# saholmes/stark-mlwe

Hardware: AMD Instinct MI355X
Metric: prove ms + Fr-NTT achieved GB/s, 2^20/2^24 trace at 1/2/4/8 GPUs (higher is better)
Workload: dtype u256 (4x u64 Montgomery limbs, Pallas Fr); 1 GPU; one 2^20-row trace x 4 columns (2^20 rows per GPU), blowup 8: LDE (iNTT + coset NTT) + DEEP-ALI merge + FRI folds + Poseidon leaf hashes + Poseidon-Merkle trees (schedule [16,16,8]), kernels only; log_trace_per_gpu=20, log_blowup=3, field=pallas_fr

## Files before the change

### stark_mlwe_amd/csrc/capi_poseidon.hip

```cpp
#include <algorithm>
#include <cstring>
#include <type_traits>
#include "poseidon_launch.hpp"
#include "poseidon_dev.hpp"
#include "poseidon_pair.hpp"
#include "poseidon_coop.hpp"
#include "poseidon_chain.hpp"
#include "poseidon_wave.hpp"
#include "poseidon_transcript.hpp"
#include "fri_dev.hpp"
#include "merkle_batch.hpp"

using namespace stark;

static const size_t kMaxLds = 160 * 1024;
static inline int poseidon_block(int t) { return (size_t)t * 32 * 64 <= kMaxLds ? 64 : 32; }
static inline size_t poseidon_lds(int t, int block) { return (size_t)t * 32 * block; }
enum class PoseidonForm { Lane, WavePair, OneWave, FiveWave, Wide };
enum class PoseidonOp { MerkleLevel, LeafLayer, TrHash, ColumnSponges, RaggedSponges, DeviceTranscript };
constexpr size_t kChainMaxNodes = 256, kChainMaxLeaves = 2048, kChainMaxSponges = 512, kCoopMaxNodes = 4096, kCoopMaxLeaves = 4096, kCoopMaxSponges = 4096;
static PoseidonForm poseidon_form(const stark_ctx* ctx, const stark_params* p, PoseidonOp op, size_t n) {
    const PoseidonDev& d = p->dev;
    const bool lane_only = ctx->opt.poseidon_lane_only, one_wave = ctx->opt.sponge_one_wave;
    const bool chain = !lane_only && !one_wave && d.t == 17 && d.rf == 8 && d.rp == 64 && d.chain_a;
    switch (op) {
    case PoseidonOp::MerkleLevel:
        if ((ctx->side_commit || ctx->opt.merkle_wave_pair) && !lane_only && (d.t == 9 || d.t == 17)) return PoseidonForm::WavePair;
        if (chain && n <= kChainMaxNodes) return PoseidonForm::FiveWave;
        if (!lane_only && (d.t == 9 || d.t == 17)) return n <= kCoopMaxNodes ? PoseidonForm::OneWave : PoseidonForm::WavePair;
        if (!lane_only && (d.t == 33 || d.t == 65 || d.t == 129) && n <= 0x7fffffffu) return PoseidonForm::Wide;
        return PoseidonForm::Lane;
    case PoseidonOp::LeafLayer:
        if (ctx->side_commit && !lane_only) return PoseidonForm::WavePair;
        if (chain && n <= kChainMaxLeaves) return PoseidonForm::FiveWave;
        if (!lane_only && !one_wave && n <= kCoopMaxLeaves) return PoseidonForm::OneWave;
        return lane_only ? PoseidonForm::Lane : PoseidonForm::WavePair;
    case PoseidonOp::TrHash:
        if (chain && n <= kChainMaxSponges) return PoseidonForm::FiveWave;
        return !lane_only && n <= kCoopMaxSponges ? PoseidonForm::OneWave : PoseidonForm::Lane;
    case PoseidonOp::RaggedSponges:
        if (lane_only) return PoseidonForm::Lane;
        [[fallthrough]];
    case PoseidonOp::ColumnSponges:
        return d.chain_a && !one_wave ? PoseidonForm::FiveWave : PoseidonForm::OneWave;
    case PoseidonOp::DeviceTranscript:
        return chain && n <= kChainMaxSponges ? PoseidonForm::FiveWave : PoseidonForm::OneWave;
    }
    return PoseidonForm::Lane;
}
static inline row::Consts row_consts_of(const stark_ctx* ctx) {
    const RowConstsHost h = row_consts_host(); row::Consts RK; for (int i = 0; i < 9; ++i) RK.ni[i] = h.ni[i]; for (int i = 0; i < 5; ++i) RK.t[i] = h.t[i]; RK.dbg = (uint32_t)ctx->opt.sponge_debug; return RK;
}

static int32_t ctx_leaf_init(stark_ctx* ctx, fr_t** out) {
    if (!ctx->leaf_init) {
        const fr_t AB = host::h_tag("FSv1-ABSORB-BYTES"), CH = host::h_tag("FSv1-CHALLENGE");
        fr_t init[17]; for (auto& x : init) x = host::h_zero();
        init[0] = AB; init[1] = host::h_words("FRI/leaf/poseidon")[0]; init[2] = AB; init[3] = host::h_words("FRI/leaf")[0];
         init[6] = CH; init[7] = AB; init[8] = host::h_words("leaf")[0]; init[16] = host::h_tag("FSv1-TRANSCRIPT-INIT");
        stark_params* tp = nullptr; STARK_TRY(ctx_transcript_params(ctx, &tp));
        const host::PoseidonConsts& c = tp->ref;
        fr_t blob[17 + 51 + 40];
        for (auto& x : blob) x = host::h_zero();
        for (int j = 0; j < 17; ++j) blob[j] = init[j];
        fr_t x[17]; for (int j = 0; j < 17; ++j) x[j] = fr_pow5<PallasFr>(host::h_add(init[j], c.rc_full[j]));
        for (int i = 0; i < 17; ++i) {
            fr_t k = host::h_zero();
            for (int j = 0; j < 17; ++j) if (j != 4 && j != 5) k = host::h_add(k, host::h_mul(c.mds[(size_t)i * 17 + j], x[j]));
            blob[17 + i] = k; blob[34 + i] = c.mds[(size_t)i * 17 + 4]; blob[51 + i] = c.mds[(size_t)i * 17 + 5];
            uint32_t* m45 = reinterpret_cast<uint32_t*>(&blob[68]);
            const fr_t k20 = fr_from_u64<PallasFr>(1ull << FR29_SBOX_SHIFT);
            fr29_const_from<PallasFr>(host::h_mul(c.mds[(size_t)i * 17 + 4], k20), m45 + 9 * i); fr29_const_from<PallasFr>(host::h_mul(c.mds[(size_t)i * 17 + 5], k20), m45 + 9 * (17 + i));
        }
        DevMem d; STARK_TRY(d.fill_sync(ctx, blob, sizeof(blob)));
        ctx->leaf_init = std::move(d);
    }
    *out = ctx->leaf_init.fr(); return STARK_OK;
}

namespace stark {

static int32_t tr_frame(stark_ctx* ctx, const char* tag, fr_t** dev, int* np, int* ns) {
    const std::string key(tag);
    auto it = ctx->tr_frames.find(key);
    if (it == ctx->tr_frames.end()) {
        std::vector<fr_t> fr; const int p = host::tr_hash_frame(tag, fr);
        DevMem d; STARK_TRY(d.fill_sync(ctx, fr.data(), fr.size() * sizeof(fr_t)));
        it = ctx->tr_frames.emplace(key, std::move(d)).first; ctx->tr_frame_dims[key] = {p, (int)fr.size() - p};
    }
    *dev = it->second.fr(); *np = ctx->tr_frame_dims[key].first; *ns = ctx->tr_frame_dims[key].second; return STARK_OK;
}
static int32_t launch_tr_hash(stark_ctx* ctx, stark_params* tp, PoseidonForm form, const TrStream& T, fr_t* out_dev) {
    const bool ragged = T.layout == TrStream::Ragged;
    switch (form) {
    case PoseidonForm::FiveWave:
        if (ragged) hipLaunchKernelGGL(k_tr_hash_chain_ragged, dim3((unsigned)T.n), dim3(320), chain_lds_bytes(), ctx->stream, tp->dev, T, row_consts_of(ctx), out_dev);
        else hipLaunchKernelGGL(k_tr_hash_chain, dim3((unsigned)T.n), dim3(320), chain_lds_bytes(), ctx->stream, tp->dev, T, row_consts_of(ctx), out_dev);
        break;
    case PoseidonForm::OneWave:
        if (ragged) hipLaunchKernelGGL((k_tr_hash_coop<true, true>), dim3((unsigned)T.n), dim3(64), coop_lds_bytes(17), ctx->stream, tp->dev, T, out_dev);
        else if (T.layout == TrStream::Equal) hipLaunchKernelGGL(k_tr_hash_coop<false>, dim3((unsigned)T.n), dim3(64), coop_lds_bytes(17), ctx->stream, tp->dev, T, out_dev);
        else hipLaunchKernelGGL(k_tr_hash_coop<true>, dim3((unsigned)T.n), dim3(64), coop_lds_bytes(17), ctx->stream, tp->dev, T, out_dev);
        break;
    default: {
        const int block = 64;
        if (ragged) hipLaunchKernelGGL(k_tr_hash_ragged, dim3((unsigned)((T.n + block - 1) / block)), dim3(block), poseidon_lds(17, block), ctx->stream, tp->dev, T, out_dev);
        else hipLaunchKernelGGL(k_tr_hash, dim3((unsigned)((T.n + block - 1) / block)), dim3(block), poseidon_lds(17, block), ctx->stream, tp->dev, T, out_dev);
    } }
    STARK_HIP(ctx, hipGetLastError());
    return STARK_OK;
}
int32_t tr_hash_dev(stark_ctx* ctx, const char* tag, const fr_t* fields_dev, size_t k, size_t n, fr_t* out_dev) {
    stark_params* tp = nullptr; STARK_TRY(ctx_transcript_params(ctx, &tp));
    fr_t* frame = nullptr; int np = 0, ns = 0; STARK_TRY(tr_frame(ctx, tag, &frame, &np, &ns));
    if (n == 0) return STARK_OK;
    const TrStream T = TrStream::equal(frame, np, ns, fields_dev, k, n, host::h_tag("FSv1-TRANSCRIPT-INIT"));
    return launch_tr_hash(ctx, tp, poseidon_form(ctx, tp, PoseidonOp::TrHash, n), T, out_dev);
}
static int32_t tr_hash_columns(stark_ctx* ctx, const char* const tags[4], const fr_t* const cols[4], const fr_t* const* ptrs_dev, size_t nblocks, size_t n0, fr_t* out_dev) {
    stark_params* tp = nullptr; STARK_TRY(ctx_transcript_params(ctx, &tp));
    TrStream T{}; T.layout = ptrs_dev ? TrStream::BatchColumns : TrStream::Columns; T.n = nblocks; T.batch = ptrs_dev; T.cap = host::h_tag("FSv1-TRANSCRIPT-INIT");
    for (int c = 0; c < 4; ++c) {
        fr_t* frame = nullptr; int np = 0, ns = 0; STARK_TRY(tr_frame(ctx, tags[c], &frame, &np, &ns));
        T.prefix[c] = frame; T.np[c] = np; T.suffix[c] = frame + np; T.ns[c] = ns; T.fields[c] = cols ? cols[c] : nullptr; T.k[c] = n0;
    }
    return launch_tr_hash(ctx, tp, poseidon_form(ctx, tp, PoseidonOp::ColumnSponges, nblocks), T, out_dev);
}
int32_t tr_hash_columns4_dev(stark_ctx* ctx, const char* const tags[4], const fr_t* const cols[4], size_t n0, fr_t* out4_dev) {
    return tr_hash_columns(ctx, tags, cols, nullptr, 4, n0, out4_dev);
}
int32_t tr_hash_columns_batch_dev(stark_ctx* ctx, const char* const tags[4], const fr_t* const* ptrs_dev, size_t batch, size_t n0, fr_t* out_dev) {
    return tr_hash_columns(ctx, tags, nullptr, ptrs_dev, 4 * batch, n0, out_dev);
}
int32_t tr_hash_many_dev(stark_ctx* ctx, size_t n, const char* const* tags, const fr_t* const* fields, const size_t* k, fr_t* out_dev, bool column_sponges) {
    stark_params* tp = nullptr; STARK_TRY(ctx_transcript_params(ctx, &tp));
    std::vector<TrFrameRef> fr(n);
    for (size_t i = 0; i < n; ++i) { fr_t* frame = nullptr; STARK_TRY(tr_frame(ctx, tags[i], &frame, &fr[i].np, &fr[i].ns)); fr[i].frame = frame; }
    if (n == 0) return STARK_OK;
    if (n > 0x7fffffffu) return ctx->fail(STARK_ERR_UNSUPPORTED, "tr_hash_many: more than 2^31 - 1 items in one call");
    const std::vector<TrStream::Item> items = tr_ragged_items(fr.data(), fields, k, n);
    DevBuf d; STARK_HIP(ctx, d.alloc(ctx, n * sizeof(TrStream::Item))); STARK_TRY(ctx_upload_staged(ctx, d.p, items.data(), n * sizeof(TrStream::Item)));
    const TrStream T = tr_ragged_stream((const TrStream::Item*)d.p, n, host::h_tag("FSv1-TRANSCRIPT-INIT"));
    return launch_tr_hash(ctx, tp, poseidon_form(ctx, tp, column_sponges ? PoseidonOp::ColumnSponges : PoseidonOp::RaggedSponges, n), T, out_dev);
}
int32_t tr_hash_host1(stark_ctx* ctx, const char* tag, const std::vector<fr_t>& fields, fr_t* out) {
    DevBuf in, o; STARK_HIP(ctx, in.alloc(ctx, fields.size() * sizeof(fr_t))); STARK_HIP(ctx, o.alloc(ctx, sizeof(fr_t)));
    STARK_TRY(ctx_upload_staged(ctx, in.p, fields.data(), fields.size() * sizeof(fr_t)));
    STARK_TRY(tr_hash_dev(ctx, tag, in.fr(), fields.size(), 1, o.fr()));
    STARK_HIP(ctx, o.download_sync(out, sizeof(fr_t)));
    return STARK_OK;
}
int32_t tr_stream_on(stark_ctx* ctx, stark_params* tp, fr_t* state, uint32_t* pos, const fr_t* fields, size_t n, bool finish, fr_t* out) {
    if (poseidon_form(ctx, tp, PoseidonOp::DeviceTranscript, 1) == PoseidonForm::FiveWave)
        hipLaunchKernelGGL(k_tr_stream_chain, dim3(1), dim3(320), chain_lds_bytes(), ctx->stream, tp->dev, row_consts_of(ctx), state, pos, fields, (uint64_t)n, finish ? 1 : 0, finish ? out : (fr_t*)nullptr);
    else
        hipLaunchKernelGGL(k_tr_stream, dim3(1), dim3(64), coop_lds_bytes(17), ctx->stream, tp->dev, state, pos, fields, (uint64_t)n, finish ? 1 : 0, finish ? out : (fr_t*)nullptr);
    STARK_HIP(ctx, hipGetLastError()); return STARK_OK;
}
int32_t tr_batch_on(stark_ctx* ctx, stark_params* tp, const TrBatchStream& T, size_t n_for_form) {
    if (!T.n_active) return STARK_OK;
    if (poseidon_form(ctx, tp, PoseidonOp::DeviceTranscript, n_for_form) == PoseidonForm::FiveWave)
        for (uint32_t sg = 0; sg < (uint32_t)T.nseg; ++sg)
            hipLaunchKernelGGL(k_tr_batch_chain, dim3((unsigned)T.n_active), dim3(320), chain_lds_bytes(), ctx->stream, tp->dev, row_consts_of(ctx), T, sg);
    else
        hipLaunchKernelGGL(k_tr_batch, dim3((unsigned)T.n_active), dim3(64), coop_lds_bytes(17), ctx->stream, tp->dev, T);
    STARK_HIP(ctx, hipGetLastError()); return STARK_OK;
}

}

extern "C" {

int32_t stark_poseidon_permute_batch_dev(stark_ctx_t* ctx, stark_params_t* p, uint64_t* states, size_t n) {
    if (!ctx || !p || (!states && n)) return STARK_ERR_INVALID_ARG;
    STARK_TRY(ctx_enter(ctx));
    if (!n) return STARK_OK;
    const int block = poseidon_block(p->dev.t);
    hipLaunchKernelGGL(k_permute_batch, dim3((unsigned)((n + block - 1) / block)), dim3(block), poseidon_lds(p->dev.t, block), ctx->stream, p->dev, as_fr(states), n);
    STARK_HIP(ctx, hipGetLastError()); return STARK_OK;
}
int32_t stark_poseidon_permute_batch(stark_ctx_t* ctx, stark_params_t* p, uint64_t* states, size_t n) {
    if (!ctx || !p || (!states && n)) return STARK_ERR_INVALID_ARG;
    STARK_TRY(ctx_enter(ctx));
    size_t bytes = n * p->dev.t * sizeof(fr_t); DevBuf d; CallerUploads up(ctx); STARK_HIP(ctx, up.up(d, states, bytes));
    STARK_TRY(stark_poseidon_permute_batch_dev(ctx, p, (uint64_t*)d.p, n));
    STARK_HIP(ctx, up.download_sync(states, d.p, bytes));
    return STARK_OK;
}
static int32_t hash_stream(stark_ctx_t* ctx, stark_params_t* p, int mode, const uint64_t* a, size_t na, const uint64_t* b, size_t nb, const fr_t& tag, size_t n, uint64_t* out) {
    DevBuf da, db, dout; CallerUploads up(ctx);
    STARK_HIP(ctx, up.up(da, a, n * na * sizeof(fr_t))); STARK_HIP(ctx, up.up(db, b, n * nb * sizeof(fr_t))); STARK_HIP(ctx, dout.alloc(ctx, n * sizeof(fr_t)));
    const int block = poseidon_block(p->dev.t);
    hipLaunchKernelGGL(k_hash_stream, dim3((unsigned)((n + block - 1) / block)), dim3(block), poseidon_lds(p->dev.t, block), ctx->stream, p->dev, mode, da.fr(), na, db.fr(), nb, tag, n, dout.fr());
    STARK_HIP(ctx, hipGetLastError());
    STARK_HIP(ctx, up.download_sync(out, dout.p, n * sizeof(fr_t)));
    return STARK_OK;
}
int32_t stark_poseidon_hash_with_ds_dynamic(stark_ctx_t* ctx, stark_params_t* p, const uint64_t* ds, size_t nds, const uint64_t* in, size_t cnt, size_t n, uint64_t* out) {
    if (!ctx || !p || !out || (!ds && nds) || (!in && cnt)) return STARK_ERR_INVALID_ARG;
    STARK_TRY(ctx_enter(ctx));
    if (!n) return STARK_OK;
    return hash_stream(ctx, p, 0, ds, nds, in, cnt, host::h_zero(), n, out);
}
int32_t stark_poseidon_hash_with_ds(stark_ctx_t* ctx, stark_params_t* p, const uint64_t* in, size_t cnt, const uint64_t* ds_tag, uint64_t* out) {
    if (!ctx || !p || !out || !ds_tag || (!in && cnt)) return STARK_ERR_INVALID_ARG;
    STARK_TRY(ctx_enter(ctx));
    if (p->dev.t != 17) return ctx->fail(STARK_ERR_INVALID_ARG, "hash_with_ds is the fixed t=17 sponge");
    return hash_stream(ctx, p, 1, nullptr, 0, in, cnt, load_fr(ds_tag), 1, out);
}
}
static int32_t pair_block8_form(stark_ctx* ctx, const stark_params* p, bool* on) {
    *on = ctx->opt.poseidon_block8 && p->dev.t == 17 && p->dev.rp % 8 == 0;
    if (*on && (!p->dev.blk8_efrag || !p->dev.blk8_lfrag || !p->dev.blk8_unit_frag || !p->dev.blk8_gfrag || !p->dev.rc_partial_scaled29)) return ctx->fail(STARK_ERR_UNSUPPORTED, "poseidon_block8: the parameter set has no block-8 tables");
    return STARK_OK;
}
template <class DS>
static int32_t launch_ds(stark_ctx_t* ctx, hipStream_t st, stark_params_t* p, const DS& D, fr_t* out) {
    if (!D.n_out) return STARK_OK;
    const int t = p->dev.t; const unsigned nodes = (unsigned)D.n_out, pairs = (unsigned)((D.n_out + 63) / 64);
    bool b8 = false; STARK_TRY(pair_block8_form(ctx, p, &b8));
    switch (poseidon_form(ctx, p, PoseidonOp::MerkleLevel, D.n_out)) {
    case PoseidonForm::FiveWave: hipLaunchKernelGGL(k_hash_ds_chain<DS>, dim3(nodes), dim3(320), chain_lds_bytes(), st, p->dev, D, row_consts_of(ctx), out); break;
    case PoseidonForm::OneWave:
        if (t == 17) hipLaunchKernelGGL((k_hash_ds_coop<17, DS>), dim3(nodes), dim3(64), coop_lds_bytes(17), st, p->dev, D, out);
        else hipLaunchKernelGGL((k_hash_ds_coop<9, DS>), dim3(nodes), dim3(64), coop_lds_bytes(9), st, p->dev, D, out);
        break;
    case PoseidonForm::WavePair:
        if constexpr (std::is_same<DS, DsStream>::value) {
            if (t == 17 && ctx->opt.merkle_node16_pair && D.mode == 0 && D.arity == 16 && D.n_in == 16 * D.n_out) {
                if (b8) hipLaunchKernelGGL(k_node16_pair<true>, dim3(pairs), dim3(128), pair_lds_bytes(17), st, p->dev, D.arity_f, D.level_f, D.label_f, D.pos0, D.in0, D.n_out, out);
                else hipLaunchKernelGGL(k_node16_pair<false>, dim3(pairs), dim3(128), pair_lds_bytes(17), st, p->dev, D.arity_f, D.level_f, D.label_f, D.pos0, D.in0, D.n_out, out);
                break;
            }
        }
        if (t == 17 && b8) hipLaunchKernelGGL((k_hash_ds2<17, DS, true>), dim3(pairs), dim3(128), pair_lds_bytes(17), st, p->dev, D, out);
        else if (t == 17) hipLaunchKernelGGL((k_hash_ds2<17, DS>), dim3(pairs), dim3(128), pair_lds_bytes(17), st, p->dev, D, out);
        else hipLaunchKernelGGL((k_hash_ds2<9, DS>), dim3(pairs), dim3(128), pair_lds_bytes(9), st, p->dev, D, out);
        break;
    case PoseidonForm::Wide:
        if (t == 33) hipLaunchKernelGGL((k_hash_ds_wave<33, DS>), dim3(nodes), dim3(64), wave_lds_bytes(t), st, p->dev, D, out);
        else if (t == 65) hipLaunchKernelGGL((k_hash_ds_wave<65, DS>), dim3(nodes), dim3(64), wave_lds_bytes(t), st, p->dev, D, out);
        else hipLaunchKernelGGL((k_hash_ds_wave<129, DS>), dim3(nodes), dim3(64), wave_lds_bytes(t), st, p->dev, D, out);
        break;
    case PoseidonForm::Lane: {
        const int block = poseidon_block(t);
        hipLaunchKernelGGL(k_hash_ds<DS>, dim3((unsigned)((D.n_out + block - 1) / block)), dim3(block), poseidon_lds(t, block), st, p->dev, D, out);
    } }
    STARK_HIP(ctx, hipGetLastError()); return STARK_OK;
}
int32_t stark::hash_ds_on(stark_ctx* ctx, hipStream_t st, stark_params* p, const DsStream& D, fr_t* out) { return launch_ds(ctx, st, p, D, out); }
int32_t stark::hash_ds_on(stark_ctx* ctx, hipStream_t st, stark_params* p, const DsGatherStream& D, fr_t* out) { return launch_ds(ctx, st, p, D, out); }
int32_t stark::hash_ds_on(stark_ctx* ctx, hipStream_t st, stark_params* p, const DsBatchStream& D, fr_t* out) { return launch_ds(ctx, st, p, D, out); }
int32_t stark::hash_ds_on(stark_ctx* ctx, hipStream_t st, stark_params* p, const DsBatchPairStream& D, fr_t* out) { return launch_ds(ctx, st, p, D, out); }
int32_t stark::hash_ds_on(stark_ctx* ctx, hipStream_t st, stark_params* p, const DsBatchPairPtrStream& D, fr_t* out) { return launch_ds(ctx, st, p, D, out); }
int32_t stark::hash_ds_on(stark_ctx* ctx, hipStream_t st, stark_params* p, const DsRaggedStream& D, fr_t* out) { return launch_ds(ctx, st, p, D, out); }
static void lds_attr(const void* kernel) { (void)hipFuncSetAttribute(kernel, hipFuncAttributeMaxDynamicSharedMemorySize, (int)kMaxLds); }
template <class DS>
static void ds_attrs() {
    lds_attr((const void*)k_hash_ds<DS>); lds_attr((const void*)k_hash_ds2<17, DS>); lds_attr((const void*)k_hash_ds2<17, DS, true>); lds_attr((const void*)k_hash_ds2<9, DS>); lds_attr((const void*)k_hash_ds_chain<DS>);
}
void stark::poseidon_set_attrs() {
    ds_attrs<DsStream>(); ds_attrs<DsGatherStream>(); ds_attrs<DsBatchStream>(); ds_attrs<DsBatchPairStream>(); ds_attrs<DsBatchPairPtrStream>(); ds_attrs<DsRaggedStream>();
    for (const void* k : {(const void*)k_leaf_pair, (const void*)k_permute_batch, (const void*)k_tr_hash, (const void*)k_hash_stream, (const void*)k_leaf_pair2<false>, (const void*)k_leaf_pair2<true>, (const void*)k_node16_pair<false>, (const void*)k_node16_pair<true>,
                          (const void*)k_tr_hash_chain, (const void*)k_tr_hash_chain_ragged, (const void*)k_tr_hash_ragged, (const void*)k_leaf_pair_chain, (const void*)k_tr_stream_chain, (const void*)k_tr_batch_chain})
        lds_attr(k);
}
extern "C" {
int32_t stark_poseidon_hash_ds_batch_dev(stark_ctx_t* ctx, stark_params_t* p, size_t arity, uint32_t level, uint64_t pos0, uint64_t label, const uint64_t* in, size_t n_in, uint64_t* out) {
    if (!ctx || !p || !in || !out || arity == 0) return STARK_ERR_INVALID_ARG;
    STARK_TRY(ctx_enter(ctx));
    if (host::width_for_arity(arity) != p->dev.t) return ctx->fail(STARK_ERR_INVALID_ARG, "arity incompatible with Poseidon width");
    STARK_TRY(ctx_enter(ctx));
    return hash_ds_on(ctx, ctx->stream, p, DsStream::make(0, arity, level, pos0, label, as_fr(in), nullptr, n_in), as_fr(out));
}
int32_t stark_poseidon_hash_ds_batch(stark_ctx_t* ctx, stark_params_t* p, size_t arity, uint32_t level, uint64_t pos0, uint64_t label, const uint64_t* in, size_t n_in, uint64_t* out) {
    if (!ctx || !p || !in || !out || arity == 0) return STARK_ERR_INVALID_ARG;
    STARK_TRY(ctx_enter(ctx));
    size_t n_out = (n_in + arity - 1) / arity; DevBuf di, dout; CallerUploads up(ctx); STARK_HIP(ctx, up.up(di, in, n_in * sizeof(fr_t))); STARK_HIP(ctx, dout.alloc(ctx, n_out * sizeof(fr_t)));
    STARK_TRY(stark_poseidon_hash_ds_batch_dev(ctx, p, arity, level, pos0, label, (const uint64_t*)di.p, n_in, (uint64_t*)dout.p));
    STARK_HIP(ctx, up.download_sync(out, dout.p, n_out * sizeof(fr_t)));
    return STARK_OK;
}
}
namespace stark {
static bool same_consts(const host::PoseidonConsts& a, const host::PoseidonConsts& b) {
    if (a.t != b.t || a.rf != b.rf || a.rp != b.rp || a.mds.size() != b.mds.size() || a.rc_full.size() != b.rc_full.size() || a.rc_partial.size() != b.rc_partial.size()) return false;
    for (size_t i = 0; i < a.mds.size(); ++i) if (!fr_eq(a.mds[i], b.mds[i])) return false;
    for (size_t i = 0; i < a.rc_full.size(); ++i) if (!fr_eq(a.rc_full[i], b.rc_full[i])) return false;
    for (size_t i = 0; i < a.rc_partial.size(); ++i) if (!fr_eq(a.rc_partial[i], b.rc_partial[i])) return false;
    return true;
}
int32_t leaf_pair_hash_on(stark_ctx* ctx, hipStream_t st, const fr_t* f, const fr_t* f_next, size_t n, size_t m, fr_t* h) {
    if (!n) return STARK_OK;
    stark_params* tp = nullptr; STARK_TRY(ctx_transcript_params(ctx, &tp));
    fr_t* init = nullptr; STARK_TRY(ctx_leaf_init(ctx, &init));
    const LeafStream L{init, f, f_next, m, n};
    bool b8 = false; STARK_TRY(pair_block8_form(ctx, tp, &b8));
    switch (poseidon_form(ctx, tp, PoseidonOp::LeafLayer, n)) {
    case PoseidonForm::FiveWave: hipLaunchKernelGGL(k_leaf_pair_chain, dim3((unsigned)n), dim3(320), chain_lds_bytes(), st, tp->dev, row_consts_of(ctx), L, h); break;
    case PoseidonForm::OneWave: hipLaunchKernelGGL(k_leaf_pair_coop, dim3((unsigned)n), dim3(64), coop_lds_bytes(17), st, tp->dev, L, h); break;
    case PoseidonForm::WavePair:
        if (b8) hipLaunchKernelGGL(k_leaf_pair2<true>, dim3((unsigned)((n + 63) / 64)), dim3(128), pair_lds_bytes(17), st, tp->dev, init + 17, f, f_next, n, m, h);
        else hipLaunchKernelGGL(k_leaf_pair2<false>, dim3((unsigned)((n + 63) / 64)), dim3(128), pair_lds_bytes(17), st, tp->dev, init + 17, f, f_next, n, m, h);
        break;
    default: hipLaunchKernelGGL(k_leaf_pair, dim3((unsigned)((n + 63) / 64)), dim3(64), poseidon_lds(17, 64), st, tp->dev, L, h);
    }
    STARK_HIP(ctx, hipGetLastError()); return STARK_OK;
}
}
extern "C" {
int32_t stark_leaf_pair_hash_dev(stark_ctx_t* ctx, stark_params_t* tp, const uint64_t* f, const uint64_t* f_next, size_t n, size_t m, uint64_t* h) {
    if (!ctx || (!f && n) || (!h && n) || m == 0) return STARK_ERR_INVALID_ARG;
    STARK_TRY(ctx_enter(ctx));
    if (tp) {
        if (tp->dev.t != 17) return ctx->fail(STARK_ERR_INVALID_ARG, "leaf hash uses the t=17 transcript permutation");
        stark_params* mine = nullptr; STARK_TRY(ctx_transcript_params(ctx, &mine));
        if (tp != mine && !same_consts(tp->ref, mine->ref)) return ctx->fail(STARK_ERR_INVALID_ARG, "hash_leaf_pair is defined over transcript::default_params(); the handle holds other constants");
    }
    return leaf_pair_hash_on(ctx, ctx->stream, as_fr(f), as_fr(f_next), n, m, as_fr(h));
}
int32_t stark_leaf_pair_hash(stark_ctx_t* ctx, stark_params_t* tp, const uint64_t* f, const uint64_t* f_next, size_t n, size_t m, uint64_t* h) {
    if (!ctx || (!f && n) || (!h && n) || m == 0) return STARK_ERR_INVALID_ARG;
    STARK_TRY(ctx_enter(ctx));
    size_t nn = f_next ? (n + m - 1) / m : 0; DevBuf df, dn, dh; CallerUploads up(ctx);
    STARK_HIP(ctx, up.up(df, f, n * sizeof(fr_t))); STARK_HIP(ctx, up.up(dn, f_next, nn * sizeof(fr_t))); STARK_HIP(ctx, dh.alloc(ctx, n * sizeof(fr_t)));
    STARK_TRY(stark_leaf_pair_hash_dev(ctx, tp, (const uint64_t*)df.p, f_next ? (const uint64_t*)dn.p : nullptr, n, m, (uint64_t*)dh.p));
    STARK_HIP(ctx, up.download_sync(h, dh.p, n * sizeof(fr_t))); return STARK_OK;
}
int32_t stark_tr_hash_fields_tagged_dev(stark_ctx_t* ctx, stark_params_t* tp, const char* tag, const uint64_t* fields, size_t k, size_t n, uint64_t* out) {
    if (!ctx || !tag || (!fields && k && n) || (!out && n)) return STARK_ERR_INVALID_ARG;
    STARK_TRY(ctx_enter(ctx));
    (void)tp;
    return tr_hash_dev(ctx, tag, as_fr(fields), k, n, as_fr(out));
}
int32_t stark_tr_hash_fields_tagged(stark_ctx_t* ctx, stark_params_t* tp, const char* tag, const uint64_t* fields, size_t k, size_t n, uint64_t* out) {
    if (!ctx || !tag || (!fields && k && n) || (!out && n)) return STARK_ERR_INVALID_ARG;
    STARK_TRY(ctx_enter(ctx));
    DevBuf di, dout; CallerUploads up(ctx); STARK_HIP(ctx, up.up(di, fields, n * k * sizeof(fr_t))); STARK_HIP(ctx, dout.alloc(ctx, n * sizeof(fr_t)));
    STARK_TRY(stark_tr_hash_fields_tagged_dev(ctx, tp, tag, (const uint64_t*)di.p, k, n, (uint64_t*)dout.p));
    STARK_HIP(ctx, up.download_sync(out, dout.p, n * sizeof(fr_t))); return STARK_OK;
}
int32_t stark_tr_hash_many_dev(stark_ctx_t* ctx, size_t n, const char* const* tags, const uint64_t* const* fields, const size_t* k, uint64_t* out) {
    if (!ctx) return STARK_ERR_INVALID_ARG;
    if (!n) return STARK_OK;
    if (!tags || !k || !out) return STARK_ERR_INVALID_ARG;
    STARK_TRY(ctx_enter(ctx));
    const uintptr_t o0 = (uintptr_t)out, o1 = o0 + n * sizeof(fr_t);
    for (size_t i = 0; i < n; ++i) {
        if (!tags[i]) return ctx->fail(STARK_ERR_INVALID_ARG, "tr_hash_many: null tag " + std::to_string(i));
        if (!k[i]) continue;
        if (!fields || !fields[i]) return ctx->fail(STARK_ERR_INVALID_ARG, "tr_hash_many: null fields with k > 0, item " + std::to_string(i));
        const uintptr_t f0 = (uintptr_t)fields[i];
        if (f0 < o1 && o0 < f0 + k[i] * sizeof(fr_t)) return ctx->fail(STARK_ERR_INVALID_ARG, "tr_hash_many: out overlaps the fields of item " + std::to_string(i));
    }
    return tr_hash_many_dev(ctx, n, tags, reinterpret_cast<const fr_t* const*>(fields), k, as_fr(out), false);
}

}
namespace stark {
int32_t merkle_build_on(stark_ctx* ctx, hipStream_t st, stark_params* p, size_t arity, uint64_t label, const fr_t* leaves, size_t n, int pairs, const fr_t* cp, size_t cp_div,
                        uint64_t first_pos, uint32_t level0, size_t stop_at_len, DevBuf&& level0_block, std::unique_ptr<stark_tree>& out) {
    if (n == 0) return ctx->fail(STARK_ERR_INVALID_ARG, "no leaves");
    if (host::width_for_arity(arity) != p->dev.t) return ctx->fail(STARK_ERR_INVALID_ARG, "arity incompatible with Poseidon width");
    if (arity == 1 && n > 1) return ctx->fail(STARK_ERR_UNSUPPORTED, "arity 1 with more than one leaf never terminates in the reference");
    std::unique_ptr<stark_tree> T(new stark_tree(ctx, p, arity, label));
    auto add_level = [&](DevBuf&& b, size_t len) { T->levels.push_back(b.fr()); T->lens.push_back(len); T->blocks.push_back(std::move(b)); };
    const bool moved_in = level0_block.p && !pairs;
    { DevBuf l0; if (moved_in) l0 = std::move(level0_block); else STARK_TRY(l0.take(ctx, n * sizeof(fr_t))); add_level(std::move(l0), n); }
    if (pairs) STARK_TRY(hash_ds_on(ctx, st, p, DsStream::make(1, arity, 0xFFFFFFFFu, first_pos, label, leaves, cp, n, cp_div), T->levels[0]));
    else if (!moved_in && hipMemcpyAsync(T->levels[0], leaves, n * sizeof(fr_t), hipMemcpyDeviceToDevice, st) != hipSuccess) return ctx->fail(STARK_ERR_HIP, "copy leaves");
    uint32_t level = level0; uint64_t pos = first_pos; size_t stop = stop_at_len > 0 ? stop_at_len : 1;
    while (T->lens.back() > stop) {
        size_t len = T->lens.back(), nn = (len + arity - 1) / arity;
        if (pos % arity) return ctx->fail(STARK_ERR_INVALID_ARG, "shard offset not aligned to the arity");
        pos /= arity;
        { DevBuf nx; STARK_TRY(nx.take(ctx, nn * sizeof(fr_t))); add_level(std::move(nx), nn); }
        STARK_TRY(hash_ds_on(ctx, st, p, DsStream::make(0, arity, level, pos, label, T->levels[T->levels.size() - 2], nullptr, len), T->levels.back()));
        level += 1;
    }
    out = std::move(T); return STARK_OK;
}
}
extern "C" {
int32_t stark_merkle_build_dev(stark_ctx_t* ctx, stark_params_t* p, size_t arity, uint64_t label, const uint64_t* leaves, size_t n, int32_t pairs, const uint64_t* cp,
                               uint64_t first_pos, uint32_t level0, int32_t stop_at_len, stark_tree_t** out) {
    if (!ctx || !p || !leaves || !out || arity == 0 || (pairs && !cp)) return ctx ? ctx->fail(STARK_ERR_INVALID_ARG, "bad merkle args") : STARK_ERR_INVALID_ARG;
    STARK_TRY(ctx_enter(ctx));
    std::unique_ptr<stark_tree> T;
    STARK_TRY(merkle_build_on(ctx, ctx->stream, p, arity, label, as_fr(leaves), n, pairs, as_fr(cp), 1, first_pos, level0, stop_at_len > 0 ? (size_t)stop_at_len : 0, DevBuf(), T));
    *out = T.release(); return STARK_OK;
}
int32_t stark_merkle_build(stark_ctx_t* ctx, stark_params_t* p, size_t arity, uint64_t label, const uint64_t* leaves, size_t n, int32_t pairs, const uint64_t* cp, stark_tree_t** out) {
    if (!ctx || !p || !leaves || !out || (pairs && !cp)) return STARK_ERR_INVALID_ARG;
    STARK_TRY(ctx_enter(ctx));
    if (n == 0) return ctx->fail(STARK_ERR_INVALID_ARG, "no leaves");
    DevBuf dl, dc; CallerUploads up(ctx); STARK_HIP(ctx, up.up(dl, leaves, n * sizeof(fr_t)));
    if (pairs) STARK_HIP(ctx, up.up(dc, cp, n * sizeof(fr_t)));
    STARK_TRY(stark_merkle_build_dev(ctx, p, arity, label, (const uint64_t*)dl.p, n, pairs, pairs ? (const uint64_t*)dc.p : nullptr, 0, 0, 0, out));
    STARK_HIP(ctx, up.sync()); return STARK_OK;
}
int32_t stark_merkle_num_levels(stark_tree_t* t) { return t ? (int32_t)t->levels.size() : STARK_ERR_INVALID_ARG; }
size_t stark_merkle_level_len(stark_tree_t* t, int32_t lvl) { return (t && lvl >= 0 && (size_t)lvl < t->lens.size()) ? t->lens[lvl] : 0; }
const uint64_t* stark_merkle_level_dev(stark_tree_t* t, int32_t lvl) { return (t && lvl >= 0 && (size_t)lvl < t->levels.size()) ? (const uint64_t*)t->levels[lvl] : nullptr; }
int32_t stark_merkle_level(stark_tree_t* t, int32_t lvl, uint64_t* out) {
    if (!t || !out || lvl < 0 || (size_t)lvl >= t->levels.size()) return STARK_ERR_INVALID_ARG;
    stark_ctx* ctx = t->ctx; STARK_TRY(ctx_enter(ctx));
    STARK_HIP(ctx, hipMemcpyAsync(out, t->levels[lvl], t->lens[lvl] * sizeof(fr_t), hipMemcpyDeviceToHost, ctx->stream)); STARK_HIP(ctx, hipStreamSynchronize(ctx->stream)); return STARK_OK;
}
int32_t stark_merkle_root(stark_tree_t* t, uint64_t* out4) {
    if (!t || !out4) return STARK_ERR_INVALID_ARG;
    if (t->lens.back() != 1) return t->ctx->fail(STARK_ERR_INVALID_ARG, "partial (sharded) tree has no root");
    return stark_merkle_level(t, (int32_t)t->levels.size() - 1, out4);
}
int32_t stark_merkle_gather(stark_tree_t* t, int32_t lvl, const size_t* idx, size_t k, uint64_t* out) {
    if (!t || (!idx && k) || (!out && k) || lvl < 0 || (size_t)lvl >= t->levels.size()) return STARK_ERR_INVALID_ARG;
    stark_ctx* ctx = t->ctx; if (!k) return STARK_OK;
    STARK_TRY(ctx_enter(ctx));
    for (size_t i = 0; i < k; ++i) if (idx[i] >= t->lens[lvl]) return ctx->fail(STARK_ERR_INVALID_ARG, "gather index out of range");
    MerkleGatherList G; G.level(t->levels[lvl], std::vector<size_t>(idx, idx + k));
    return gather_rows(ctx, G, nullptr, out);
}
int32_t stark_merkle_free(stark_tree_t* t) { if (!t) return STARK_ERR_INVALID_ARG; delete t; return STARK_OK; }

}

namespace stark {
struct MerkleBatchDevExec {
    stark_ctx* ctx; stark_params* p; std::shared_ptr<TreeBlocks> blocks; DevArena mem;
    MerkleBatchDevExec(stark_ctx* c, stark_params* p_) : ctx(c), p(p_), blocks(std::make_shared<TreeBlocks>()), mem(c) {}
    int32_t level_block(size_t n_fr, fr_t** out) {
        DevBuf b; STARK_TRY(b.take(ctx, n_fr * sizeof(fr_t))); *out = b.fr(); blocks->blocks.push_back(std::move(b)); return STARK_OK;
    }
    int32_t tables(const uint64_t* labels, const fr_t* const* leaves, const fr_t* const* cp, size_t B, const uint64_t** labels_x, const fr_t* const** leaves_x, const fr_t* const** cp_x) {
        std::vector<uint64_t> h((cp ? 3 : 2) * B);
        for (size_t b = 0; b < B; ++b) { h[b] = labels[b]; h[B + b] = (uint64_t)(uintptr_t)leaves[b]; if (cp) h[2 * B + b] = (uint64_t)(uintptr_t)cp[b]; }
        uint64_t* d = nullptr; STARK_TRY(mem.put(h, &d));
        *labels_x = d; *leaves_x = (const fr_t* const*)(d + B); *cp_x = cp ? (const fr_t* const*)(d + 2 * B) : nullptr; return STARK_OK;
    }
    int32_t copy_rows(const fr_t* const* src_x, size_t n, size_t B, fr_t* dst) {
        for (size_t b0 = 0; b0 < B; b0 += 65535)
            hipLaunchKernelGGL(k_copy_rows, dim3((unsigned)((n + 255) / 256), (unsigned)std::min<size_t>(65535, B - b0)), dim3(256), 0, ctx->stream, src_x + b0, (uint64_t)n, dst + b0 * n);
        STARK_HIP(ctx, hipGetLastError()); return STARK_OK;
    }
    int32_t pair_level(const DsBatchPairPtrStream& D, fr_t* out) { return hash_ds_on(ctx, ctx->stream, p, D, out); }
    int32_t ds_level(const DsBatchStream& D, fr_t* out) { return hash_ds_on(ctx, ctx->stream, p, D, out); }
};
int32_t merkle_build_batch_on(stark_ctx* ctx, stark_params* p, size_t arity, size_t batch, const uint64_t* labels, const uint64_t* const* leaves, size_t n, int pairs,
                              const uint64_t* const* cp, stark_tree** out) {
    for (size_t b = 0; b < batch; ++b) out[b] = nullptr;
    if (n == 0) return ctx->fail(STARK_ERR_INVALID_ARG, "no leaves");
    if (arity == 0 || host::width_for_arity(arity) != p->dev.t) return ctx->fail(STARK_ERR_INVALID_ARG, "arity incompatible with Poseidon width");
    if (arity == 1 && n > 1) return ctx->fail(STARK_ERR_UNSUPPORTED, "arity 1 with more than one leaf never terminates in the reference");
    for (size_t b = 0; b < batch; ++b) if (!leaves[b]) return ctx->fail(STARK_ERR_INVALID_ARG, "null leaves entry");
    if (n > 0x7fffffffu / batch) return ctx->fail(STARK_ERR_INVALID_ARG, "batch x n exceeds 2^31 - 1 leaves: one level of the batch is one launch");
    MerkleBatchDevExec X(ctx, p);
    std::vector<size_t> lens; std::vector<fr_t*> base;
    STARK_TRY(merkle_build_batch(X, arity, batch, labels, reinterpret_cast<const fr_t* const*>(leaves), n, pairs, reinterpret_cast<const fr_t* const*>(cp), lens, base));
    std::vector<std::unique_ptr<stark_tree>> trees(batch);
    for (size_t b = 0; b < batch; ++b) {
        trees[b].reset(new stark_tree(ctx, p, arity, labels[b])); trees[b]->shared = X.blocks;
        for (size_t v = 0; v < lens.size(); ++v) { trees[b]->levels.push_back(base[v] + b * lens[v]); trees[b]->lens.push_back(lens[v]); }
    }
    for (size_t b = 0; b < batch; ++b) out[b] = trees[b].release();
    return STARK_OK;
}
struct MerkleMixedDevExec : MerkleBatchDevExec {
    using MerkleBatchDevExec::MerkleBatchDevExec;
    int32_t segments(const std::vector<DsRaggedStream::Seg>& h, const DsRaggedStream::Seg** x) { DsRaggedStream::Seg* d = nullptr; STARK_TRY(mem.put(h, &d)); *x = d; return STARK_OK; }
    int32_t copy_ragged(const DsRaggedStream& D, fr_t* dst) {
        hipLaunchKernelGGL(k_copy_ragged, dim3((unsigned)((D.n_out + 255) / 256)), dim3(256), 0, ctx->stream, D, dst);
        STARK_HIP(ctx, hipGetLastError()); return STARK_OK;
    }
    int32_t ragged_level(const DsRaggedStream& D, fr_t* out) { return hash_ds_on(ctx, ctx->stream, p, D, out); }
};
int32_t merkle_build_mixed_batch_on(stark_ctx* ctx, stark_params* p, size_t arity, size_t batch, const uint64_t* labels, const uint64_t* const* leaves, const size_t* n, int pairs,
                                    const uint64_t* const* cp, stark_tree** out) {
    for (size_t b = 0; b < batch; ++b) out[b] = nullptr;
    if (arity == 0 || host::width_for_arity(arity) != p->dev.t) return ctx->fail(STARK_ERR_INVALID_ARG, "arity incompatible with Poseidon width");
    size_t sum = 0;
    for (size_t b = 0; b < batch; ++b) {
        if (!leaves[b]) return ctx->fail(STARK_ERR_INVALID_ARG, "null leaves entry");
        if (n[b] == 0) return ctx->fail(STARK_ERR_INVALID_ARG, "no leaves");
        if (n[b] > 0x7fffffffu - sum) return ctx->fail(STARK_ERR_INVALID_ARG, "the sum of n exceeds 2^31 - 1 leaves: one level of the batch is one launch");
        sum += n[b];
    }
    if (arity == 1 && sum > batch) return ctx->fail(STARK_ERR_UNSUPPORTED, "arity 1 with more than one leaf never terminates in the reference");
    MerkleMixedDevExec X(ctx, p);
    std::vector<std::vector<size_t>> lens, at; std::vector<fr_t*> base;
    STARK_TRY(merkle_build_mixed_batch(X, arity, batch, labels, reinterpret_cast<const fr_t* const*>(leaves), n, pairs, reinterpret_cast<const fr_t* const*>(cp), lens, at, base));
    std::vector<std::unique_ptr<stark_tree>> trees(batch);
    for (size_t b = 0; b < batch; ++b) {
        trees[b].reset(new stark_tree(ctx, p, arity, labels[b])); trees[b]->shared = X.blocks;
        for (size_t v = 0; v < lens[b].size(); ++v) { trees[b]->levels.push_back(base[v] + at[b][v]); trees[b]->lens.push_back(lens[b][v]); }
    }
    for (size_t b = 0; b < batch; ++b) out[b] = trees[b].release();
    return STARK_OK;
}
int32_t gather_rows(stark_ctx* ctx, const MerkleGatherList& G, fr_t* out_dev, void* out_host) {
    const size_t k = G.size(), nb = G.base.size();
    if (!k) return STARK_OK;
    std::vector<uint64_t> h(nb + 2 * k + (k + 1) / 2);
    for (size_t i = 0; i < nb; ++i) h[i] = (uint64_t)(uintptr_t)G.base[i];
    for (size_t i = 0; i < k; ++i) { h[nb + i] = G.index[i]; h[nb + k + i] = G.row_of(i); }
    memcpy(h.data() + nb + 2 * k, G.src.data(), k * 4);
    DevBuf d, o; STARK_HIP(ctx, d.alloc(ctx, h.size() * 8));
    if (!out_dev) { STARK_HIP(ctx, o.alloc(ctx, k * sizeof(fr_t))); out_dev = o.fr(); }
    STARK_TRY(ctx_upload_staged(ctx, d.p, h.data(), h.size() * 8));
    const uint64_t* t = (const uint64_t*)d.p;
    hipLaunchKernelGGL(k_gather_rows, dim3((unsigned)((k + 255) / 256)), dim3(256), 0, ctx->stream, (const fr_t* const*)t, (const uint32_t*)(t + nb + 2 * k), t + nb, t + nb + k, (uint64_t)k, out_dev);
    STARK_HIP(ctx, hipGetLastError());
    if (!out_host) return STARK_OK;
    STARK_HIP(ctx, hipMemcpyAsync(out_host, out_dev, k * sizeof(fr_t), hipMemcpyDeviceToHost, ctx->stream)); STARK_HIP(ctx, hipStreamSynchronize(ctx->stream));
    return STARK_OK;
}
struct MerkleOpenDevExec { stark_ctx* ctx; int32_t gather(const MerkleGatherList& G, fr_t* out_host) { return gather_rows(ctx, G, nullptr, out_host); } };
static int32_t same_ctx_trees(stark_tree* const* trees, size_t batch, stark_ctx** ctx) {
    for (size_t b = 0; b < batch; ++b) if (!trees[b]) return STARK_ERR_INVALID_ARG;
    stark_ctx* c = trees[0]->ctx;
    for (size_t b = 1; b < batch; ++b) if (trees[b]->ctx != c) return c->fail(STARK_ERR_INVALID_ARG, "the trees of a batch must share one context");
    for (size_t b = 0; b < batch; ++b) if (trees[b]->lens.back() != 1) return c->fail(STARK_ERR_INVALID_ARG, "partial (sharded) tree in a batch");
    *ctx = c; return STARK_OK;
}
}

extern "C" {
int32_t stark_merkle_build_batch_dev(stark_ctx_t* ctx, stark_params_t* p, size_t arity, size_t batch, const uint64_t* tree_labels, const uint64_t* const* leaves, size_t n, int32_t pairs,
                                     const uint64_t* const* cp, stark_tree_t** out) {
    if (!batch) return STARK_OK;
    if (!out) return ctx ? ctx->fail(STARK_ERR_INVALID_ARG, "bad merkle batch args") : STARK_ERR_INVALID_ARG;
    for (size_t b = 0; b < batch; ++b) out[b] = nullptr;
    if (!ctx || !p || !tree_labels || !leaves || (pairs && !cp)) return ctx ? ctx->fail(STARK_ERR_INVALID_ARG, "bad merkle batch args") : STARK_ERR_INVALID_ARG;
    STARK_TRY(ctx_enter(ctx));
    return merkle_build_batch_on(ctx, p, arity, batch, tree_labels, leaves, n, pairs, pairs ? cp : nullptr, out);
}
int32_t stark_merkle_build_mixed_batch_dev(stark_ctx_t* ctx, stark_params_t* p, size_t arity, size_t batch, const uint64_t* tree_labels, const uint64_t* const* leaves, const size_t* n,
                                           int32_t pairs, const uint64_t* const* cp, stark_tree_t** out) {
    if (!batch) return STARK_OK;
    if (!out) return ctx ? ctx->fail(STARK_ERR_INVALID_ARG, "bad merkle batch args") : STARK_ERR_INVALID_ARG;
    for (size_t b = 0; b < batch; ++b) out[b] = nullptr;
    if (!ctx || !p || !tree_labels || !leaves || !n || (pairs && !cp)) return ctx ? ctx->fail(STARK_ERR_INVALID_ARG, "bad merkle batch args") : STARK_ERR_INVALID_ARG;
    STARK_TRY(ctx_enter(ctx));
    return merkle_build_mixed_batch_on(ctx, p, arity, batch, tree_labels, leaves, n, pairs, pairs ? cp : nullptr, out);
}
int32_t stark_merkle_roots_batch(stark_tree_t* const* trees, size_t batch, uint64_t* roots) {
    if (!batch) return STARK_OK;
    if (!trees || !roots) return STARK_ERR_INVALID_ARG;
    stark_ctx* ctx = nullptr; STARK_TRY(same_ctx_trees(trees, batch, &ctx));
    STARK_TRY(ctx_enter(ctx));
    MerkleGatherList G;
    for (size_t b = 0; b < batch; ++b) G.level(trees[b]->levels.back(), std::vector<size_t>(1, 0));
    return gather_rows(ctx, G, nullptr, roots);
}
int32_t stark_merkle_open_batch(stark_tree_t* const* trees, size_t batch, const size_t* idx, const size_t* idx_off, stark_proof_t** out) {
    if (!batch) return STARK_OK;
    if (!out) return STARK_ERR_INVALID_ARG;
    for (size_t b = 0; b < batch; ++b) out[b] = nullptr;
    if (!trees || !idx || !idx_off) return STARK_ERR_INVALID_ARG;
    stark_ctx* ctx = nullptr; STARK_TRY(same_ctx_trees(trees, batch, &ctx));
    STARK_TRY(ctx_enter(ctx));
    std::vector<MerkleTreeView> views(batch);
    for (size_t b = 0; b < batch; ++b) views[b] = MerkleTreeView{trees[b]->arity, &trees[b]->lens, trees[b]->levels.data()};
    MerkleOpenDevExec X{ctx}; std::vector<std::vector<uint8_t>> proofs;
    const int32_t rc = merkle_open_batch(X, views.data(), batch, idx, idx_off, proofs);
    if (rc == -1) return ctx->fail(STARK_ERR_INVALID_ARG, "open batch: idx_off not increasing, an empty index list or a leaf index out of range");
    if (rc) return rc;
    std::vector<std::unique_ptr<stark_proof>> pf(batch);
    for (size_t b = 0; b < batch; ++b) { pf[b].reset(new stark_proof()); pf[b]->bytes = std::move(proofs[b]); }
    hand_out(pf, out); return STARK_OK;
}
int32_t stark_merkle_open(stark_tree_t* t, const size_t* idx, size_t k, uint8_t* buf, size_t cap, size_t* len) {
    if (!t || !len || (!idx && k)) return STARK_ERR_INVALID_ARG;
    stark_ctx* ctx = t->ctx;
    if (!k) return ctx->fail(STARK_ERR_INVALID_ARG, "open_many: empty indices");
    if (t->lens.back() != 1) return ctx->fail(STARK_ERR_INVALID_ARG, "cannot open a partial tree");
    for (size_t i = 0; i < k; ++i) if (idx[i] >= t->lens[0]) return ctx->fail(STARK_ERR_INVALID_ARG, "leaf index out of range");
    STARK_TRY(ctx_enter(ctx));
    const MerkleTreeView view{t->arity, &t->lens, t->levels.data()}; const size_t off[2] = {0, k};
    MerkleOpenDevExec X{ctx}; std::vector<std::vector<uint8_t>> proofs;
    STARK_TRY(merkle_open_batch(X, &view, 1, idx, off, proofs));
    const std::vector<uint8_t>& b = proofs[0];
    *len = b.size();
    if (buf) { if (cap < b.size()) return ctx->fail(STARK_ERR_INVALID_ARG, "buffer too small"); memcpy(buf, b.data(), b.size()); }
    return STARK_OK;
}
}
```

### stark_mlwe_amd/csrc/host_util.hpp

```cpp
#pragma once
#include <cstdint>
#include <cstring>
#include <string>
#include <vector>
#include "fr.hpp"
#include "fr29.hpp"

namespace stark {
namespace host {

struct Blake3 {
    static constexpr uint32_t kIV[8] = {0x6A09E667u, 0xBB67AE85u, 0x3C6EF372u, 0xA54FF53Au, 0x510E527Fu, 0x9B05688Cu, 0x1F83D9ABu, 0x5BE0CD19u};
    enum : uint32_t { F_CHUNK_START = 1, F_CHUNK_END = 2, F_PARENT = 4, F_ROOT = 8 };
    static uint32_t ror(uint32_t x, unsigned n) { return (x >> n) | (x << (32 - n)); }
    static void mix(uint32_t* v, int a, int b, int c, int d, uint32_t x, uint32_t y) {
        v[a] += v[b] + x; v[d] = ror(v[d] ^ v[a], 16); v[c] += v[d]; v[b] = ror(v[b] ^ v[c], 12);
        v[a] += v[b] + y; v[d] = ror(v[d] ^ v[a], 8);  v[c] += v[d]; v[b] = ror(v[b] ^ v[c], 7);
    }
    static void compress(const uint32_t h[8], const uint8_t block[64], uint32_t blen, uint64_t ctr, uint32_t flags, uint32_t out[16]) {
        static const uint8_t sched[7][16] = {
            {0, 1, 2, 3, 4, 5, 6, 7, 8, 9, 10, 11, 12, 13, 14, 15}, {2, 6, 3, 10, 7, 0, 4, 13, 1, 11, 12, 5, 9, 14, 15, 8},
            {3, 4, 10, 12, 13, 2, 7, 14, 6, 5, 9, 0, 11, 15, 8, 1}, {10, 7, 12, 9, 14, 3, 13, 15, 4, 0, 11, 2, 5, 8, 1, 6},
            {12, 13, 9, 11, 15, 10, 14, 8, 7, 2, 5, 3, 0, 1, 6, 4}, {9, 14, 11, 5, 8, 12, 15, 1, 13, 3, 0, 10, 2, 6, 4, 7},
            {11, 15, 5, 0, 1, 9, 8, 6, 14, 10, 2, 12, 3, 4, 7, 13}};
// ... 8 lines not shown
            mix(v, 2, 6, 10, 14, m[s[4]], m[s[5]]);  mix(v, 3, 7, 11, 15, m[s[6]], m[s[7]]);
            mix(v, 0, 5, 10, 15, m[s[8]], m[s[9]]);  mix(v, 1, 6, 11, 12, m[s[10]], m[s[11]]);
            mix(v, 2, 7, 8, 13, m[s[12]], m[s[13]]); mix(v, 3, 4, 9, 14, m[s[14]], m[s[15]]);
        }
        for (int i = 0; i < 8; ++i) { out[i] = v[i] ^ v[i + 8]; out[i + 8] = v[i + 8] ^ h[i]; }
    }
    struct Node { uint32_t h[8]; uint8_t block[64]; uint32_t blen; uint64_t ctr; uint32_t flags; };
    static void cv_of(const Node& n, uint32_t extra, uint32_t cv[8]) { uint32_t o[16]; compress(n.h, n.block, n.blen, n.ctr, n.flags | extra, o); memcpy(cv, o, 32); }
    static Node chunk_node(const uint8_t* p, size_t len, uint64_t index) {
        Node n; memcpy(n.h, kIV, 32); n.ctr = index;
        size_t off = 0; bool first = true;
        while (len - off > 64) {
            uint32_t o[16]; compress(n.h, p + off, 64, index, first ? F_CHUNK_START : 0, o); memcpy(n.h, o, 32);
            off += 64; first = false;
        }
        memset(n.block, 0, 64); memcpy(n.block, p + off, len - off); n.blen = (uint32_t)(len - off);
        n.flags = (first ? F_CHUNK_START : 0) | F_CHUNK_END;
        return n;
    }
    static Node subtree(const uint8_t* p, size_t len, uint64_t index) {
        if (len <= 1024) return chunk_node(p, len, index);
        size_t chunks = (len + 1023) / 1024, left = 1; while (left * 2 < chunks) left *= 2;
        Node l = subtree(p, left * 1024, index), r = subtree(p + left * 1024, len - left * 1024, index + left);
        Node n; memcpy(n.h, kIV, 32); n.ctr = 0; n.blen = 64; n.flags = F_PARENT;
        uint32_t a[8], b[8]; cv_of(l, 0, a); cv_of(r, 0, b);
        for (int i = 0; i < 8; ++i) for (int j = 0; j < 4; ++j) { n.block[4 * i + j] = (uint8_t)(a[i] >> (8 * j)); n.block[32 + 4 * i + j] = (uint8_t)(b[i] >> (8 * j)); }
        return n;
    }
    static void hash(const uint8_t* p, size_t len, uint8_t out[32]) {
        Node root = subtree(p, len, 0);
        if (root.flags & F_PARENT) root.ctr = 0;
        uint32_t cv[8]; cv_of(root, F_ROOT, cv);
        for (int i = 0; i < 8; ++i) for (int j = 0; j < 4; ++j) out[4 * i + j] = (uint8_t)(cv[i] >> (8 * j));
    }
};

struct ChaCha12Rng {
    uint32_t st[16]; uint32_t out[16]; unsigned have = 0;
    explicit ChaCha12Rng(const uint8_t seed[32]) {
        st[0] = 0x61707865u; st[1] = 0x3320646eu; st[2] = 0x79622d32u; st[3] = 0x6b206574u;
        for (int i = 0; i < 8; ++i) st[4 + i] = (uint32_t)seed[4 * i] | (uint32_t)seed[4 * i + 1] << 8 | (uint32_t)seed[4 * i + 2] << 16 | (uint32_t)seed[4 * i + 3] << 24;
        st[12] = st[13] = st[14] = st[15] = 0;
    }
    static uint32_t rol(uint32_t x, unsigned n) { return (x << n) | (x >> (32 - n)); }
    void block() {
        uint32_t x[16]; memcpy(x, st, 64);
        auto Q = [&](int a, int b, int c, int d) {
            x[a] += x[b]; x[d] = rol(x[d] ^ x[a], 16); x[c] += x[d]; x[b] = rol(x[b] ^ x[c], 12);
            x[a] += x[b]; x[d] = rol(x[d] ^ x[a], 8);  x[c] += x[d]; x[b] = rol(x[b] ^ x[c], 7); };
        for (int i = 0; i < 6; ++i) { Q(0, 4, 8, 12); Q(1, 5, 9, 13); Q(2, 6, 10, 14); Q(3, 7, 11, 15); Q(0, 5, 10, 15); Q(1, 6, 11, 12); Q(2, 7, 8, 13); Q(3, 4, 9, 14); }
        for (int i = 0; i < 16; ++i) out[i] = x[i] + st[i];
        if (++st[12] == 0) ++st[13];
        have = 16;
    }
    uint32_t next_u32() { if (!have) block(); return out[16 - have--]; }
    uint64_t next_u64() { uint64_t lo = next_u32(), hi = next_u32(); return lo | hi << 32; }
};

typedef PallasFr PF;
inline fr_t h_one() { return fr_one<PF>(); }
inline fr_t h_zero() { return fr_zero<PF>(); }
inline fr_t h_mul(const fr_t& a, const fr_t& b) { return fr_mul<PF>(a, b); }
inline fr_t h_add(const fr_t& a, const fr_t& b) { return fr_add<PF>(a, b); }
inline fr_t h_sub(const fr_t& a, const fr_t& b) { return fr_sub<PF>(a, b); }
inline fr_t h_u64(uint64_t x) { return fr_from_u64<PF>(x); }
inline fr_t h_from_le_bytes_mod_order(const uint8_t* b, size_t n) {
    fr_t acc = h_zero(); const fr_t two32 = h_u64(1ull << 32);
    size_t nw = (n + 3) / 4;
    for (size_t k = nw; k-- > 0;) {
        uint32_t w = 0; for (size_t j = 0; j < 4; ++j) if (4 * k + j < n) w |= (uint32_t)b[4 * k + j] << (8 * j);
        acc = h_add(h_mul(acc, two32), h_u64(w));
    }
    return acc;
}
inline void h_to_bytes_le(const fr_t& a, uint8_t out[32]) {
    fr_t c = fr_to_canonical<PF>(a);
    for (int i = 0; i < 8; ++i) for (int j = 0; j < 4; ++j) out[4 * i + j] = (uint8_t)(c.v[i] >> (8 * j));
}
inline fr_t h_fr_from_hash(const char* tag, const std::vector<uint8_t>& data) {
    std::vector<uint8_t> buf(tag, tag + strlen(tag)); buf.insert(buf.end(), data.begin(), data.end());
    uint8_t d[32]; Blake3::hash(buf.data(), buf.size(), d);
    uint8_t wide[64]; memset(wide, 0, 64); memcpy(wide, d, 32);
    return h_from_le_bytes_mod_order(wide, 64);
}
inline fr_t h_tag(const char* s) {
    size_t n = strlen(s);
    if (n <= 32) { uint8_t le[32] = {0}; memcpy(le, s, n); return h_from_le_bytes_mod_order(le, 32); }
    fr_t acc = h_zero();
    for (size_t off = 0; off < n; off += 32) { uint8_t le[32] = {0}; size_t c = n - off < 32 ? n - off : 32; memcpy(le, s + off, c); acc = h_add(acc, h_from_le_bytes_mod_order(le, 32)); }
    return acc;
}
inline std::vector<fr_t> h_words(const char* s) {
    std::vector<fr_t> out; size_t n = strlen(s);
    for (size_t off = 0; off < n; off += 31) { uint8_t le[32] = {0}; size_t c = n - off < 31 ? n - off : 31; memcpy(le, s + off, c); out.push_back(h_from_le_bytes_mod_order(le, 32)); }
    return out;
}
inline int tr_hash_frame(const char* tag, std::vector<fr_t>& frame) {
    const fr_t AB = h_tag("FSv1-ABSORB-BYTES"), CH = h_tag("FSv1-CHALLENGE");
    frame.clear();
    frame.push_back(AB); for (auto& w : h_words("FRI/FS")) frame.push_back(w);
    frame.push_back(AB); for (auto& w : h_words(tag)) frame.push_back(w);
    const int np = (int)frame.size();
    frame.push_back(CH); frame.push_back(AB); for (auto& w : h_words("out")) frame.push_back(w);
    return np;
}

struct PoseidonConsts {
    int t = 0, rf = 0, rp = 0;
    std::vector<fr_t> mds;
    std::vector<fr_t> rc_full;
    std::vector<fr_t> rc_partial;
};
inline void put64(std::vector<uint8_t>& v, uint64_t x) { for (int j = 0; j < 8; ++j) v.push_back((uint8_t)(x >> (8 * j))); }
inline PoseidonConsts derive_consts(const std::string& seed, int t, int rf, int rp) {
    PoseidonConsts c; c.t = t; c.rf = rf; c.rp = rp;
    c.mds.resize((size_t)t * t); c.rc_full.resize((size_t)rf * t); c.rc_partial.resize(rp);
    for (int i = 0; i < t; ++i) for (int j = 0; j < t; ++j) { std::vector<uint8_t> d; put64(d, i); put64(d, j); d.insert(d.end(), seed.begin(), seed.end()); c.mds[(size_t)i * t + j] = h_fr_from_hash("POSEIDON-MDS", d); }
    for (int r = 0; r < rf; ++r) for (int i = 0; i < t; ++i) { std::vector<uint8_t> d; put64(d, r); put64(d, i); d.insert(d.end(), seed.begin(), seed.end()); c.rc_full[(size_t)r * t + i] = h_fr_from_hash("POSEIDON-RC-FULL", d); }
    for (int r = 0; r < rp; ++r) { std::vector<uint8_t> d; put64(d, r); d.insert(d.end(), seed.begin(), seed.end()); c.rc_partial[r] = h_fr_from_hash("POSEIDON-RC-PART", d); }
    return c;
}
inline int width_for_arity(size_t arity) { return arity <= 8 ? 9 : arity <= 16 ? 17 : arity <= 32 ? 33 : arity <= 64 ? 65 : arity <= 128 ? 129 : -1; }
inline int rp_for_width(int t) { switch (t) { case 9: return 60; case 17: return 64; case 33: return 68; case 65: return 76; case 129: return 84; default: return -1; } }
inline PoseidonConsts consts_for_width(int t) {
    std::string seed = "POSEIDON-PALLAS-T"; for (int j = 0; j < 8; ++j) seed.push_back((char)(((uint64_t)t >> (8 * j)) & 0xff));
    return derive_consts(seed, t, 8, rp_for_width(t));
}
inline PoseidonConsts consts_transcript() { return derive_consts("POSEIDON-T17-X5-TRANSCRIPT", 17, 8, 64); }

struct KernelConsts {
    int t = 0, rf = 0, rp = 0;
    std::vector<fr_t> rc_full, rc_partial;
    std::vector<fr_t> lu, lu_pre;
    std::vector<fr_t> row0;
    std::vector<fr_t> sparse;
    std::vector<fr_t> mds;
    std::vector<fr_t> mds_pre;
    std::vector<fr_t> gamma;
    std::vector<uint32_t> lu29, lu_pre29, row0_29, sparse29, gamma29;
    std::vector<uint32_t> mds29, mds_pre29;
    std::vector<uint32_t> rc_full29;
    std::vector<int8_t> mds_frag, mds_pre_frag;
    std::vector<uint32_t> chain_a, chain_g, chain_w;
    std::vector<int8_t> blk8_efrag, blk8_lfrag, blk8_gfrag;
    std::vector<uint32_t> gamma8_29;
    std::vector<fr_t> blk8_lambda, rc_partial_scaled;
    std::vector<int8_t> blk8s_efrag, blk8s_lfrag, blk8s_gfrag;
    std::vector<uint32_t> blk8_unscale29, rc_partial_scaled29;
    bool ok = false;
};
template <class Pred> inline std::vector<uint32_t> to_radix29(const std::vector<fr_t>& v, Pred scaled) {
    const fr_t k = fr_from_u64<PF>(1ull << FR29_SBOX_SHIFT);
    std::vector<uint32_t> o(v.size() * 9);
    for (size_t i = 0; i < v.size(); ++i) fr29_const_from<PF>(scaled(i) ? fr_mul<PF>(v[i], k) : v[i], &o[9 * i]);
    return o;
}
inline void mfma_frag_of(fr_t g, int8_t* out) {
    const fr_t k256 = fr_from_u64<PF>(256);
    int8_t d[32][32];
    for (int b = 0; b < 32; ++b, g = h_mul(g, k256)) {
        const fr_t c = fr_to_canonical<PF>(g); int cy = 0;
        for (int k = 0; k < 32; ++k) { const int v = (int)((c.v[k >> 2] >> (8 * (k & 3))) & 0xff) + 0x80 + cy; cy = v >> 8; d[b][k] = (int8_t)((v & 0xff) - 0x80); }
    }
    for (int l = 0; l < 64; ++l) for (int j = 0; j < 16; ++j) out[(size_t)l * 16 + j] = d[16 * (l >> 5) + j][l & 31];
}
inline std::vector<int8_t> mfma_frags(const fr_t* mat, int rows, int cols, const fr_t& scale) {
    std::vector<int8_t> out((size_t)rows * cols * 64 * 16, 0);
    for (int i = 0; i < rows; ++i) for (int e = 0; e < cols; ++e) mfma_frag_of(h_mul(mat[(size_t)i * cols + e], scale), &out[((size_t)i * cols + e) * 64 * 16]);
    return out;
}
inline std::vector<int8_t> mfma_frags(const std::vector<fr_t>& mat, int t) { return mfma_frags(mat.data(), t, t, fr_from_u64<PF>(1ull << FR29_SBOX_SHIFT)); }
inline bool mat_inverse(std::vector<fr_t> a, int n, std::vector<fr_t>& inv) {
    inv.assign((size_t)n * n, h_zero()); for (int i = 0; i < n; ++i) inv[(size_t)i * n + i] = h_one();
    for (int c = 0; c < n; ++c) {
        int p = -1; for (int r = c; r < n; ++r) if (!fr_is_zero(a[(size_t)r * n + c])) { p = r; break; }
        if (p < 0) return false;
        if (p != c) for (int k = 0; k < n; ++k) { std::swap(a[(size_t)p * n + k], a[(size_t)c * n + k]); std::swap(inv[(size_t)p * n + k], inv[(size_t)c * n + k]); }
        fr_t pi = fr_inv<PF>(a[(size_t)c * n + c]);
        for (int k = 0; k < n; ++k) { a[(size_t)c * n + k] = h_mul(a[(size_t)c * n + k], pi); inv[(size_t)c * n + k] = h_mul(inv[(size_t)c * n + k], pi); }
        for (int r = 0; r < n; ++r) if (r != c) {
            fr_t f = a[(size_t)r * n + c]; if (fr_is_zero(f)) continue;
            for (int k = 0; k < n; ++k) { a[(size_t)r * n + k] = h_sub(a[(size_t)r * n + k], h_mul(f, a[(size_t)c * n + k])); inv[(size_t)r * n + k] = h_sub(inv[(size_t)r * n + k], h_mul(f, inv[(size_t)c * n + k])); }
        }
    }
    return true;
}
inline bool lu_pack(const std::vector<fr_t>& m, int n, std::vector<fr_t>& lu) {
    lu = m;
    for (int k = 0; k < n; ++k) {
        if (fr_is_zero(lu[(size_t)k * n + k])) return false;
        fr_t pi = fr_inv<PF>(lu[(size_t)k * n + k]);
        for (int i = k + 1; i < n; ++i) {
            fr_t f = h_mul(lu[(size_t)i * n + k], pi); lu[(size_t)i * n + k] = f;
            for (int j = k + 1; j < n; ++j) lu[(size_t)i * n + j] = h_sub(lu[(size_t)i * n + j], h_mul(f, lu[(size_t)k * n + j]));
        }
    }
    return true;
}
inline KernelConsts make_kernel_consts(const PoseidonConsts& c) {
    KernelConsts k; k.t = c.t; k.rf = c.rf; k.rp = c.rp; k.rc_full = c.rc_full; k.rc_partial = c.rc_partial; k.mds = c.mds;
    const int t = c.t, n = t - 1;
    k.row0.assign(c.mds.begin(), c.mds.begin() + t);
    std::vector<fr_t> cur = c.mds;
    k.sparse.assign((size_t)c.rp * (2 * t - 1), h_zero());
    for (int r = c.rp - 1; r >= 0; --r) {
        std::vector<fr_t> hat((size_t)n * n), hinv;
        for (int i = 0; i < n; ++i) for (int j = 0; j < n; ++j) hat[(size_t)i * n + j] = cur[(size_t)(i + 1) * t + (j + 1)];
        if (!mat_inverse(hat, n, hinv)) return k;
        fr_t* sp = &k.sparse[(size_t)r * (2 * t - 1)];
        sp[0] = cur[0];
        for (int j = 0; j < n; ++j) { fr_t acc = h_zero(); for (int q = 0; q < n; ++q) acc = h_add(acc, h_mul(cur[(size_t)0 * t + (q + 1)], hinv[(size_t)q * n + j])); sp[1 + j] = acc; }
        for (int i = 0; i < n; ++i) sp[t + i] = cur[(size_t)(i + 1) * t + 0];
        std::vector<fr_t> nxt((size_t)t * t);
        for (int j = 0; j < t; ++j) nxt[j] = c.mds[j];
        for (int i = 0; i < n; ++i) for (int j = 0; j < t; ++j) { fr_t acc = h_zero(); for (int q = 0; q < n; ++q) acc = h_add(acc, h_mul(hat[(size_t)i * n + q], c.mds[(size_t)(q + 1) * t + j])); nxt[(size_t)(i + 1) * t + j] = acc; }
        cur.swap(nxt);
    }
    if (c.rp % 4) return k;
    k.gamma.assign((size_t)(c.rp / 4) * 6, h_zero());
    for (int b = 0; b < c.rp / 4; ++b)
        for (int q = 1; q < 4; ++q)
            for (int p2 = 0; p2 < q; ++p2) {
                const fr_t* uq = &k.sparse[(size_t)(4 * b + q) * (2 * t - 1)];
                const fr_t* wp = &k.sparse[(size_t)(4 * b + p2) * (2 * t - 1)];
                fr_t acc = h_zero();
                for (int j = 1; j < t; ++j) acc = h_add(acc, h_mul(uq[j], wp[t - 1 + j]));
                k.gamma[(size_t)b * 6 + q * (q - 1) / 2 + p2] = acc;
            }
    if (!lu_pack(c.mds, t, k.lu)) return k;
    if (!lu_pack(cur, t, k.lu_pre)) return k;
    k.mds_pre = cur;
    const auto upper = [t](size_t i) { return (int)(i % t) >= (int)(i / t); };
    const auto all = [](size_t) { return true; };
    const auto a_and_w = [t](size_t i) { const int c = (int)(i % (2 * t - 1)); return c == 0 || c >= t; };
    k.lu29 = to_radix29(k.lu, upper); k.lu_pre29 = to_radix29(k.lu_pre, upper); k.row0_29 = to_radix29(k.row0, all);
    k.sparse29 = to_radix29(k.sparse, a_and_w); k.gamma29 = to_radix29(k.gamma, all);
    k.mds29 = to_radix29(k.mds, all); k.mds_pre29 = to_radix29(k.mds_pre, all);
    k.rc_full29.resize(k.rc_full.size() * 9);
    for (size_t i = 0; i < k.rc_full.size(); ++i) { const fr29_t u = fr29_unpack(k.rc_full[i]); for (int j = 0; j < 9; ++j) k.rc_full29[9 * i + j] = u.l[j]; }
    if (t == 17) { k.mds_frag = mfma_frags(k.mds, t); k.mds_pre_frag = mfma_frags(k.mds_pre, t); }
    if (t == 17 && c.rp % 8 == 0) {
        const int nb = c.rp / 8, w = 2 * t - 1;
        const fr_t s20 = fr_from_u64<PF>(1ull << FR29_SBOX_SHIFT);
        std::vector<fr_t> g8((size_t)nb * 28, h_zero()), um((size_t)8 * n), wm((size_t)n * 8);
        const fr_t kappa = fr_inv<PF>(s20), a_inv = fr_inv<PF>(c.mds[0]);
        std::vector<fr_t> yinv(c.rp), ums((size_t)8 * n), wms((size_t)n * 8);
        k.blk8_lambda.assign((size_t)c.rp + 1, h_one()); k.rc_partial_scaled.resize(c.rp);
        for (int q = 0; q < c.rp; ++q) {
            const fr_t l5k = h_mul(fr_pow5<PF>(k.blk8_lambda[q]), kappa);
            k.blk8_lambda[q + 1] = h_mul(l5k, a_inv); yinv[q] = fr_inv<PF>(l5k);
            k.rc_partial_scaled[q] = h_mul(k.blk8_lambda[q], c.rc_partial[q]);
        }
        k.rc_partial_scaled29.assign((size_t)(c.rp + 1) * 9, 0u);
        for (int q = 0; q < c.rp; ++q) { const fr29_t u = fr29_unpack(k.rc_partial_scaled[q]); for (int j = 0; j < 9; ++j) k.rc_partial_scaled29[(size_t)9 * q + j] = u.l[j]; }
        k.blk8_unscale29.resize(9); fr29_const_from<PF>(fr_inv<PF>(k.blk8_lambda[c.rp]), k.blk8_unscale29.data());
        for (int b = 0; b < nb; ++b) {
            for (int q = 0; q < 8; ++q) for (int j = 1; j < t; ++j) {
                um[(size_t)q * n + (j - 1)] = k.sparse[(size_t)(8 * b + q) * w + j];
                wm[(size_t)(j - 1) * 8 + q] = k.sparse[(size_t)(8 * b + q) * w + t - 1 + j];
            }
            const std::vector<int8_t> ef = mfma_frags(um.data(), 8, n, h_one()), lf = mfma_frags(wm.data(), n, 8, s20);
            k.blk8_efrag.insert(k.blk8_efrag.end(), ef.begin(), ef.end()); k.blk8_lfrag.insert(k.blk8_lfrag.end(), lf.begin(), lf.end());
            for (int q = 1; q < 8; ++q) for (int p2 = 0; p2 < q; ++p2) {
                fr_t acc = h_zero();
                for (int j = 0; j < n; ++j) acc = h_add(acc, h_mul(um[(size_t)q * n + j], wm[(size_t)j * 8 + p2]));
                g8[(size_t)b * 28 + q * (q - 1) / 2 + p2] = acc;
                k.blk8_gfrag.resize(k.blk8_gfrag.size() + 1024); mfma_frag_of(h_mul(acc, s20), &k.blk8_gfrag[k.blk8_gfrag.size() - 1024]);
                k.blk8s_gfrag.resize(k.blk8s_gfrag.size() + 1024); mfma_frag_of(h_mul(h_mul(acc, k.blk8_lambda[8 * b + q + 1]), yinv[8 * b + p2]), &k.blk8s_gfrag[k.blk8s_gfrag.size() - 1024]);
            }
            for (int q = 0; q < 8; ++q) for (int j = 0; j < n; ++j) {
                ums[(size_t)q * n + j] = h_mul(um[(size_t)q * n + j], k.blk8_lambda[8 * b + q + 1]);
                wms[(size_t)j * 8 + q] = h_mul(wm[(size_t)j * 8 + q], yinv[8 * b + q]);
            }
            const std::vector<int8_t> efs = mfma_frags(ums.data(), 8, n, h_one()), lfs = mfma_frags(wms.data(), n, 8, h_one());
            k.blk8s_efrag.insert(k.blk8s_efrag.end(), efs.begin(), efs.end()); k.blk8s_lfrag.insert(k.blk8s_lfrag.end(), lfs.begin(), lfs.end());
        }
        k.blk8_lfrag.resize(k.blk8_lfrag.size() + 1024); mfma_frag_of(h_one(), &k.blk8_lfrag[k.blk8_lfrag.size() - 1024]);
        k.gamma8_29 = to_radix29(g8, all);
    }
    if (t == 17 && c.rp == 64) {
        const int rp = c.rp, w = 2 * t - 1;
        const fr_t scale = fr_from_u64<PF>(1ull << 25);
        auto limbs = [&](const fr_t& v, uint32_t* out) { const fr29_t u = fr29_unpack(h_mul(v, scale)); for (int i = 0; i < 9; ++i) out[i] = u.l[i]; };
        k.chain_a.assign((size_t)rp * 64, 0u); k.chain_g.assign((size_t)rp * 9 * 64, 0u); k.chain_w.assign((size_t)rp * (t - 1) * 9, 0u);
        for (int q = 0; q < rp; ++q) {
            uint32_t l[9]; limbs(k.sparse[(size_t)q * w], l);
            for (int i = 0; i < 9; ++i) k.chain_a[(size_t)q * 64 + 16 + i] = l[i];
            for (int j = 1; j < t; ++j) limbs(k.sparse[(size_t)q * w + t - 1 + j], &k.chain_w[((size_t)q * (t - 1) + (j - 1)) * 9]);
        }
        for (int q = 1; q < rp; ++q)
            for (int p2 = 0; p2 < q; ++p2) {
                const fr_t* uq = &k.sparse[(size_t)q * w]; const fr_t* wp = &k.sparse[(size_t)p2 * w];
                fr_t acc = h_zero();
                for (int j = 1; j < t; ++j) acc = h_add(acc, h_mul(uq[j], wp[t - 1 + j]));
                uint32_t l[9]; limbs(acc, l);
                if (q == p2 + 1) { for (int i = 0; i < 9; ++i) k.chain_a[(size_t)p2 * 64 + 32 + i] = l[i]; }
                else for (int i = 0; i < 9; ++i) k.chain_g[((size_t)p2 * 9 + i) * 64 + q] = l[i];
            }
    }
    k.ok = true;
    return k;
}

inline void permute_dense(fr_t* s, const PoseidonConsts& c) {
    const int t = c.t, half = c.rf / 2; std::vector<fr_t> o(t);
    auto mds = [&]() { for (int i = 0; i < t; ++i) { fr_t acc = h_zero(); for (int j = 0; j < t; ++j) acc = h_add(acc, h_mul(c.mds[(size_t)i * t + j], s[j])); o[i] = acc; } for (int i = 0; i < t; ++i) s[i] = o[i]; };
    for (int r = 0; r < half; ++r) { for (int i = 0; i < t; ++i) s[i] = fr_pow5<PF>(h_add(s[i], c.rc_full[(size_t)r * t + i])); mds(); }
    for (int r = 0; r < c.rp; ++r) { s[0] = fr_pow5<PF>(h_add(s[0], c.rc_partial[r])); mds(); }
    for (int r = half; r < c.rf; ++r) { for (int i = 0; i < t; ++i) s[i] = fr_pow5<PF>(h_add(s[i], c.rc_full[(size_t)r * t + i])); mds(); }
}

}
}
```

### stark_mlwe_amd/csrc/hostcheck.cpp

```cpp
#include <algorithm>
#include <atomic>
#include <cstring>
#include <vector>
#include "fr.hpp"
#include "host_util.hpp"
#include "poseidon_dev.hpp"
#include "fri_plan.hpp"
#include "fri_verify.hpp"
#include "fri_verify_batch.hpp"
#include "mfma_digits.hpp"
#include "poseidon_chain.hpp"
#include "fri_batch.hpp"
#include "ntt_batch_plan.hpp"
#include "sumcheck_impl.hpp"
#include "mle_dev.hpp"
#include "merkle_batch.hpp"
#include "lagrange_dev.hpp"

using namespace stark;

static fr_t ld4(const uint64_t* p) { fr_t x; for (int i = 0; i < 4; ++i) { x.v[2 * i] = (uint32_t)p[i]; x.v[2 * i + 1] = (uint32_t)(p[i] >> 32); } return x; }
static void st4(uint64_t* p, const fr_t& x) { for (int i = 0; i < 4; ++i) p[i] = (uint64_t)x.v[2 * i] | ((uint64_t)x.v[2 * i + 1] << 32); }

static int g_alloc_fill = 0;
static std::vector<uint64_t> hc_block(size_t bytes) { std::vector<uint64_t> v((bytes + 7) / 8 + 1); memset(v.data(), g_alloc_fill, v.size() * sizeof(uint64_t)); return v; }
static std::vector<fr_t> hc_fr_block(size_t n) { std::vector<fr_t> v(n); if (n) memset((void*)v.data(), g_alloc_fill, n * sizeof(fr_t)); return v; }
struct HostArena {
    std::vector<std::vector<uint64_t>> mem;
    int32_t alloc(size_t bytes, void** out) { mem.push_back(hc_block(bytes)); *out = mem.back().data(); return 0; }
    int32_t upload(void* dst, const void* src, size_t bytes) { memcpy(dst, src, bytes); return 0; }
    template <class T> int32_t put(const std::vector<T>& h, T** out) {
        void* p = nullptr; alloc(std::max<size_t>(h.size(), 1) * sizeof(T), &p);
        if (!h.empty()) upload(p, h.data(), h.size() * sizeof(T));
        *out = (T*)p; return 0;
    }
    int32_t download(void* dst, const void* src, size_t bytes) { memcpy(dst, src, bytes); return 0; }
};

struct HcParams { host::PoseidonConsts ref; host::KernelConsts kc; PoseidonDev dev; };
static void bind(HcParams* P) {
    P->kc = host::make_kernel_consts(P->ref);
    P->dev.t = P->kc.t; P->dev.rf = P->kc.rf; P->dev.rp = P->kc.rp; P->dev.rc_full = P->kc.rc_full.data(); P->dev.rc_partial = P->kc.rc_partial.data();
    P->dev.lu = P->kc.lu.data(); P->dev.lu_pre = P->kc.lu_pre.data(); P->dev.row0 = P->kc.row0.data(); P->dev.sparse = P->kc.sparse.data(); P->dev.mds = P->kc.mds.data(); P->dev.mds_pre = P->kc.mds_pre.data(); P->dev.gamma = P->kc.gamma.data();
    P->dev.lu29 = P->kc.lu29.data(); P->dev.lu_pre29 = P->kc.lu_pre29.data(); P->dev.row0_29 = P->kc.row0_29.data(); P->dev.sparse29 = P->kc.sparse29.data(); P->dev.gamma29 = P->kc.gamma29.data(); P->dev.mds29 = P->kc.mds29.data(); P->dev.mds_pre29 = P->kc.mds_pre29.data(); P->dev.rc_full29 = P->kc.rc_full29.data();
    P->dev.mds_frag = nullptr; P->dev.mds_pre_frag = nullptr; P->dev.blk8_efrag = nullptr; P->dev.blk8_lfrag = nullptr; P->dev.blk8_unit_frag = nullptr; P->dev.blk8_gfrag = nullptr; P->dev.rc_partial_scaled29 = nullptr;
    P->dev.chain_a = P->kc.chain_a.empty() ? nullptr : P->kc.chain_a.data(); P->dev.chain_g = P->kc.chain_g.empty() ? nullptr : P->kc.chain_g.data(); P->dev.chain_w = P->kc.chain_w.empty() ? nullptr : P->kc.chain_w.data();
}

extern "C" {

int hc_set_alloc_fill(int byte) { if (byte < 0 || byte > 255) return -1; const int old = g_alloc_fill; g_alloc_fill = byte; return old; }
int hc_alloc_probe(size_t bytes, uint8_t* out) { const std::vector<uint64_t> v = hc_block(bytes); memcpy(out, v.data(), bytes); return 0; }

int hc_fr_op(int field, int op, const uint64_t* a, const uint64_t* b, uint64_t* out) {
    fr_t x = ld4(a), y = b ? ld4(b) : x, z;
    if (field == 0) {
        switch (op) { case 0: z = fr_add<PallasFr>(x, y); break; case 1: z = fr_sub<PallasFr>(x, y); break; case 2: z = fr_mul<PallasFr>(x, y); break; case 3: z = fr_inv<PallasFr>(x); break;
            case 4: z = fr_from_u64<PallasFr>(a[0]); break; case 5: z = fr_to_canonical<PallasFr>(x); break; case 6: z = fr_root_of_unity<PallasFr>((unsigned)a[0]); break;
            case 7: z = fr_pow_u64<PallasFr>(x, b[0]); break; case 8: z = fr_pow5_r29<PallasFr>(x); break; default: return -1; }
    } else {
        switch (op) { case 0: z = fr_add<Bls12381Fr>(x, y); break; case 1: z = fr_sub<Bls12381Fr>(x, y); break; case 2: z = fr_mul<Bls12381Fr>(x, y); break; case 3: z = fr_inv<Bls12381Fr>(x); break;
            case 4: z = fr_from_u64<Bls12381Fr>(a[0]); break; case 5: z = fr_to_canonical<Bls12381Fr>(x); break; case 6: z = fr_root_of_unity<Bls12381Fr>((unsigned)a[0]); break;
            case 7: z = fr_pow_u64<Bls12381Fr>(x, b[0]); break; case 8: z = fr_pow5_r29<Bls12381Fr>(x); break; default: return -1; }
    }
    st4(out, z); return 0;
}
int hc_wide_dot(const uint64_t* a, const uint64_t* b, size_t n, uint64_t* out) {
    DotAcc d; d.init();
    for (size_t i = 0; i < n; ++i) { uint32_t c[9]; fr29_const_from<PF>(ld4(a + 4 * i), c); d.mac(c, ld4(b + 4 * i)); }
    st4(out, d.finish()); return 0;
}
int hc_wide_dot32(const uint64_t* a, const uint64_t* b, size_t n, uint64_t* out) {
    if (n > 24) return -1;
    fr_wide w; fr_wide_zero(w);
    for (size_t i = 0; i < n; ++i) fr_wide_mac_f<PF>(w, ld4(a + 4 * i), ld4(b + 4 * i));
    st4(out, fr_wide_reduce<PF>(w)); return 0;
}
}
template <class F> static int hc_ntt29_impl(uint64_t* data, int log_b, int inverse, uint64_t* max_limb, uint64_t* max_top) {
    if (log_b < 1 || log_b > 16) return -1;
    const size_t B = (size_t)1 << log_b;
    fr_t w = fr_root_of_unity<F>((unsigned)log_b); if (inverse) w = fr_inv<F>(w);
    const fr_t k32 = fr_from_u64<F>(32);
    std::vector<fr29_t> tw(B / 2), x(B);
    { fr_t acc = k32; for (size_t i = 0; i < B / 2; ++i) { tw[i] = fr29_unpack(acc); acc = fr_mul<F>(acc, w); } }
    uint32_t D[9]; ntt29_offset<F>(D);
    auto brev = [&](size_t v) { size_t r = 0; for (int i = 0; i < log_b; ++i) r |= ((v >> i) & 1) << (log_b - 1 - i); return r; };
    for (size_t p = 0; p < B; ++p) x[brev(p)] = fr29_unpack(ld4(data + 4 * p));
    uint64_t ml = 0, mt = 0;
    const int head = log_b >= 3 ? 3 : log_b;
    {
        const fr29_t w1 = tw[log_b >= 3 ? B >> 3 : 0], w2 = tw[log_b >= 2 ? B >> 2 : 0], w3 = tw[log_b >= 3 ? 3 * (B >> 3) : 0];
        for (size_t g = 0; g < (B >> head); ++g) {
            fr29_t* xs = &x[g << head];
            if (head == 3) ntt29_head<F, 3>(*reinterpret_cast<fr29_t (*)[8]>(xs), w1, w2, w3, D);
            else if (head == 2) ntt29_head<F, 2>(*reinterpret_cast<fr29_t (*)[4]>(xs), w1, w2, w3, D);
            else ntt29_head<F, 1>(*reinterpret_cast<fr29_t (*)[2]>(xs), w1, w2, w3, D);
        }
    }
    for (int s = head + 1; s <= log_b; ++s) {
        const size_t half = (size_t)1 << (s - 1); const bool nrm = ntt29_norm_before(s);
        for (size_t bq = 0; bq < B / 2; ++bq) {
            const size_t j = bq & (half - 1), grp = bq >> (s - 1), i0 = (grp << s) + j, i1 = i0 + half;
            fr29_t a = x[i0], b = x[i1];
            { fr29_t bb = b, aa = a; if (nrm) { fr29_norm(bb); fr29_norm(aa); } for (int k = 0; k < 8; ++k) { ml = std::max<uint64_t>(ml, bb.l[k]); ml = std::max<uint64_t>(ml, aa.l[k]); } mt = std::max<uint64_t>(mt, std::max(bb.l[8], aa.l[8])); }
            ntt29_butterfly<F>(a, b, tw[j << (log_b - s)], D, nrm);
            x[i0] = a; x[i1] = b;
        }
    }
    const bool nrm_out = ntt29_norm_after(log_b);
    fr_t mult = k32; if (inverse) mult = fr_mul<F>(k32, fr_inv<F>(fr_from_u64<F>((uint64_t)B)));
    for (size_t k = 0; k < B; ++k) {
        fr29_t y = x[k];
        for (int i = 0; i < 8; ++i) ml = std::max<uint64_t>(ml, nrm_out ? 0 : y.l[i]);
        if (inverse) {
            if (nrm_out) fr29_norm(y);
            mt = std::max<uint64_t>(mt, y.l[8]);
            const fr29_t r = fr29_mul_mont<F>(fr29_unpack(mult), y);
            st4(data + 4 * k, fr29_pack_reduce<F>(r.l));
        } else {
            fr29_partial_reduce<F>(y);
            st4(data + 4 * k, fr29_pack_reduce<F>(y.l));
        }
    }
    if (max_limb) *max_limb = ml; if (max_top) *max_top = mt;
    return 0;
}
extern "C" {
int hc_partial_reduce(int field, uint32_t* limbs, size_t n) {
    for (size_t i = 0; i < n; ++i) {
        fr29_t x; for (int k = 0; k < 9; ++k) x.l[k] = limbs[9 * i + k];
        if (field == 0) fr29_partial_reduce<PallasFr>(x); else fr29_partial_reduce<Bls12381Fr>(x);
        for (int k = 0; k < 9; ++k) limbs[9 * i + k] = x.l[k];
    }
    return 0;
}
int hc_ntt29(int field, uint64_t* data, int log_b, int inverse, uint64_t* max_limb, uint64_t* max_top) {
    return field == 0 ? hc_ntt29_impl<PallasFr>(data, log_b, inverse, max_limb, max_top) : hc_ntt29_impl<Bls12381Fr>(data, log_b, inverse, max_limb, max_top);
}
int hc_blake3(const uint8_t* p, size_t n, uint8_t* out32) { host::Blake3::hash(p, n, out32); return 0; }
int hc_chacha12_u64s(const uint8_t* seed32, size_t n, uint64_t* out) { host::ChaCha12Rng r(seed32); for (size_t i = 0; i < n; ++i) out[i] = r.next_u64(); return 0; }
int hc_from_le_bytes_mod_order(const uint8_t* b, size_t n, uint64_t* out) { st4(out, host::h_from_le_bytes_mod_order(b, n)); return 0; }
int hc_to_bytes_le(const uint64_t* a, uint8_t* out32) { host::h_to_bytes_le(ld4(a), out32); return 0; }

void* hc_params_new(int kind, int t, const char* seed) {
    HcParams* P = new HcParams();
    P->ref = kind == 0 ? host::consts_for_width(t) : kind == 1 ? host::consts_transcript() : host::derive_consts(seed, 17, 8, 64);
    bind(P); return P;
}
void* hc_params_upload(int t, int rf, int rp, const uint64_t* mds, const uint64_t* rc_full, const uint64_t* rc_partial) {
    if (!mds || !rc_full || !rc_partial || t < 2 || rf <= 0 || (rf & 1) || rp <= 0) return nullptr;
    HcParams* P = new HcParams();
    P->ref.t = t; P->ref.rf = rf; P->ref.rp = rp;
    P->ref.mds.resize((size_t)t * t); P->ref.rc_full.resize((size_t)rf * t); P->ref.rc_partial.resize(rp);
    for (size_t i = 0; i < P->ref.mds.size(); ++i) P->ref.mds[i] = ld4(mds + 4 * i);
    for (size_t i = 0; i < P->ref.rc_full.size(); ++i) P->ref.rc_full[i] = ld4(rc_full + 4 * i);
    for (size_t i = 0; i < P->ref.rc_partial.size(); ++i) P->ref.rc_partial[i] = ld4(rc_partial + 4 * i);
    bind(P); return P;
}
int hc_params_ok(void* h) { return ((HcParams*)h)->kc.ok ? 1 : 0; }
void hc_params_free(void* h) { delete (HcParams*)h; }
int hc_params_export(void* h, uint64_t* mds, uint64_t* rc_full, uint64_t* rc_partial) {
    HcParams* P = (HcParams*)h;
    for (size_t i = 0; i < P->ref.mds.size(); ++i) st4(mds + 4 * i, P->ref.mds[i]);
    for (size_t i = 0; i < P->ref.rc_full.size(); ++i) st4(rc_full + 4 * i, P->ref.rc_full[i]);
    for (size_t i = 0; i < P->ref.rc_partial.size(); ++i) st4(rc_partial + 4 * i, P->ref.rc_partial[i]);
    return 0;
}
int hc_full_round_linear(void* h, int which, int pre, uint64_t* states, size_t n) {
    HcParams* P = (HcParams*)h; const int t = P->dev.t;
    if (t != 17 || P->kc.mds_frag.empty()) return -1;
    std::vector<fr_t> st(t), out(t);
    const std::vector<int8_t>& F = pre ? P->kc.mds_pre_frag : P->kc.mds_frag;
    for (size_t s = 0; s < n; ++s) {
        for (int j = 0; j < t; ++j) st[j] = ld4(states + 4 * (s * t + j));
        if (which == 0) { ArrayState a{st.data()}; apply_lu(a, pre ? P->dev.lu_pre29 : P->dev.lu29, t); out = st; }
        else {
            std::vector<fr_t> xd(t); for (int e = 0; e < t; ++e) xd[e] = recode_signed(st[e]);
            for (int i = 0; i < t; ++i) {
                int32_t S[32];
                for (int r = 0; r < 32; ++r) { int64_t acc = 0;
                    for (int e = 0; e < t; ++e) for (int kh = 0; kh < 2; ++kh) { const int8_t* a = &F[((((size_t)i * t + e) * 64) + (r + 32 * kh)) * 16];
                        const int8_t* b = reinterpret_cast<const int8_t*>(xd[e].v) + 16 * kh; for (int j = 0; j < 16; ++j) acc += (int64_t)a[j] * b[j]; }
                    if (acc > 0x7fffffffll || acc < -0x80000000ll) return -2; S[r] = (int32_t)acc; }
                int64_t col[9]; mfma_cols_of_sums(S, col);
                out[i] = mfma_finish_cols(col);
            }
        }
        for (int j = 0; j < t; ++j) st4(states + 4 * (s * t + j), out[j]);
    }
    return 0;
}
size_t hc_mfma_frag_table(void* h, int pre, int8_t* out, size_t cap) {
    HcParams* P = (HcParams*)h; const std::vector<int8_t>& F = pre ? P->kc.mds_pre_frag : P->kc.mds_frag;
    if (out) memcpy(out, F.data(), std::min(cap, F.size()));
    return F.size();
}
int hc_mfma_finish(const int32_t* sums, size_t n, uint64_t* out) {
    for (size_t s = 0; s < n; ++s) {
        const int32_t* S = sums + 32 * s;
        for (int c = 0; c < 32; ++c) if (S[c] >= (1 << 24) || S[c] <= -(1 << 24)) return -1;
        int64_t col[9]; mfma_cols_of_sums(S, col);
        st4(out + 4 * s, mfma_finish_cols(col));
    }
    return 0;
}
int hc_mfma_finish_limbs(const int32_t* sums, size_t n, uint32_t* out) {
    for (size_t s = 0; s < n; ++s) {
        const int32_t* S = sums + 32 * s;
        for (int c = 0; c < 32; ++c) if (S[c] >= (1 << 24) || S[c] <= -(1 << 24)) return -1;
        int64_t col[9]; mfma_cols_of_sums(S, col);
        mfma_finish_limbs(col, out + 9 * s);
    }
    return 0;
}
int hc_sbox_lazy29(const uint32_t* l, const uint32_t* c, size_t n, uint64_t* out, uint64_t* colmax) {
    for (size_t s = 0; s < n; ++s) {
        const uint32_t* ls = l + 9 * s; const uint32_t* cs = c + 9 * s;
        for (int i = 0; i < 9; ++i) if (ls[i] >= (i < 8 ? 1u << 29 : 1u << 24) || cs[i] >= (i < 8 ? 1u << 29 : 1u << 23)) return -1;
        const fr_t z = sbox_lazy29(ls, cs);
        Lazy29Wide wide; const fr29_t x5 = wide.pow5(ls, cs);
        const fr_t zw = fr29_pack_reduce<PF>(x5.l);
        if (colmax) { colmax[2 * s] = (uint64_t)wide.max_col; colmax[2 * s + 1] = (uint64_t)(wide.max_col >> 64); }
        if ((wide.max_col >> 64) == 0 && memcmp(&z, &zw, sizeof(fr_t)) != 0) return -2;
        st4(out + 4 * s, z);
    }
    return 0;
}
static int blk8_tile_sums(const int8_t* const* frag, const fr_t* xd, int K, int32_t* S) {
    for (int r = 0; r < 32; ++r) { int64_t acc = 0;
        for (int k = 0; k < K; ++k) for (int kh = 0; kh < 2; ++kh) { const int8_t* a = frag[k] + (size_t)(r + 32 * kh) * 16;
            const int8_t* b = reinterpret_cast<const int8_t*>(xd[k].v) + 16 * kh; for (int j = 0; j < 16; ++j) acc += (int64_t)a[j] * b[j]; }
        if (acc >= (1 << 24) || acc <= -(1 << 24)) return -2; S[r] = (int32_t)acc; }
    return 0;
}
static fr_t blk8_finish_sums(const int32_t* S) { int64_t col[9]; mfma_cols_of_sums(S, col); return mfma_finish_cols(col); }
static void blk8_finish_sums_limbs(const int32_t* S, uint32_t* l, const uint32_t* c29 = nullptr) { int64_t col[8]; mfma_word_cols_mad_of_sums(S, col, c29); mfma_finish_words(col, l); }
static int blk8_tile(const int8_t* const* frag, const fr_t* xd, int K, fr_t& out) { int32_t S[32]; const int rc = blk8_tile_sums(frag, xd, K, S); if (rc) return rc; out = blk8_finish_sums(S); return 0; }
static std::atomic<int32_t> g_blk8_row23_max{0};
int32_t hc_blk8_row23_max(int reset) { return reset ? g_blk8_row23_max.exchange(0) : g_blk8_row23_max.load(); }
int hc_permute_block8(void* h, uint64_t* states, size_t n) {
    HcParams* P = (HcParams*)h; const host::KernelConsts& k = P->kc; const int t = k.t, half = k.rf / 2;
    if (t != 17 || k.blk8s_efrag.empty() || k.blk8s_gfrag.empty() || k.blk8_unscale29.empty() || k.mds_frag.empty()) return -1;
    const int8_t* unit = k.blk8_lfrag.data() + k.blk8_lfrag.size() - 1024;
    std::vector<fr_t> st(t), xd(t), o(t);
    auto sbox = [&](int r) { for (int j = 0; j < t; ++j) xd[j] = recode_signed(fr_pow5_r29<PF>(fr_add<PF>(st[j], k.rc_full[(size_t)r * t + j]))); };
    auto product = [&](const std::vector<int8_t>& F, int next) -> int {
        for (int i = 0; i < t; ++i) {
            const int8_t* fr[17]; for (int e = 0; e < t; ++e) fr[e] = &F[((size_t)i * t + e) * 1024];
            int32_t S[32]; const int rc = blk8_tile_sums(fr, xd.data(), t, S); if (rc) return rc;
            if (next < 0) { int64_t col[8]; mfma_word_cols_mad_of_sums(S, col); o[i] = mfma_finish_words_canonical(col); }
            else { uint32_t l[9]; blk8_finish_sums_limbs(S, l); o[i] = sbox_lazy29_recoded(l, &k.rc_full29[((size_t)next * t + i) * 9]); }
        }
        if (next < 0) st = o; else xd = o;
        return 0; };
    for (size_t s = 0; s < n; ++s) {
        for (int j = 0; j < t; ++j) st[j] = ld4(states + 4 * (s * t + j));
        sbox(0);
        for (int r = 0; r < half; ++r) { const int rc = product(r == half - 1 ? k.mds_pre_frag : k.mds_frag, r == half - 1 ? -1 : r + 1); if (rc) return rc; }
        fr_t rec[17], yd[9], kx[23];
        fr29_t u = lazy29_add_c29(fr29_unpack(st[0]).l, &k.rc_partial_scaled29[0]);
        for (int j = 1; j < t; ++j) rec[j] = recode_signed(st[j]);
        const int nb = k.rp / 8;
        for (int b = 0; b < nb; ++b) {
            const int8_t* ef = k.blk8s_efrag.data() + (size_t)b * 8 * 16 * 1024; const int8_t* lf = k.blk8s_lfrag.data() + (size_t)b * 16 * 8 * 1024;
            const int8_t* gf = k.blk8s_gfrag.data() + (size_t)b * 28 * 1024;
            for (int j = 0; j < 16; ++j) kx[j] = rec[1 + j];
            for (int q = 0; q < 8; ++q) {
                const int8_t* fr[23]; for (int j = 0; j < 16; ++j) fr[j] = ef + ((size_t)q * 16 + j) * 1024;
                for (int p2 = 0; p2 < q; ++p2) { fr[16 + p2] = gf + ((size_t)q * (q - 1) / 2 + p2) * 1024; kx[16 + p2] = yd[p2]; }
                int32_t S[32]; { const int rc = blk8_tile_sums(fr, kx, 16 + q, S); if (rc) return rc; }
                if (q == 7) { int32_t m = 0; for (int c = 0; c < 32; ++c) m = std::max(m, S[c] < 0 ? -S[c] : S[c]);
                              int32_t seen = g_blk8_row23_max.load(); while (m > seen && !g_blk8_row23_max.compare_exchange_weak(seen, m)) {} }
                uint32_t l[9]; blk8_finish_sums_limbs(S, l, &k.rc_partial_scaled29[(size_t)9 * (8 * b + q + 1)]);
                const fr_t slot = lazy29_to_slot(l);
                const fr29_t x5 = pow5_lazy29(u);
                yd[q] = recode_lazy29(x5);
                u = lazy29_add_slot(x5, slot);
                for (int i = 0; i < 9; ++i) if (u.l[i] >= (1u << 30)) return -4;
            }
            for (int j = 1; j < t; ++j) {
                const int8_t* fr[9]; for (int p2 = 0; p2 < 8; ++p2) fr[p2] = lf + ((size_t)(j - 1) * 8 + p2) * 1024; fr[8] = unit;
                yd[8] = rec[j];
                if (b == nb - 1) {
                    int32_t S[32]; { const int rc = blk8_tile_sums(fr, yd, 9, S); if (rc) return rc; }
                    uint32_t l[9]; blk8_finish_sums_limbs(S, l); xd[j] = sbox_lazy29_recoded(l, &k.rc_full29[((size_t)half * t + j) * 9]);
                } else { int32_t S[32]; { const int rc = blk8_tile_sums(fr, yd, 9, S); if (rc) return rc; } int64_t col[8]; mfma_word_cols_of_sums(S, col); rec[j] = mfma_finish_bytes(col); }
            }
        }
        const fr29_t x0 = fr29_mul_c29(k.blk8_unscale29.data(), u);
        xd[0] = sbox_lazy29_recoded(x0.l, &k.rc_full29[((size_t)half * t) * 9]);
        for (int r = half; r < k.rf; ++r) { const int rc = product(k.mds_frag, r == k.rf - 1 ? -1 : r + 1); if (rc) return rc; }
        for (int j = 0; j < t; ++j) st4(states + 4 * (s * t + j), st[j]);
    }
    return 0;
}
int hc_mfma_finish_limbs_c(const int32_t* sums, const uint32_t* c, size_t n, uint32_t* limbs, uint32_t* slots) {
    for (size_t s = 0; s < n; ++s) {
        const int32_t* S = sums + 32 * s; const uint32_t* cs = c + 9 * s;
        for (int i = 0; i < 32; ++i) if (S[i] >= (1 << 24) || S[i] <= -(1 << 24)) return -1;
        for (int i = 0; i < 9; ++i) if (cs[i] >= (i < 8 ? 1u << 29 : 1u << 23)) return -1;
        int64_t col[9]; mfma_cols_of_sums(S, col, cs);
        mfma_finish_limbs(col, limbs + 9 * s);
        const fr_t z = lazy29_to_slot(limbs + 9 * s);
        memcpy(slots + 8 * s, z.v, 32);
    }
    return 0;
}
void hc_lazy29_add_slot(const uint32_t* x5, const uint32_t* slots, size_t n, uint32_t* u) {
    for (size_t s = 0; s < n; ++s) { fr29_t a; fr_t z; memcpy(a.l, x5 + 9 * s, 36); memcpy(z.v, slots + 8 * s, 32); const fr29_t r = lazy29_add_slot(a, z); memcpy(u + 9 * s, r.l, 36); }
}
void hc_recode_lazy29(const uint32_t* x5, size_t n, int8_t* digits) {
    for (size_t s = 0; s < n; ++s) { fr29_t a; memcpy(a.l, x5 + 9 * s, 36); const fr_t d = recode_lazy29(a); memcpy(digits + 32 * s, d.v, 32); }
}
int hc_chain_census(const uint32_t* u, size_t n, uint32_t* x245, uint64_t* colmax, uint8_t* topbyte) {
    static const uint32_t zero9[9] = {0, 0, 0, 0, 0, 0, 0, 0, 0};
    for (size_t s = 0; s < n; ++s) {
        fr29_t a; memcpy(a.l, u + 9 * s, 36);
        for (int i = 0; i < 9; ++i) if (a.l[i] >= (1u << 30)) return -1;
        Lazy29Wide wide; const fr29_t x5w = wide.pow5(a.l, zero9);
        const fr29_t x5 = pow5_lazy29(a);
        colmax[2 * s] = (uint64_t)wide.max_col; colmax[2 * s + 1] = (uint64_t)(wide.max_col >> 64);
        if ((wide.max_col >> 64) == 0 && memcmp(x5.l, x5w.l, 36) != 0) return -2;
        memcpy(x245 + 27 * s, wide.x2.l, 36); memcpy(x245 + 27 * s + 9, wide.x4.l, 36); memcpy(x245 + 27 * s + 18, x5w.l, 36);
        topbyte[s] = (uint8_t)(fr29_pack(x5w.l).v[7] >> 24);
    }
    return 0;
}
int hc_mfma_finish_recoded(const int32_t* sums, size_t n, uint32_t* limbs, int8_t* digits) {
    for (size_t s = 0; s < n; ++s) {
        const int32_t* S = sums + 32 * s;
        for (int i = 0; i < 32; ++i) if (S[i] >= (1 << 24) || S[i] <= -(1 << 24)) return -1;
        int64_t col[9]; mfma_cols_of_sums(S, col); mfma_finish_limbs_floor(col, limbs + 9 * s);
        mfma_cols_of_sums(S, col); const fr_t d = mfma_finish_recoded(col); memcpy(digits + 32 * s, d.v, 32);
    }
    return 0;
}
int hc_mfma_finish_bytes(const int32_t* sums, size_t n, int wide, int64_t* cols, int32_t* qh, int64_t* carry, int8_t* digits) {
    const int32_t lim = (wide ? 17 : 9) * 32 * 128 * 128;
    for (size_t s = 0; s < n; ++s) {
        const int32_t* S = sums + 32 * s;
        for (int i = 0; i < 32; ++i) if (S[i] > lim || S[i] < -lim) return -1;
        int64_t* col = cols + 8 * s;
        if (wide) mfma_word_cols_of_sums<true>(S, col); else mfma_word_cols_of_sums<false>(S, col);
        const fr_t d = mfma_finish_bytes(col, qh + s, carry + s); memcpy(digits + 32 * s, d.v, 32);
    }
    return 0;
}
int hc_mfma_finish_words(const int32_t* sums, const uint32_t* c, size_t n, int64_t* cols, int32_t* qh, int64_t* carry, uint32_t* limbs, uint64_t* canon) {
    const int32_t lim = 23 * 32 * 128 * 128;
    for (size_t s = 0; s < n; ++s) {
        const int32_t* S = sums + 32 * s; const uint32_t* cs = c ? c + 9 * s : nullptr;
        for (int i = 0; i < 32; ++i) if (S[i] > lim || S[i] < -lim) return -1;
        if (cs) for (int i = 0; i < 9; ++i) if (cs[i] >= (i < 8 ? 1u << 29 : 1u << 23)) return -1;
        int64_t* col = cols + 8 * s;
        mfma_word_cols_mad_of_sums(S, col, cs);
        mfma_finish_words(col, limbs + 9 * s, qh + s, carry + s);
        if (canon) st4(canon + 4 * s, mfma_finish_words_canonical(col));
    }
    return 0;
}
size_t hc_rc_partial_scaled29_table(void* h, uint32_t* out, size_t cap) {
    const std::vector<uint32_t>& v = ((HcParams*)h)->kc.rc_partial_scaled29;
    if (out && !v.empty()) memcpy(out, v.data(), std::min(cap, v.size()) * 4);
    return v.size();
}
size_t hc_blk8_table(void* h, int which, void* out, size_t cap) {
    HcParams* P = (HcParams*)h; const host::KernelConsts& k = P->kc;
    if (which >= 4) {
        std::vector<uint8_t> lam;
        if (which == 8 && !k.blk8_lambda.empty()) { lam.resize(k.blk8_lambda.size() * sizeof(fr_t) + k.blk8_unscale29.size() * 4);
            memcpy(lam.data(), k.blk8_lambda.data(), k.blk8_lambda.size() * sizeof(fr_t)); memcpy(lam.data() + k.blk8_lambda.size() * sizeof(fr_t), k.blk8_unscale29.data(), k.blk8_unscale29.size() * 4); }
        const void* src = which == 4 ? (const void*)k.blk8s_efrag.data() : which == 5 ? (const void*)k.blk8s_lfrag.data() : which == 6 ? (const void*)k.blk8s_gfrag.data() : which == 7 ? (const void*)k.rc_partial_scaled.data() : (const void*)lam.data();
        const size_t len = which == 4 ? k.blk8s_efrag.size() : which == 5 ? k.blk8s_lfrag.size() : which == 6 ? k.blk8s_gfrag.size() : which == 7 ? k.rc_partial_scaled.size() * sizeof(fr_t) : which == 8 ? lam.size() : 0;
        if (out && len) memcpy(out, src, std::min(cap, len));
        return len;
    }
    const void* src = which == 0 ? (const void*)k.blk8_efrag.data() : which == 1 ? (const void*)k.blk8_lfrag.data() : which == 3 ? (const void*)k.blk8_gfrag.data() : (const void*)k.gamma8_29.data();
    const size_t len = which == 0 ? k.blk8_efrag.size() : which == 1 ? k.blk8_lfrag.size() : which == 3 ? k.blk8_gfrag.size() : k.gamma8_29.size() * 4;
    if (out && len) memcpy(out, src, std::min(cap, len));
    return len;
}
size_t hc_rc_full29_table(void* h, uint32_t* out, size_t cap) {
    const std::vector<uint32_t>& v = ((HcParams*)h)->kc.rc_full29;
    if (out && !v.empty()) memcpy(out, v.data(), std::min(cap, v.size()) * 4);
    return v.size();
}
int hc_blk8_finish_with_base(void* h, const int32_t* sums, const uint64_t* bases, size_t n, uint64_t* out) {
    HcParams* P = (HcParams*)h; if (P->kc.blk8_lfrag.empty()) return -3;
    const int8_t* unit = P->kc.blk8_lfrag.data() + P->kc.blk8_lfrag.size() - 1024;
    for (size_t s = 0; s < n; ++s) {
        const fr_t bd = recode_signed(ld4(bases + 4 * s)); int32_t U[32], S[32];
        if (blk8_tile_sums(&unit, &bd, 1, U)) return -1;
        for (int c = 0; c < 32; ++c) { const int64_t v = (int64_t)sums[32 * s + c] + U[c]; if (v >= (1 << 24) || v <= -(1 << 24)) return -1; S[c] = (int32_t)v; }
        st4(out + 4 * s, blk8_finish_sums(S));
    }
    return 0;
}
int hc_permute_kernel_form(void* h, uint64_t* states, size_t n) {
    HcParams* P = (HcParams*)h; int t = P->dev.t; std::vector<fr_t> st(t);
    for (size_t i = 0; i < n; ++i) { for (int j = 0; j < t; ++j) st[j] = ld4(states + 4 * (i * t + j)); ArrayState s{st.data()}; permute_core(s, P->dev, false); for (int j = 0; j < t; ++j) st4(states + 4 * (i * t + j), st[j]); }
    return 0;
}
int hc_permute_chain_model(void* h, uint64_t* states, size_t n) {
    HcParams* P = (HcParams*)h; const int t = P->ref.t, half = P->ref.rf / 2; if (!P->dev.chain_a) return -1;
    std::vector<fr_t> st(t), o(t);
    auto dense = [&](const std::vector<fr_t>& M) { for (int i = 0; i < t; ++i) { fr_t acc = host::h_zero(); for (int j = 0; j < t; ++j) acc = host::h_add(acc, host::h_mul(M[(size_t)i * t + j], st[j])); o[i] = acc; } st = o; };
    for (size_t i = 0; i < n; ++i) {
        for (int j = 0; j < t; ++j) st[j] = ld4(states + 4 * (i * t + j));
        for (int r = 0; r < half; ++r) { for (int j = 0; j < t; ++j) st[j] = fr_pow5<PallasFr>(host::h_add(st[j], P->ref.rc_full[(size_t)r * t + j])); dense(r == half - 1 ? P->kc.mds_pre : P->kc.mds); }
        chain_partial_model(st.data(), P->dev);
        for (int r = half; r < P->ref.rf; ++r) { for (int j = 0; j < t; ++j) st[j] = fr_pow5<PallasFr>(host::h_add(st[j], P->ref.rc_full[(size_t)r * t + j])); dense(P->kc.mds); }
        for (int j = 0; j < t; ++j) st4(states + 4 * (i * t + j), st[j]);
    }
    return 0;
}
int hc_row_consts(uint32_t* out14) { const RowConstsHost K = row_consts_host(); for (int i = 0; i < 9; ++i) out14[i] = K.ni[i]; for (int i = 0; i < 5; ++i) out14[9 + i] = K.t[i]; return 0; }
size_t hc_chain_table(void* h, int which, uint32_t* out, size_t cap) {
    HcParams* P = (HcParams*)h; const std::vector<uint32_t>& v = which == 0 ? P->kc.chain_a : which == 1 ? P->kc.chain_g : P->kc.chain_w;
    if (out) for (size_t i = 0; i < v.size() && i < cap; ++i) out[i] = v[i];
    return v.size();
}
int hc_permute_dense(void* h, uint64_t* states, size_t n) {
    HcParams* P = (HcParams*)h; int t = P->ref.t; std::vector<fr_t> st(t);
    for (size_t i = 0; i < n; ++i) { for (int j = 0; j < t; ++j) st[j] = ld4(states + 4 * (i * t + j)); host::permute_dense(st.data(), P->ref); for (int j = 0; j < t; ++j) st4(states + 4 * (i * t + j), st[j]); }
    return 0;
}
}
static void leaf_init(fr_t init[17]) {
    const fr_t AB = host::h_tag("FSv1-ABSORB-BYTES"), CH = host::h_tag("FSv1-CHALLENGE");
    for (int j = 0; j < 17; ++j) init[j] = host::h_zero();
    init[0] = AB; init[1] = host::h_words("FRI/leaf/poseidon")[0]; init[2] = AB; init[3] = host::h_words("FRI/leaf")[0];
    init[6] = CH; init[7] = AB; init[8] = host::h_words("leaf")[0]; init[16] = host::h_tag("FSv1-TRANSCRIPT-INIT");
}
extern "C" {
int hc_leaf_pair(void* tparams, const uint64_t* f, const uint64_t* f_next, size_t n, size_t m, uint64_t* hout) {
    HcParams* P = (HcParams*)tparams;
    fr_t init[17]; leaf_init(init);
    std::vector<fr_t> fv(n), nv(f_next ? (n + m - 1) / m : 0);
    for (size_t i = 0; i < fv.size(); ++i) fv[i] = ld4(f + 4 * i);
    for (size_t i = 0; i < nv.size(); ++i) nv[i] = ld4(f_next + 4 * i);
    const LeafStream L{init, fv.data(), f_next ? nv.data() : nullptr, m, n};
    fr_t st[17];
    for (size_t i = 0; i < n; ++i) { ArrayState s{st}; st4(hout + 4 * i, leaf_pair_body(s, P->dev, L, i)); }
    return 0;
}
int hc_hash_ds_level(void* params, int mode, size_t arity, uint32_t level, uint64_t pos0, uint64_t label, const uint64_t* in0, const uint64_t* in1, size_t n_in, uint64_t* out) {
    HcParams* P = (HcParams*)params;
    std::vector<fr_t> a(n_in), b(in1 ? n_in : 0), st(P->dev.t);
    for (size_t i = 0; i < n_in; ++i) { a[i] = ld4(in0 + 4 * i); if (in1) b[i] = ld4(in1 + 4 * i); }
    const DsStream D = DsStream::make(mode, arity, level, pos0, label, a.data(), in1 ? b.data() : nullptr, n_in);
    for (size_t k = 0; k < D.n_out; ++k) { ArrayState s{st.data()}; st4(out + 4 * k, hash_ds_body(s, P->dev, D, k)); }
    return 0;
}
int hc_tr_hash(void* tparams, const char* tag, const uint64_t* fields, size_t k, size_t n, uint64_t* out) {
    HcParams* P = (HcParams*)tparams;
    std::vector<fr_t> fr; const int np = host::tr_hash_frame(tag, fr);
    std::vector<fr_t> fl(n * k); for (size_t i = 0; i < n * k; ++i) fl[i] = ld4(fields + 4 * i);
    const TrStream T = TrStream::equal(fr.data(), np, (int)fr.size() - np, fl.data(), k, n, host::h_tag("FSv1-TRANSCRIPT-INIT"));
    fr_t st[17];
    for (size_t i = 0; i < n; ++i) { ArrayState s{st}; st4(out + 4 * i, tr_hash_body(s, P->dev, T, i)); }
    return 0;
}
int hc_tr_frame_dims(const char* tag, int* np, int* ns) { std::vector<fr_t> fr; *np = host::tr_hash_frame(tag, fr); *ns = (int)fr.size() - *np; return 0; }
int hc_tr_hash_many(void* tparams, size_t n, const char* const* tags, const uint64_t* const* fields, const size_t* k, uint64_t* out, size_t* launch_order) {
    HcParams* P = (HcParams*)tparams;
    std::vector<std::vector<fr_t>> frames(n), fl(n); std::vector<TrFrameRef> fr(n); std::vector<const fr_t*> fp(n, nullptr);
    for (size_t i = 0; i < n; ++i) {
        const int np = host::tr_hash_frame(tags[i], frames[i]); fr[i] = TrFrameRef{frames[i].data(), np, (int)frames[i].size() - np};
        if (!k[i]) continue;
        if (!fields || !fields[i]) return -1;
        fl[i].resize(k[i]); for (size_t q = 0; q < k[i]; ++q) fl[i][q] = ld4(fields[i] + 4 * q);
        fp[i] = fl[i].data();
    }
    const std::vector<TrStream::Item> items = tr_ragged_items(fr.data(), fp.data(), k, n);
    const TrStream T = tr_ragged_stream(items.data(), n, host::h_tag("FSv1-TRANSCRIPT-INIT"));
    fr_t st[17];
    for (size_t j = 0; j < n; ++j) {
        ArrayState s{st}; size_t slot = n; const fr_t d = tr_hash_body<true>(s, P->dev, T, j, &slot);
        if (slot >= n) return -2;
        st4(out + 4 * slot, d); if (launch_order) launch_order[j] = slot;
    }
    return 0;
}
size_t hc_mixed_prove_groups(size_t B, const size_t* n0, const size_t* schedule, const size_t* sched_off, const size_t* r, size_t* group_of, size_t* order) {
    const std::vector<std::vector<size_t>> G = mixed_prove_groups(B, n0, schedule, sched_off, r);
    size_t pos = 0;
    for (size_t g = 0; g < G.size(); ++g) for (size_t i : G[g]) { group_of[i] = g; order[pos++] = i; }
    return G.size();
}
int hc_hash_stream(void* params, int mode, const uint64_t* a, size_t na, const uint64_t* b, size_t nb, const uint64_t* tag, size_t n, uint64_t* out) {
    HcParams* P = (HcParams*)params;
    std::vector<fr_t> av(n * na), bv(n * nb), st(P->dev.t);
    for (size_t i = 0; i < n * na; ++i) av[i] = ld4(a + 4 * i); for (size_t i = 0; i < n * nb; ++i) bv[i] = ld4(b + 4 * i);
    for (size_t k = 0; k < n; ++k) { ArrayState s{st.data()}; st4(out + 4 * k, hash_stream_body(s, P->dev, mode, av.data(), na, bv.data(), nb, tag ? ld4(tag) : host::h_zero(), k)); }
    return 0;
}

struct HcHasher : TrHasher {
    void* tp; explicit HcHasher(void* p) : tp(p) {}
    int32_t hash(const char* tag, const fr_t* fields, size_t k, size_t n, fr_t* out) override {
        std::vector<uint64_t> in(4 * k * n), o(4 * n);
        for (size_t i = 0; i < k * n; ++i) st4(in.data() + 4 * i, fields[i]);
        int rc = hc_tr_hash(tp, tag, in.data(), k, n, o.data()); if (rc) return rc;
        for (size_t i = 0; i < n; ++i) out[i] = ld4(o.data() + 4 * i);
        return 0;
    }
};
struct HcPlan { FriPlan plan; void* tp; };
void* hc_fri_plan_create(void* tparams, const uint64_t* roots, size_t n0, const size_t* schedule, size_t L, size_t r) {
    std::vector<fr_t> rt(L + 1); for (size_t l = 0; l <= L; ++l) rt[l] = ld4(roots + 4 * l);
    HcPlan* P = new HcPlan(); P->tp = tparams; P->plan.r = r; std::string err;
    if (!P->plan.shape.make(n0, schedule, L, rt.data(), err)) { delete P; return nullptr; }
    HcHasher H(tparams); if (fri_plan_make(P->plan, H)) { delete P; return nullptr; }
    return P;
}
size_t hc_fri_plan_num_requests(void* p) { return ((HcPlan*)p)->plan.req.size(); }
int hc_fri_plan_requests(void* p, uint32_t* kind, uint32_t* which, uint32_t* level, uint64_t* index) {
    auto& rq = ((HcPlan*)p)->plan.req;
    for (size_t i = 0; i < rq.size(); ++i) { kind[i] = rq[i].kind; which[i] = rq[i].which; level[i] = rq[i].level; index[i] = rq[i].index; }
    return 0;
}
size_t hc_fri_plan_assemble(void* p, const uint64_t* values, size_t n_values, uint8_t* buf, size_t cap, size_t* est) {
    HcPlan* P = (HcPlan*)p; if (n_values != P->plan.req.size()) return 0;
    std::vector<fr_t> v(n_values); for (size_t i = 0; i < n_values; ++i) v[i] = ld4(values + 4 * i);
    ReplaySource src(v.data(), v.size()); HcHasher H(P->tp); std::vector<uint8_t> b; size_t e = 0;
    if (assemble_proof(P->plan.shape, P->plan.r, H, src, b, e) || src.pos != v.size()) return 0;
    if (est) *est = e;
    if (buf && cap >= b.size()) memcpy(buf, b.data(), b.size());
    return b.size();
}
void hc_fri_plan_free(void* p) { delete (HcPlan*)p; }

struct HcParamCache {
    std::map<int, HcParams*> mp;
    ~HcParamCache() { for (auto& kv : mp) delete kv.second; }
    HcParams* params(size_t arity) { int t = host::width_for_arity(arity); auto it = mp.find(t); if (it != mp.end()) return it->second; HcParams* P = new HcParams(); P->ref = host::consts_for_width(t); bind(P); mp[t] = P; return P; }
};
static HcParamCache& hc_param_cache() { static HcParamCache c; return c; }
static void run_plan_host(VerifyBatchPlan V, const HcParams* tparams, int32_t* accepted) {
    { std::vector<fr_t> dev = hc_fr_block(V.pool.size()); std::copy(V.pool.begin(), V.pool.begin() + V.n_known, dev.begin()); V.pool.swap(dev); }
    if (V.nl) {
        fr_t init[17]; leaf_init(init);
        const LeafStream LS{init, V.pool.data() + V.leaf_f0, V.pool.data() + V.leaf_f0 + V.nl, 1, V.nl};
        fr_t st[17]; for (size_t j = 0; j < V.nl; ++j) { ArrayState s{st}; V.pool[V.leaf_out0 + j] = leaf_pair_body(s, tparams->dev, LS, j); }
    }
    for (const VerifyBatchPlan::Group& G : V.groups) {
        HcParams* P = hc_param_cache().params((size_t)G.t - 1); std::vector<fr_t> st(P->dev.t);
        const DsGatherStream D{V.hdr.data() + 4 * G.job0, V.off.data() + G.job0, V.idx.data(), V.pool.data(), G.n, G.max_children};
        for (size_t k = 0; k < D.n_out; ++k) { ArrayState s{st.data()}; V.pool[G.out0 + k] = hash_ds_body(s, P->dev, D, k); }
    }
    for (size_t b = 0; b < V.batch; ++b) {
        int32_t acc = V.flag[b];
        for (uint32_t j = V.chk_off[b]; j < V.chk_off[b + 1]; ++j) acc &= fr_eq(V.pool[V.chk[2 * j]], V.pool[V.chk[2 * j + 1]]) ? 1 : 0;
        accepted[b] = acc;
    }
}
int hc_deep_fri_verify_batch(void* tparams, size_t batch, const uint8_t* const* proofs, const size_t* lens, const size_t* schedule, size_t L, size_t r, int32_t* accepted) {
    VerifyBatchPlanner pl; for (size_t b = 0; b < batch; ++b) pl.add(proofs[b], lens[b], schedule, L, r);
    if (!pl.fits_u32()) return -1;
    VerifyBatchPlan V; pl.finish(V);
    run_plan_host(std::move(V), (const HcParams*)tparams, accepted);
    return 0;
}
int hc_deep_fri_verify(void* tparams, const uint8_t* bytes, size_t len, const size_t* schedule, size_t L, size_t r) {
    int32_t acc = 0; const int rc = hc_deep_fri_verify_batch(tparams, 1, &bytes, &len, schedule, L, r, &acc);
    return rc ? rc : acc;
}
size_t hc_verify_batch_groups(size_t batch, const uint8_t* const* proofs, const size_t* lens, const size_t* schedule, size_t L, size_t r, int32_t* t, uint32_t* depth, size_t* n, size_t cap) {
    VerifyBatchPlanner pl; for (size_t b = 0; b < batch; ++b) pl.add(proofs[b], lens[b], schedule, L, r);
    VerifyBatchPlan V; pl.finish(V);
    for (size_t g = 0; g < V.groups.size() && g < cap; ++g) { t[g] = V.groups[g].t; depth[g] = V.groups[g].depth; n[g] = V.groups[g].n; }
    return V.groups.size();
}
int hc_merkle_verify(void* tparams, int pairs, size_t cfg_arity, uint64_t label, const uint64_t* root, const size_t* idx, size_t k, const uint64_t* vals, const uint64_t* cp, const uint8_t* proof, size_t len) {
    (void)tparams;
    const uint64_t none[4] = {0, 0, 0, 0};
    MerkleVerifyPlanner pl; pl.add(cfg_arity, label, root, idx, k, vals, pairs ? (cp ? cp : none) : nullptr, proof, len);
    if (!pl.fits_u32()) return -1;
    VerifyBatchPlan V; pl.finish(V);
    int32_t acc = 0; run_plan_host(std::move(V), nullptr, &acc);
    return acc;
}

}

struct ScHostExec : HostArena {
    HcParams* cp; HcParams* tp;
    ScHostExec(HcParams* c, HcParams* t) : cp(c), tp(t) {}
    int32_t ds_level(const DsBatchStream& D, fr_t* out) {
        std::vector<fr_t> st(cp->dev.t);
        for (size_t k = 0; k < D.n_out; ++k) { ArrayState s{st.data()}; out[k] = hash_ds_body(s, cp->dev, D, k); }
        return 0;
    }
    int32_t ragged_level(const DsRaggedStream& D, fr_t* out) {
        std::vector<fr_t> st(cp->dev.t);
        for (size_t k = 0; k < D.n_out; ++k) { ArrayState s{st.data()}; out[k] = hash_ds_body(s, cp->dev, D, k); }
        return 0;
    }
    int32_t coeffs(const fr_t* const* ptrs, const fr_t* layers, size_t len, size_t B, fr_t* c01, fr_t* claim, size_t claim_from) {
        for (size_t b = 0; b < B; ++b) {
            const fr_t* l = ptrs ? ptrs[b] : layers + b * len; fr_t c0 = fr_zero<PF>(), c1 = fr_zero<PF>();
            for (size_t j = 0; j < len / 2; ++j) { c0 = fr_add<PF>(c0, l[2 * j]); c1 = fr_add<PF>(c1, fr_sub<PF>(l[2 * j + 1], l[2 * j])); }
            c01[2 * b] = c0; c01[2 * b + 1] = c1; if (claim && b >= claim_from) claim[b] = fr_add<PF>(fr_add<PF>(c0, c0), c1);
        }
        return 0;
    }
    int32_t fold(const fr_t* const* ptrs, const fr_t* layers, size_t len, size_t B, const fr_t* r, fr_t* next) {
        for (size_t b = 0; b < B; ++b) {
            const fr_t* l = ptrs ? ptrs[b] : layers + b * len;
            for (size_t j = 0; j < len / 2; ++j) next[b * (len / 2) + j] = fr_add<PF>(l[2 * j], fr_mul<PF>(r[b], fr_sub<PF>(l[2 * j + 1], l[2 * j])));
        }
        return 0;
    }
    int32_t transcript(const TrBatchStream& T) { fr_t st[17]; for (size_t a = 0; a < T.n_active; ++a) { ArrayState s{st}; tr_batch_body(s, tp->dev, T, a); } return 0; }
    int32_t gather(const fr_t* const* addr, size_t n, fr_t* out) { for (size_t j = 0; j < n; ++j) out[j] = *addr[j]; return 0; }
};
extern "C" {
int hc_hash_ds_batch_level(void* params, size_t arity, uint32_t level, uint64_t pos0, const uint64_t* labels, const uint64_t* in, size_t n_in, size_t trees, int by_ptrs, uint64_t* out) {
    HcParams* P = (HcParams*)params;
    std::vector<fr_t> a(n_in * trees), st(P->dev.t); for (size_t i = 0; i < a.size(); ++i) a[i] = ld4(in + 4 * i);
    std::vector<const fr_t*> ptrs(trees); for (size_t b = 0; b < trees; ++b) ptrs[b] = a.data() + b * n_in;
    const DsBatchStream D = DsBatchStream::make(arity, level, pos0, labels, by_ptrs ? ptrs.data() : nullptr, by_ptrs ? nullptr : a.data(), n_in, trees);
    for (size_t k = 0; k < D.n_out; ++k) { ArrayState s{st.data()}; st4(out + 4 * k, hash_ds_body(s, P->dev, D, k)); }
    return 0;
}
int hc_tr_batch(void* tparams, uint64_t* state, uint32_t* pos, size_t n_inst, const uint32_t* inst, size_t inst0, size_t n_active, size_t nseg, const uint32_t* el_off,
                const uint32_t* idx, const uint64_t* pool0, size_t n0, const uint64_t* pool1, size_t n1, int reset, int finish_last, uint64_t* out) {
    HcParams* P = (HcParams*)tparams;
    std::vector<fr_t> st(17 * n_inst), p0(n0), p1(n1), o(n_active * nseg, host::h_zero());
    for (size_t i = 0; i < st.size(); ++i) st[i] = ld4(state + 4 * i);
    for (size_t i = 0; i < n0; ++i) p0[i] = ld4(pool0 + 4 * i); for (size_t i = 0; i < n1; ++i) p1[i] = ld4(pool1 + 4 * i);
    TrBatchStream T; T.state = st.data(); T.pos = pos; T.inst = inst; T.inst0 = inst0; T.n_active = n_active; T.nseg = nseg; T.el_off = el_off; T.idx = idx;
    T.pool0 = p0.data(); T.pool1 = p1.data(); T.out = o.data(); T.init_cap = host::h_tag("FSv1-TRANSCRIPT-INIT"); T.reset_from = reset ? 0 : n_active; T.finish_last = finish_last;
    fr_t s17[17]; for (size_t a = 0; a < n_active; ++a) { ArrayState s{s17}; tr_batch_body(s, P->dev, T, a); }
    for (size_t i = 0; i < st.size(); ++i) st4(state + 4 * i, st[i]);
    for (size_t i = 0; i < o.size(); ++i) st4(out + 4 * i, o[i]);
    return 0;
}
size_t hc_sumcheck_prove_batch(void* tparams, void* cparams, int mf, size_t B, const uint64_t* const* witnesses, size_t k, const uint64_t* labels, size_t q,
                               uint8_t* buf, size_t cap, size_t* lens) {
    const size_t n = (size_t)1 << k;
    std::vector<std::vector<fr_t>> w(B, std::vector<fr_t>(n)); std::vector<const fr_t*> wp(B);
    for (size_t b = 0; b < B; ++b) { for (size_t i = 0; i < n; ++i) w[b][i] = ld4(witnesses[b] + 4 * i); wp[b] = w[b].data(); }
    ScHostExec X((HcParams*)cparams, (HcParams*)tparams);
    const std::vector<size_t> ks(B, k);
    ScBatch<ScHostExec> S(X, B, wp.data(), ks.data(), labels);
    std::vector<std::vector<uint8_t>> pr;
    if (mf ? S.prove_mf(q, pr) : S.prove_plain(pr)) return 0;
    size_t tot = 0; for (size_t b = 0; b < B; ++b) { lens[b] = pr[b].size(); tot += pr[b].size(); }
    if (buf && cap >= tot) { size_t o = 0; for (auto& p : pr) { memcpy(buf + o, p.data(), p.size()); o += p.size(); } }
    return tot;
}
size_t hc_sumcheck_prove_mixed_batch(void* tparams, void* cparams, int mf, size_t B, const uint64_t* const* witnesses, const size_t* k, const uint64_t* labels, size_t q,
                                     uint8_t* buf, size_t cap, size_t* lens) {
    std::vector<std::vector<fr_t>> w(B); std::vector<const fr_t*> wp(B);
    for (size_t b = 0; b < B; ++b) {
        if (k[b] > 40) return 0;
        const size_t n = (size_t)1 << k[b]; w[b].resize(n);
        for (size_t i = 0; i < n; ++i) w[b][i] = ld4(witnesses[b] + 4 * i);
        wp[b] = w[b].data();
    }
    ScHostExec X((HcParams*)cparams, (HcParams*)tparams);
    ScBatch<ScHostExec> S(X, B, wp.data(), k, labels);
    std::vector<std::vector<uint8_t>> pr;
    if (mf ? S.prove_mf(q, pr) : S.prove_plain(pr)) return 0;
    size_t tot = 0; for (size_t b = 0; b < B; ++b) { lens[b] = pr[b].size(); tot += pr[b].size(); }
    if (buf && cap >= tot) { size_t o = 0; for (auto& p : pr) { memcpy(buf + o, p.data(), p.size()); o += p.size(); } }
    return tot;
}
}

static int sc_verify_plan(int mf, size_t batch, const uint8_t* const* proofs, const size_t* lens, const uint64_t* labels, ScVerifyPlan& V) {
    bool fits = false;
    if (sc_verify_plan_some(mf, 0, batch, proofs, lens, labels, (size_t)-1, V, fits) != batch || !fits) return -1;
    return 0;
}
extern "C" {
int hc_sc_decode_fr(const uint8_t* blob, size_t len, size_t off, uint64_t* out4) {
    if (off + 32 > len) return -1;
    std::vector<uint32_t> w((len + 3) / 4 + 2, 0u); memcpy(w.data(), blob, len);
    fr_t x; const bool ok = sc_decode_fr(w.data(), (uint32_t)off, 0u, x); st4(out4, x); return ok ? 1 : 0;
}
static void run_sc_plan_host(ScVerifyPlan& V, HcParams* tp, HcParams* cp, int32_t* accepted) {
    const int mf = V.mf;
    std::vector<fr_t> pool = hc_fr_block(std::max<size_t>(V.pool_slots, 1));
    for (size_t j = 0; j < V.n_dec; ++j) if (!sc_decode_fr(V.blob.data(), V.dec_off[j], V.dec_proof[j], pool[j])) V.flag[V.dec_proof[j] & ~kScClaim] = 0;
    std::vector<fr_t> state = hc_fr_block(17 * std::max<size_t>(V.n_inst, 1)); std::vector<uint32_t> pos(std::max<size_t>(V.n_inst, 1), 0x01010101u * (uint32_t)g_alloc_fill);
    for (const ScVerifyPlan::Stream& S : V.tr) {
        TrBatchStream T; T.state = state.data(); T.pos = pos.data(); T.inst = nullptr; T.inst0 = S.inst0; T.n_active = S.n; T.nseg = S.nseg; T.el_off = V.tr_off.data() + S.seg0;
        T.idx = V.tr_idx.data(); T.pool0 = pool.data(); T.pool1 = V.consts.data(); T.out = pool.data() + V.n_dec + S.seg0; T.init_cap = host::h_tag("FSv1-TRANSCRIPT-INIT"); T.reset_from = 0; T.finish_last = 1;
        fr_t st[17]; for (size_t a = 0; a < S.n; ++a) { ArrayState s{st}; tr_batch_body(s, tp->dev, T, a); }
    }
    for (const VerifyBatchPlan::Group& G : V.ds.groups) {
        std::vector<fr_t> st(cp->dev.t);
        const DsGatherStream D{V.ds.hdr.data() + 4 * G.job0, V.ds.off.data() + G.job0, V.ds.idx.data(), pool.data(), G.n, G.max_children};
        for (size_t k = 0; k < D.n_out; ++k) { ArrayState s{st.data()}; pool[G.out0 + k] = hash_ds_body(s, cp->dev, D, k); }
    }
    for (size_t j = 0; j < V.n_rec(); ++j) {
        const uint32_t* r = V.rec.data() + 8 * j;
        if (!(mf ? sc_check_mf(pool.data(), r) : sc_check_plain(pool.data(), r))) V.flag[mf ? r[1] : r[0]] = 0;
    }
    for (size_t b = 0; b < V.batch; ++b) accepted[b] = V.flag[b];
}
int hc_sumcheck_verify_batch(void* tparams, void* cparams, int mf, size_t batch, const uint8_t* const* proofs, const size_t* lens, const uint64_t* labels, int32_t* accepted) {
    ScVerifyPlan V; if (sc_verify_plan(mf, batch, proofs, lens, labels, V)) return -1;
    run_sc_plan_host(V, (HcParams*)tparams, (HcParams*)cparams, accepted);
    return 0;
}
int hc_sumcheck_verify_batch_slots(void* tparams, void* cparams, int mf, size_t batch, const uint8_t* const* proofs, const size_t* lens, const uint64_t* labels, size_t max_slots, int32_t* accepted) {
    size_t b0 = 0;
    while (b0 < batch) {
        ScVerifyPlan V; bool fits = false;
        const size_t b1 = sc_verify_plan_some(mf, b0, batch, proofs, lens, labels, max_slots, V, fits);
        if (!fits) return -1;
        run_sc_plan_host(V, (HcParams*)tparams, (HcParams*)cparams, accepted + b0);
        b0 = b1;
    }
    return 0;
}
size_t hc_sumcheck_verify_batch_steps(int mf, size_t batch, const uint8_t* const* proofs, const size_t* lens, const uint64_t* labels, int32_t* kind, size_t* count, size_t cap) {
    ScVerifyPlan V; if (sc_verify_plan(mf, batch, proofs, lens, labels, V)) return 0;
    const auto st = V.steps();
    for (size_t i = 0; i < st.size() && i < cap; ++i) { kind[i] = st[i].first; count[i] = st[i].second; }
    return st.size();
}
}

struct FriHostExec : HostArena {
    HcParams* tp;
    HcParamCache& mp;
    explicit FriHostExec(HcParams* t) : tp(t), mp(hc_param_cache()) {}
    int32_t zpows(const fr_t& z, size_t m, fr_t* zp) { fr_t acc = fr_one<PF>(); for (size_t t = 0; t < m; ++t) { zp[t] = acc; acc = fr_mul<PF>(acc, z); } return 0; }
    int32_t fold(const fr_t* f, size_t n, const fr_t* zp, size_t m, fr_t* out) {
        for (size_t b = 0; b < n / m; ++b) { fr_t acc = fr_zero<PF>(); for (size_t t = 0; t < m; ++t) acc = fr_add<PF>(acc, fr_mul<PF>(f[b * m + t], zp[t])); out[b] = acc; }
        return 0;
    }
    int32_t leaf_pairs(const fr_t* f, const fr_t* f_next, size_t n, size_t m, fr_t* h) {
// ... 344 lines not shown
```

### stark_mlwe_amd/csrc/poseidon_pair.hpp

```cpp
#pragma once
#include "fr.hpp"
#include "dev_common.hpp"
#include "poseidon_params.hpp"
#include "poseidon_dev.hpp"
#include "poseidon_streams.hpp"
#include "mfma_digits.hpp"

#if defined(__HIPCC__)
namespace stark {

template <int T> struct PairCfg {
#ifndef STARK_NXD17
#define STARK_NXD17 5
#endif
    static constexpr int NXD = T == 17 ? STARK_NXD17 : 2;
#ifndef STARK_NXU17
#define STARK_NXU17 8
#endif
    static constexpr int NXU = T == 17 ? STARK_NXU17 : (T - 1) / 2;
    static constexpr int NX = (T - 1) / 2;
    static constexpr int EXTRA = 3;
    __host__ __device__ static constexpr int xslot(int p) { return p == 0 ? 0 : T + (p - 1); }
    __host__ __device__ static constexpr int dslot(int q) { return 1 + (q % NXD); }
    __host__ __device__ static constexpr size_t lds_bytes() { return (size_t)(T + EXTRA) * 2 * 64 * 16; }
};
static inline size_t pair_lds_bytes(int t) { return t == 17 ? PairCfg<17>::lds_bytes() : PairCfg<9>::lds_bytes(); }

struct PairState {
    uint4* st;
    int lane; bool isY;
    __device__ __forceinline__ fr_t ld(int j) const {
        uint4 lo = st[(2 * j) * 64 + lane], hi = st[(2 * j + 1) * 64 + lane];
        fr_t x; x.v[0] = lo.x; x.v[1] = lo.y; x.v[2] = lo.z; x.v[3] = lo.w; x.v[4] = hi.x; x.v[5] = hi.y; x.v[6] = hi.z; x.v[7] = hi.w; return x;
    }
    __device__ __forceinline__ void sto(int j, const fr_t& x) const {
        st[(2 * j) * 64 + lane] = make_uint4(x.v[0], x.v[1], x.v[2], x.v[3]);
        st[(2 * j + 1) * 64 + lane] = make_uint4(x.v[4], x.v[5], x.v[6], x.v[7]);
    }
};

template <int T>
__device__ __forceinline__ void pair_apply_lu(const PairState& s, const uint32_t* lu) {
    const int yo = s.isY ? 1 : 0;
#pragma unroll 1
    for (int k = 0; 2 * k < T; ++k) {
        const int i = 2 * k + yo; const bool have = i < T;
        fr_t res;
        if (have) { DotAcc w; w.init(); _Pragma("unroll 1") for (int j = i; j < T; ++j) w.mac(c29(lu, i * T + j), s.ld(j)); res = w.finish(); }
        __syncthreads();
        if (have) s.sto(i, res);
    }
    __syncthreads();
#pragma unroll 1
    for (int k = 0; T - 1 - 2 * k >= 1; ++k) {
        const int i = T - 1 - 2 * k - yo; const bool have = i >= 1;
        fr_t res;
        if (have) { DotAcc w; w.init(); _Pragma("unroll 1") for (int j = 0; j < i; ++j) w.mac(c29(lu, i * T + j), s.ld(j)); res = fr_add<PF>(s.ld(i), w.finish()); }
        __syncthreads();
        if (have) s.sto(i, res);
    }
    __syncthreads();
}
template <int T, bool RECODE = false>
__device__ __forceinline__ void pair_sbox_full(const PairState& s, const fr_t* rc) {
    const int j0 = s.isY ? PairCfg<T>::NX : 0, j1 = s.isY ? T : PairCfg<T>::NX;
    for (int j = j0; j < j1; ++j) { const fr_t x = fr_pow5_r29<PF>(fr_add<PF>(s.ld(j), rc[j])); s.sto(j, RECODE ? recode_signed(x) : x); }
    __syncthreads();
}

typedef int mfma_v4i __attribute__((ext_vector_type(4)));
typedef int mfma_v16i __attribute__((ext_vector_type(16)));
__device__ __forceinline__ void mfma_zero_tile(mfma_v16i (&acc)[2]) {
#pragma unroll
    for (int ct = 0; ct < 2; ++ct)
#pragma unroll
        for (int r = 0; r < 16; ++r) acc[ct][r] = 0;
}
__device__ __forceinline__ void mfma_post_cols(const mfma_v16i (&acc)[2], int64_t* col, const uint32_t* c29 = nullptr) {
    mfma_v16i lo, hi;
#pragma unroll
    for (int r = 0; r < 16; ++r) {
        const auto sw = __builtin_amdgcn_permlane32_swap((unsigned)acc[0][r], (unsigned)acc[1][r], false, false);
        lo[r] = (int)sw[0]; hi[r] = (int)sw[1];
    }
    if (c29) mfma_cols_set(col, c29);
    else {
#pragma unroll
        for (int k = 0; k < 9; ++k) col[k] = 0;
    }
    mfma_fold_rows(col, lo, hi);
}
__device__ __forceinline__ fr_t mfma_post(const mfma_v16i (&acc)[2]) {
    int64_t col[9];
    mfma_post_cols(acc, col);
    return mfma_finish_cols(col);
}
__device__ __forceinline__ fr_t mfma_post_bytes(const mfma_v16i (&acc)[2]) {
    int64_t c0[4], c1[4], col[8];
    mfma_word_cols(acc[0], c0); mfma_word_cols(acc[1], c1);
#pragma unroll
    for (int q = 0; q < 4; ++q) {
        const auto lo = __builtin_amdgcn_permlane32_swap((unsigned)(uint64_t)c0[q], (unsigned)(uint64_t)c1[q], false, false);
        const auto hi = __builtin_amdgcn_permlane32_swap((unsigned)((uint64_t)c0[q] >> 32), (unsigned)((uint64_t)c1[q] >> 32), false, false);
        col[2 * q] = (int64_t)((uint64_t)lo[0] | ((uint64_t)hi[0] << 32)); col[2 * q + 1] = (int64_t)((uint64_t)lo[1] | ((uint64_t)hi[1] << 32));
    }
    return mfma_finish_bytes(col);
}
__device__ __forceinline__ void mfma_post_words(const mfma_v16i (&acc)[2], int64_t* col, const uint32_t* c29 = nullptr) {
    int64_t c0[4], c1[4];
    mfma_word_cols_mad(acc[0], c0); mfma_word_cols_mad(acc[1], c1);
#pragma unroll
    for (int q = 0; q < 4; ++q) {
        const auto lo = __builtin_amdgcn_permlane32_swap((unsigned)(uint64_t)c0[q], (unsigned)(uint64_t)c1[q], false, false);
        const auto hi = __builtin_amdgcn_permlane32_swap((unsigned)((uint64_t)c0[q] >> 32), (unsigned)((uint64_t)c1[q] >> 32), false, false);
        col[2 * q] = (int64_t)((uint64_t)lo[0] | ((uint64_t)hi[0] << 32)); col[2 * q + 1] = (int64_t)((uint64_t)lo[1] | ((uint64_t)hi[1] << 32));
    }
    if (c29) mfma_words_add_c29(col, c29);
}
__device__ __forceinline__ void mfma_post_limbs(const mfma_v16i (&acc)[2], uint32_t* l, const uint32_t* c29 = nullptr) {
    int64_t col[8];
    mfma_post_words(acc, col, c29);
    mfma_finish_words(col, l);
}
__device__ __forceinline__ void pair_sto_sbox29(const PairState& s, int j, const uint32_t* l, const uint32_t* rc29, bool recode) {
    const fr29_t x5 = pow5_lazy29(lazy29_add_c29(l, rc29));
    s.sto(j, recode ? recode_lazy29(x5) : fr29_pack_reduce<PF>(x5.l));
}
__device__ __forceinline__ void pair_mds_sbox_mfma(const PairState& s, const void* frag, const uint32_t* rc29, bool recode) {
    constexpr int T = 17;
    const int lane = s.lane, h = lane >> 5;
    mfma_v4i b[T][2];
#pragma unroll
    for (int e = 0; e < T; ++e)
#pragma unroll
        for (int ct = 0; ct < 2; ++ct) { const uint4 u = s.st[(2 * e + h) * 64 + 32 * ct + (lane & 31)]; b[e][ct] = mfma_v4i{(int)u.x, (int)u.y, (int)u.z, (int)u.w}; }
    __syncthreads();
    const mfma_v4i* A = reinterpret_cast<const mfma_v4i*>(frag) + lane;
#pragma unroll 1
    for (int i = s.isY ? 1 : 0; i < T; i += 2) {
        mfma_v16i acc[2];
        mfma_zero_tile(acc);
        const mfma_v4i* Ai = A + (size_t)i * T * 64;
#pragma unroll
        for (int e = 0; e < T; ++e) {
            const mfma_v4i a = Ai[(size_t)e * 64];
#pragma unroll
            for (int ct = 0; ct < 2; ++ct) acc[ct] = __builtin_amdgcn_mfma_i32_32x32x32_i8(a, b[e][ct], acc[ct], 0, 0, 0);
        }
        int64_t col[8];
        mfma_post_words(acc, col);
        if (rc29) { uint32_t l[9]; mfma_finish_words(col, l); pair_sto_sbox29(s, i, l, c29(rc29, i), recode); }
        else s.sto(i, mfma_finish_words_canonical(col));
    }
    __syncthreads();
}

struct Blk8Tabs {
    const mfma_v4i* efrag;
    const mfma_v4i* lfrag;
    const mfma_v4i* unit;
    const mfma_v4i* gfrag;
    const uint32_t* rc29;
};
struct Blk8Cfg {
    static constexpr int NLX = 8;
    __host__ __device__ static constexpr int ymail(int q) { return 17 + (q & 1); }
    __host__ __device__ static constexpr int hmail(int q) { return (q & 1) ? 19 : 0; }
};
__device__ __forceinline__ void blk8_load_frags16(mfma_v4i (&a)[16], const mfma_v4i* A, int lane) {
#pragma unroll
    for (int e = 0; e < 16; ++e) a[e] = (A + (size_t)e * 64)[lane];
}
__device__ __forceinline__ mfma_v4i blk8_b_of_slot(const PairState& s, int j, int ct) {
    const uint4 u = s.st[(2 * j + (s.lane >> 5)) * 64 + 32 * ct + (s.lane & 31)];
    return mfma_v4i{(int)u.x, (int)u.y, (int)u.z, (int)u.w};
}
template <int Q>
__device__ __forceinline__ void blk8_round_x(const PairState& s, const Blk8Tabs& Tb, fr29_t& u, mfma_v4i (&b)[8][2]) {
    __builtin_amdgcn_sched_barrier(0);
    const fr29_t x5 = pow5_lazy29(u);
    s.sto(Blk8Cfg::ymail(Q), recode_lazy29(x5));
    __syncthreads();
    u = lazy29_add_slot(x5, s.ld(Blk8Cfg::hmail(Q)));
    b[Q][0] = blk8_b_of_slot(s, Blk8Cfg::ymail(Q), 0); b[Q][1] = blk8_b_of_slot(s, Blk8Cfg::ymail(Q), 1);
}
template <int Q>
__device__ __forceinline__ void blk8_round_y(const PairState& s, const Blk8Tabs& Tb, mfma_v4i (&b)[8][2], mfma_v4i (&a)[16], mfma_v4i (&g)[7]) {
    __builtin_amdgcn_sched_barrier(0);
    const int lane = s.lane;
    mfma_v16i acc[2];
    mfma_zero_tile(acc);
#pragma unroll
    for (int e = 0; e < 16; ++e)
#pragma unroll
        for (int ct = 0; ct < 2; ++ct) acc[ct] = __builtin_amdgcn_mfma_i32_32x32x32_i8(a[e], blk8_b_of_slot(s, e + 1, ct), acc[ct], 0, 0, 0);
    if constexpr (Q > 0) {
#pragma unroll
        for (int p = 0; p < Q; ++p)
#pragma unroll
            for (int ct = 0; ct < 2; ++ct) acc[ct] = __builtin_amdgcn_mfma_i32_32x32x32_i8(g[p], b[p][ct], acc[ct], 0, 0, 0);
    }
    if constexpr (Q < 7) {
        blk8_load_frags16(a, Tb.efrag + (size_t)(Q + 1) * 16 * 64, lane);
#pragma unroll
        for (int p = 0; p <= Q; ++p) g[p] = (Tb.gfrag + (size_t)((Q + 1) * Q / 2 + p) * 64)[lane];
    }
    { uint32_t l[9]; mfma_post_limbs(acc, l, c29(Tb.rc29, Q)); s.sto(Blk8Cfg::hmail(Q), lazy29_to_slot(l)); }
    __syncthreads();
    b[Q][0] = blk8_b_of_slot(s, Blk8Cfg::ymail(Q), 0); b[Q][1] = blk8_b_of_slot(s, Blk8Cfg::ymail(Q), 1);
}
template <int NLX, bool LAZY = false>
__device__ __forceinline__ void blk8_lane_rows(const PairState& s, const Blk8Tabs& Tb, const mfma_v4i (&b)[8][2], bool last, const uint32_t* rc29_next = nullptr, bool recode_next = true) {
    static_assert(NLX >= 1 && NLX <= 15, "shares");
    const int lane = s.lane;
    const int j0 = s.isY ? NLX + 1 : 1, j1 = s.isY ? 16 : NLX;
    const mfma_v4i aunit = Tb.unit[lane];
    mfma_v4i a[8];
#pragma unroll
    for (int p = 0; p < 8; ++p) a[p] = (Tb.lfrag + ((size_t)(j0 - 1) * 8 + p) * 64)[lane];
#pragma unroll 1
    for (int j = j0; j <= j1; ++j) {
        mfma_v16i acc[2];
        mfma_zero_tile(acc);
#pragma unroll
        for (int p = 0; p < 8; ++p)
#pragma unroll
            for (int ct = 0; ct < 2; ++ct) acc[ct] = __builtin_amdgcn_mfma_i32_32x32x32_i8(a[p], b[p][ct], acc[ct], 0, 0, 0);
#pragma unroll
        for (int ct = 0; ct < 2; ++ct) acc[ct] = __builtin_amdgcn_mfma_i32_32x32x32_i8(aunit, blk8_b_of_slot(s, j, ct), acc[ct], 0, 0, 0);
        const int jn = j < j1 ? j + 1 : j1;
#pragma unroll
        for (int p = 0; p < 8; ++p) a[p] = (Tb.lfrag + ((size_t)(jn - 1) * 8 + p) * 64)[lane];
        if (rc29_next) { uint32_t l[9]; mfma_post_limbs(acc, l); pair_sto_sbox29(s, j, l, c29(rc29_next, j), recode_next); }
        else if (LAZY && !last) s.sto(j, mfma_post_bytes(acc));
        else { const fr_t z = mfma_post(acc); s.sto(j, last ? z : recode_signed(z)); }
    }
    __syncthreads();
}
template <int NLX, bool LAZY = false>
__device__ __forceinline__ void pair_block8(const PairState& s, const Blk8Tabs& Tb, fr29_t& u, bool last, const uint32_t* rc29_next = nullptr, bool recode_next = true,
                                            const uint32_t* unscale29 = nullptr) {
    mfma_v4i b[8][2];
    if (!s.isY) {
        blk8_round_x<0>(s, Tb, u, b); blk8_round_x<1>(s, Tb, u, b); blk8_round_x<2>(s, Tb, u, b); blk8_round_x<3>(s, Tb, u, b);
        blk8_round_x<4>(s, Tb, u, b); blk8_round_x<5>(s, Tb, u, b); blk8_round_x<6>(s, Tb, u, b); blk8_round_x<7>(s, Tb, u, b);
    } else {
        mfma_v4i a[16], g[7];
        blk8_load_frags16(a, Tb.efrag, s.lane);
        blk8_round_y<0>(s, Tb, b, a, g); blk8_round_y<1>(s, Tb, b, a, g); blk8_round_y<2>(s, Tb, b, a, g); blk8_round_y<3>(s, Tb, b, a, g);
        blk8_round_y<4>(s, Tb, b, a, g); blk8_round_y<5>(s, Tb, b, a, g); blk8_round_y<6>(s, Tb, b, a, g); blk8_round_y<7>(s, Tb, b, a, g);
    }
    __builtin_amdgcn_sched_barrier(0);
    if (rc29_next && !s.isY) { const fr29_t x = fr29_mul_c29(unscale29, u); pair_sto_sbox29(s, 0, x.l, c29(rc29_next, 0), recode_next); }
    blk8_lane_rows<NLX, LAZY>(s, Tb, b, last, rc29_next, recode_next);
}

template <int T>
__device__ __forceinline__ fr_t pair_lane_update(const uint32_t* sp, int j, const fr_t& base, const fr29_t& x0, const fr29_t& x1, const fr29_t& x2, const fr29_t& x3) {
    constexpr int W = 2 * T - 1;
    fr_wide29 u; fr_wide29_zero(u);
    fr_wide29_mac(u, c29(sp, 0 * W + T - 1 + j), x0); fr_wide29_mac(u, c29(sp, 1 * W + T - 1 + j), x1);
    fr_wide29_mac(u, c29(sp, 2 * W + T - 1 + j), x2); fr_wide29_mac(u, c29(sp, 3 * W + T - 1 + j), x3);
    return fr_add<PF>(base, fr_wide29_reduce_lazy<PF>(u));
}

template <int T, bool BLK8 = false, bool FUSE = BLK8>
__device__ __forceinline__ fr_t pair_permute(const PairState& s, const PoseidonDev& P, bool only0, int r_begin = 0) {
    static_assert(!BLK8 || T == 17, "8-round blocks exist for t = 17");
    static_assert(!FUSE || BLK8, "the fused hand-over belongs to the 8-round form");
    typedef PairCfg<T> Cfg;
    constexpr int NXD = Cfg::NXD, NXU = Cfg::NXU, W = 2 * T - 1;
    const int half = P.rf / 2;
    if constexpr (FUSE) {
        if (r_begin < half) pair_sbox_full<T, true>(s, P.rc_full + r_begin * T);
        for (int r = r_begin; r < half; ++r)
            pair_mds_sbox_mfma(s, (r == half - 1) ? P.mds_pre_frag : P.mds_frag, (r == half - 1) ? nullptr : c29(P.rc_full29, (size_t)(r + 1) * T), true);
    } else
    for (int r = r_begin; r < half; ++r) {
        if constexpr (T == 17) { pair_sbox_full<T, true>(s, P.rc_full + r * T); pair_mds_sbox_mfma(s, (r == half - 1) ? P.mds_pre_frag : P.mds_frag, nullptr, true); }
        else { pair_sbox_full<T>(s, P.rc_full + r * T); pair_apply_lu<T>(s, (r == half - 1) ? P.lu_pre29 : P.lu29); }
    }
    fr_t s0 = fr_zero<PF>();
    if (!s.isY) s0 = s.ld(0);
    if constexpr (BLK8) {
        fr29_t u = fr29_unpack(s0);
        if (!s.isY) u = lazy29_add_c29(u.l, c29(P.rc_partial_scaled29, 0));
        for (int j = s.isY ? 9 : 1; j <= (s.isY ? 16 : 8); ++j) s.sto(j, recode_signed(s.ld(j)));
        __syncthreads();
        const int nb = P.rp / 8;
#pragma unroll 1
        for (int b = 0; b < nb; ++b) {
            const Blk8Tabs Tb{reinterpret_cast<const mfma_v4i*>(P.blk8_efrag) + (size_t)b * 8 * 16 * 64, reinterpret_cast<const mfma_v4i*>(P.blk8_lfrag) + (size_t)b * 16 * 8 * 64,
                              reinterpret_cast<const mfma_v4i*>(P.blk8_unit_frag), reinterpret_cast<const mfma_v4i*>(P.blk8_gfrag) + (size_t)b * 28 * 64,
                              c29(P.rc_partial_scaled29, (size_t)8 * b + 1)};
            if constexpr (FUSE) pair_block8<Blk8Cfg::NLX, true>(s, Tb, u, b == nb - 1, b == nb - 1 ? c29(P.rc_full29, (size_t)half * T) : nullptr, !(only0 && half == P.rf - 1), P.blk8_unscale29());
            else pair_block8<Blk8Cfg::NLX>(s, Tb, u, b == nb - 1);
        }
        if constexpr (!FUSE) { if (!s.isY) s0 = fr29_pack_reduce<PF>(fr29_mul_c29(P.blk8_unscale29(), u).l); }
    } else
    for (int b = 0; b < P.rp / 4; ++b) {
        const uint32_t* sp = c29(P.sparse29, (size_t)(4 * b) * W);
        const uint32_t* g = c29(P.gamma29, (size_t)b * 6);
        if (!s.isY) {
            fr_t keep[NXD];
#pragma unroll
            for (int j = 0; j < NXD; ++j) keep[j] = s.ld(1 + j);
            __syncthreads();
#define STARK_PAIR_ROUND(q)                                                                           \
            {                                                                                         \
                __builtin_amdgcn_sched_barrier(0);                      \
                const fr_t xq = fr_pow5_r29<PF>(fr_add<PF>(s0, P.rc_partial[4 * b + q]));              \
                s.sto(Cfg::xslot(q), xq);                                                             \
                fr_wide29 acc; fr_wide29_zero(acc);                                                   \
                fr_wide29_mac(acc, c29(sp, q * W), fr29_unpack(xq));                                  \
                if (q > 0) fr_wide29_mac(acc, c29(g, q * (q - 1) / 2 + 0), fr29_unpack(s.ld(Cfg::xslot(0)))); \
                if (q > 1) fr_wide29_mac(acc, c29(g, q * (q - 1) / 2 + 1), fr29_unpack(s.ld(Cfg::xslot(1)))); \
                if (q > 2) fr_wide29_mac(acc, c29(g, q * (q - 1) / 2 + 2), fr29_unpack(s.ld(Cfg::xslot(2)))); \
                if (1 + q + NXD > fr29_max_terms<PF>()) fr_wide29_norm(acc);    \
                _Pragma("unroll") for (int j = 0; j < NXD; ++j) fr_wide29_mac(acc, c29(sp, q * W + 1 + j), fr29_unpack(keep[j])); \
                const fr_t part = fr_wide29_reduce<PF>(acc);                                          \
                __syncthreads();                                        \
                s0 = fr_add<PF>(part, s.ld(Cfg::dslot(q)));                                           \
            }
            STARK_PAIR_ROUND(0) STARK_PAIR_ROUND(1) STARK_PAIR_ROUND(2) STARK_PAIR_ROUND(3)
#undef STARK_PAIR_ROUND
            const fr29_t x0 = fr29_unpack(s.ld(Cfg::xslot(0))), x1 = fr29_unpack(s.ld(Cfg::xslot(1))), x2 = fr29_unpack(s.ld(Cfg::xslot(2))), x3 = fr29_unpack(s.ld(Cfg::xslot(3)));
#pragma unroll
            for (int j = 1; j <= NXD; ++j) { __builtin_amdgcn_sched_barrier(0); s.sto(j, pair_lane_update<T>(sp, j, keep[j - 1], x0, x1, x2, x3)); }
#pragma unroll 1
            for (int j = NXD + 1; j <= NXU; ++j) s.sto(j, pair_lane_update<T>(sp, j, s.ld(j), x0, x1, x2, x3));
        } else {
            __syncthreads();
            for (int q = 0; q < 4; ++q) {
                DotAcc acc; acc.init();
#pragma unroll 1
                for (int j = NXD + 1; j < T; ++j) acc.mac(c29(sp, q * W + j), s.ld(j));
                const fr_t dy = acc.finish();
                s.sto(Cfg::dslot(q), dy);
                __syncthreads();
            }
            const fr29_t x0 = fr29_unpack(s.ld(Cfg::xslot(0))), x1 = fr29_unpack(s.ld(Cfg::xslot(1))), x2 = fr29_unpack(s.ld(Cfg::xslot(2))), x3 = fr29_unpack(s.ld(Cfg::xslot(3)));
#pragma unroll 1
            for (int j = NXU + 1; j < T; ++j) s.sto(j, pair_lane_update<T>(sp, j, s.ld(j), x0, x1, x2, x3));
        }
        __syncthreads();
    }
    if constexpr (!FUSE) {
        if (!s.isY) s.sto(0, s0);
        __syncthreads();
    }
    for (int r = half; r < P.rf; ++r) {
        const bool squeeze = only0 && r == P.rf - 1;
        if constexpr (FUSE) {  }
        else if constexpr (T == 17) { if (squeeze) pair_sbox_full<T>(s, P.rc_full + r * T); else pair_sbox_full<T, true>(s, P.rc_full + r * T); }
        else pair_sbox_full<T>(s, P.rc_full + r * T);
        if (squeeze) {
            const int j0 = s.isY ? Cfg::NX : 0, j1 = s.isY ? T : Cfg::NX;
            DotAcc acc; acc.init();
#pragma unroll 1
            for (int j = j0; j < j1; ++j) acc.mac(c29(P.row0_29, j), s.ld(j));
            s.sto(T + (s.isY ? 1 : 0), acc.finish());
            __syncthreads();
            fr_t out = fr_add<PF>(s.ld(T + 0), s.ld(T + 1));
            __syncthreads();
            return out;
        }
        if constexpr (FUSE) pair_mds_sbox_mfma(s, P.mds_frag, r == P.rf - 1 ? nullptr : c29(P.rc_full29, (size_t)(r + 1) * T), !(only0 && r + 1 == P.rf - 1));
        else if constexpr (T == 17) pair_mds_sbox_mfma(s, P.mds_frag, nullptr, true); else pair_apply_lu<T>(s, P.lu29);
    }
    return s.ld(0);
}

__device__ __forceinline__ PairState pair_setup(uint4* lds) {
    PairState s; s.st = lds; s.lane = threadIdx.x & 63;
    s.isY = __builtin_amdgcn_readfirstlane((int)(threadIdx.x >> 6)) != 0;
    return s;
}

template <bool BLK8>
__global__ void __launch_bounds__(128) __attribute__((amdgpu_waves_per_eu(2))) k_leaf_pair2(PoseidonDev P, const fr_t* __restrict__ leafc, const fr_t* __restrict__ f,
                                                    const fr_t* __restrict__ f_next, size_t n, size_t m, fr_t* __restrict__ h) {
    extern __shared__ uint4 lds[];
    PairState s = pair_setup(lds);
    const size_t i = (size_t)blockIdx.x * 64 + s.lane; const bool live = i < n; const size_t ii = live ? i : n - 1;
    const fr_t x4 = fr_pow5_r29<PF>(fr_add<PF>(ldg(f + ii), P.rc_full[4]));
    const fr_t x5 = fr_pow5_r29<PF>(fr_add<PF>(f_next ? ldg(f_next + ii / m) : fr_zero<PF>(), P.rc_full[5]));
    const int j0 = s.isY ? PairCfg<17>::NX : 0, j1 = s.isY ? 17 : PairCfg<17>::NX;
    const uint32_t* m45 = reinterpret_cast<const uint32_t*>(leafc + 51);
    const fr29_t x4u = fr29_unpack(x4), x5u = fr29_unpack(x5);
    for (int j = j0; j < j1; ++j) {
        fr_wide29 w; fr_wide29_zero(w);
        fr_wide29_mac(w, c29(m45, j), x4u); fr_wide29_mac(w, c29(m45, 17 + j), x5u);
        s.sto(j, fr_add<PF>(leafc[j], fr_wide29_reduce<PF>(w)));
    }
    __syncthreads();
    fr_t out = pair_permute<17, BLK8>(s, P, true, 1);
    if (live && !s.isY) stg(h + i, out);
}

template <int T, class DS, bool BLK8 = false>
__global__ void __launch_bounds__(128) __attribute__((amdgpu_waves_per_eu(2))) k_hash_ds2(PoseidonDev P, DS D, fr_t* __restrict__ out) {
    extern __shared__ uint4 lds[];
    constexpr int rate = T - 1;
    PairState s = pair_setup(lds);
    const size_t k0 = (size_t)blockIdx.x * 64 + s.lane; const bool live = k0 < D.n_out; const size_t k = live ? k0 : D.n_out - 1;
    const int o0 = s.isY ? PairCfg<T>::NX : 0, o1 = s.isY ? T : PairCfg<T>::NX;
    for (int j = o0; j < o1; ++j) s.sto(j, fr_zero<PF>());
    __syncthreads();
    const size_t total = D.total(k), nperm = (total + rate - 1) / rate;
    const size_t max_perm = (D.max_total() + rate - 1) / rate;
    const size_t skip = max_perm - nperm;
    size_t q = 0; fr_t res = fr_zero<PF>();
    for (size_t pidx = 0; pidx < max_perm; ++pidx) {
        if (pidx >= skip) {
            if (skip && pidx == skip) for (int j = o0; j < o1; ++j) s.sto(j, fr_zero<PF>());
            for (int cur = 0; cur < rate && q < total; ++cur, ++q) {
                if (cur < o0 || cur >= o1) continue;
                s.sto(cur, fr_add<PF>(s.ld(cur), D.elem(k, q)));
            }
        }
        __syncthreads();
        res = pair_permute<T, BLK8, false>(s, P, pidx + 1 == max_perm);
        __syncthreads();
    }
    if (live && !s.isY) stg(out + k0, res);
}

template <bool BLK8>
__global__ void __launch_bounds__(128) __attribute__((amdgpu_waves_per_eu(2))) k_node16_pair(PoseidonDev P, fr_t arity_f, fr_t level_f, fr_t label_f, uint64_t pos0,
                                                    const fr_t* __restrict__ in, size_t n_out, fr_t* __restrict__ out) {
    extern __shared__ uint4 lds[];
    PairState s = pair_setup(lds);
    const size_t k0 = (size_t)blockIdx.x * 64 + s.lane; const bool live = k0 < n_out; const size_t k = live ? k0 : n_out - 1;
    const fr_t* c = in + k * 16;
    static_assert(PairCfg<17>::NX == 8, "X fills elements 0..7");
    if (!s.isY) {
        s.sto(0, arity_f); s.sto(1, level_f); s.sto(2, fr_from_u64<PF>(pos0 + k)); s.sto(3, label_f);
#pragma unroll
        for (int j = 4; j < 8; ++j) s.sto(j, ldg(c + (j - 4)));
    } else {
#pragma unroll
        for (int j = 8; j < 16; ++j) s.sto(j, ldg(c + (j - 4)));
        s.sto(16, fr_zero<PF>());
    }
    __syncthreads();
    pair_permute<17, BLK8>(s, P, false);
    if (!s.isY) {
#pragma unroll
        for (int j = 0; j < 4; ++j) s.sto(j, fr_add<PF>(s.ld(j), ldg(c + 12 + j)));
        s.sto(4, fr_add<PF>(s.ld(4), fr_one<PF>()));
    }
    __syncthreads();
    const fr_t res = pair_permute<17, BLK8>(s, P, true);
    if (live && !s.isY) stg(out + k0, res);
}

}
#endif
```

Measured before the change: 13.01 million trace rows/s.

## Fuse leaf round-0 MDS into MFMA with folded constants and MFMA squeeze row

After: 13.33 million trace rows/s, median of 6. 1.02x the previous value.

```diff
diff --git a/stark_mlwe_amd/csrc/capi_poseidon.hip b/stark_mlwe_amd/csrc/capi_poseidon.hip
--- a/stark_mlwe_amd/csrc/capi_poseidon.hip
+++ b/stark_mlwe_amd/csrc/capi_poseidon.hip
@@ -54,20 +54,16 @@
 
 static int32_t ctx_leaf_init(stark_ctx* ctx, fr_t** out) {
     if (!ctx->leaf_init) {
-        const fr_t AB = host::h_tag("FSv1-ABSORB-BYTES"), CH = host::h_tag("FSv1-CHALLENGE");
-        fr_t init[17]; for (auto& x : init) x = host::h_zero();
-        init[0] = AB; init[1] = host::h_words("FRI/leaf/poseidon")[0]; init[2] = AB; init[3] = host::h_words("FRI/leaf")[0];
-         init[6] = CH; init[7] = AB; init[8] = host::h_words("leaf")[0]; init[16] = host::h_tag("FSv1-TRANSCRIPT-INIT");
+        fr_t init[17]; host::leaf_template(init);
         stark_params* tp = nullptr; STARK_TRY(ctx_transcript_params(ctx, &tp));
         const host::PoseidonConsts& c = tp->ref;
-        fr_t blob[17 + 51 + 40];
+        fr_t blob[17 + 51 + 40 + 20];
+        static_assert(kLeafKrcOff == 51 + 40, "k_leaf_pair2<true> reads its table at leafc + kLeafKrcOff");
         for (auto& x : blob) x = host::h_zero();
         for (int j = 0; j < 17; ++j) blob[j] = init[j];
-        fr_t x[17]; for (int j = 0; j < 17; ++j) x[j] = fr_pow5<PallasFr>(host::h_add(init[j], c.rc_full[j]));
+        host::leaf_round0_consts(c, init, &blob[17], reinterpret_cast<uint32_t*>(&blob[17 + kLeafKrcOff]));
         for (int i = 0; i < 17; ++i) {
-            fr_t k = host::h_zero();
-            for (int j = 0; j < 17; ++j) if (j != 4 && j != 5) k = host::h_add(k, host::h_mul(c.mds[(size_t)i * 17 + j], x[j]));
-            blob[17 + i] = k; blob[34 + i] = c.mds[(size_t)i * 17 + 4]; blob[51 + i] = c.mds[(size_t)i * 17 + 5];
+            blob[34 + i] = c.mds[(size_t)i * 17 + 4]; blob[51 + i] = c.mds[(size_t)i * 17 + 5];
             uint32_t* m45 = reinterpret_cast<uint32_t*>(&blob[68]);
             const fr_t k20 = fr_from_u64<PallasFr>(1ull << FR29_SBOX_SHIFT);
             fr29_const_from<PallasFr>(host::h_mul(c.mds[(size_t)i * 17 + 4], k20), m45 + 9 * i); fr29_const_from<PallasFr>(host::h_mul(c.mds[(size_t)i * 17 + 5], k20), m45 + 9 * (17 + i));
@@ -210,7 +206,7 @@
 }
 }
 static int32_t pair_block8_form(stark_ctx* ctx, const stark_params* p, bool* on) {
-    *on = ctx->opt.poseidon_block8 && p->dev.t == 17 && p->dev.rp % 8 == 0;
+    *on = ctx->opt.poseidon_block8 && p->dev.t == 17 && p->dev.rp % 8 == 0 && p->dev.rf >= 2;
     if (*on && (!p->dev.blk8_efrag || !p->dev.blk8_lfrag || !p->dev.blk8_unit_frag || !p->dev.blk8_gfrag || !p->dev.rc_partial_scaled29)) return ctx->fail(STARK_ERR_UNSUPPORTED, "poseidon_block8: the parameter set has no block-8 tables");
     return STARK_OK;
 }
@@ -296,6 +292,7 @@
     fr_t* init = nullptr; STARK_TRY(ctx_leaf_init(ctx, &init));
     const LeafStream L{init, f, f_next, m, n};
     bool b8 = false; STARK_TRY(pair_block8_form(ctx, tp, &b8));
+    if (tp->ref.rf < 4) b8 = false;
     switch (poseidon_form(ctx, tp, PoseidonOp::LeafLayer, n)) {
     case PoseidonForm::FiveWave: hipLaunchKernelGGL(k_leaf_pair_chain, dim3((unsigned)n), dim3(320), chain_lds_bytes(), st, tp->dev, row_consts_of(ctx), L, h); break;
     case PoseidonForm::OneWave: hipLaunchKernelGGL(k_leaf_pair_coop, dim3((unsigned)n), dim3(64), coop_lds_bytes(17), st, tp->dev, L, h); break;
diff --git a/stark_mlwe_amd/csrc/host_util.hpp b/stark_mlwe_amd/csrc/host_util.hpp
--- a/stark_mlwe_amd/csrc/host_util.hpp
+++ b/stark_mlwe_amd/csrc/host_util.hpp
@@ -334,6 +334,23 @@
     return k;
 }
 
+inline void leaf_template(fr_t init[17]) {
+    const fr_t AB = h_tag("FSv1-ABSORB-BYTES"), CH = h_tag("FSv1-CHALLENGE");
+    for (int j = 0; j < 17; ++j) init[j] = h_zero();
+    init[0] = AB; init[1] = h_words("FRI/leaf/poseidon")[0]; init[2] = AB; init[3] = h_words("FRI/leaf")[0];
+    init[6] = CH; init[7] = AB; init[8] = h_words("leaf")[0]; init[16] = h_tag("FSv1-TRANSCRIPT-INIT");
+}
+inline void leaf_round0_consts(const PoseidonConsts& c, const fr_t* init, fr_t* K, uint32_t* krc29) {
+    fr_t x[17]; for (int j = 0; j < 17; ++j) x[j] = fr_pow5<PF>(h_add(init[j], c.rc_full[j]));
+    for (int i = 0; i < 17; ++i) {
+        fr_t k = h_zero();
+        for (int j = 0; j < 17; ++j) if (j != 4 && j != 5) k = h_add(k, h_mul(c.mds[(size_t)i * 17 + j], x[j]));
+        K[i] = k;
+        const fr29_t u = fr29_unpack(h_add(k, c.rc_full[17 + i]));
+        for (int j = 0; j < 9; ++j) krc29[9 * i + j] = u.l[j];
+    }
+}
+
 inline void permute_dense(fr_t* s, const PoseidonConsts& c) {
     const int t = c.t, half = c.rf / 2; std::vector<fr_t> o(t);
     auto mds = [&]() { for (int i = 0; i < t; ++i) { fr_t acc = h_zero(); for (int j = 0; j < t; ++j) acc = h_add(acc, h_mul(c.mds[(size_t)i * t + j], s[j])); o[i] = acc; } for (int i = 0; i < t; ++i) s[i] = o[i]; };
diff --git a/stark_mlwe_amd/csrc/hostcheck.cpp b/stark_mlwe_amd/csrc/hostcheck.cpp
--- a/stark_mlwe_amd/csrc/hostcheck.cpp
+++ b/stark_mlwe_amd/csrc/hostcheck.cpp
@@ -245,22 +245,25 @@
     const int8_t* unit = k.blk8_lfrag.data() + k.blk8_lfrag.size() - 1024;
     std::vector<fr_t> st(t), xd(t), o(t);
     auto sbox = [&](int r) { for (int j = 0; j < t; ++j) xd[j] = recode_signed(fr_pow5_r29<PF>(fr_add<PF>(st[j], k.rc_full[(size_t)r * t + j]))); };
-    auto product = [&](const std::vector<int8_t>& F, int next) -> int {
+    fr_t rec[17]; uint32_t l0[9];
+    auto product = [&](const std::vector<int8_t>& F, int next, bool entry) -> int {
         for (int i = 0; i < t; ++i) {
             const int8_t* fr[17]; for (int e = 0; e < t; ++e) fr[e] = &F[((size_t)i * t + e) * 1024];
             int32_t S[32]; const int rc = blk8_tile_sums(fr, xd.data(), t, S); if (rc) return rc;
-            if (next < 0) { int64_t col[8]; mfma_word_cols_mad_of_sums(S, col); o[i] = mfma_finish_words_canonical(col); }
+            if (next < 0 && entry) { int64_t col[8]; mfma_word_cols_mad_of_sums(S, col); if (i == 0) mfma_finish_words(col, l0); else rec[i] = mfma_finish_bytes(col); }
+            else if (next < 0) { int64_t col[8]; mfma_word_cols_mad_of_sums(S, col); o[i] = mfma_finish_words_canonical(col); }
             else { uint32_t l[9]; blk8_finish_sums_limbs(S, l); o[i] = sbox_lazy29_recoded(l, &k.rc_full29[((size_t)next * t + i) * 9]); }
         }
-        if (next < 0) st = o; else xd = o;
+        if (next >= 0) xd = o; else if (!entry) st = o;
         return 0; };
     for (size_t s = 0; s < n; ++s) {
         for (int j = 0; j < t; ++j) st[j] = ld4(states + 4 * (s * t + j));
         sbox(0);
-        for (int r = 0; r < half; ++r) { const int rc = product(r == half - 1 ? k.mds_pre_frag : k.mds_frag, r == half - 1 ? -1 : r + 1); if (rc) return rc; }
-        fr_t rec[17], yd[9], kx[23];
-        fr29_t u = lazy29_add_c29(fr29_unpack(st[0]).l, &k.rc_partial_scaled29[0]);
-        for (int j = 1; j < t; ++j) rec[j] = recode_signed(st[j]);
+        for (int r = 0; r < half; ++r) { const int rc = product(r == half - 1 ? k.mds_pre_frag : k.mds_frag, r == half - 1 ? -1 : r + 1, r == half - 1); if (rc) return rc; }
+        fr_t yd[9], kx[23];
+        fr29_t zero9; for (int i = 0; i < 9; ++i) zero9.l[i] = 0;
+        fr29_t u = lazy29_add_c29(lazy29_add_slot(zero9, lazy29_to_slot(l0)).l, &k.rc_partial_scaled29[0]);
+        for (int i = 0; i < 9; ++i) if (u.l[i] >= (1u << 30)) return -4;
         const int nb = k.rp / 8;
         for (int b = 0; b < nb; ++b) {
             const int8_t* ef = k.blk8s_efrag.data() + (size_t)b * 8 * 16 * 1024; const int8_t* lf = k.blk8s_lfrag.data() + (size_t)b * 16 * 8 * 1024;
@@ -290,7 +293,7 @@
         }
         const fr29_t x0 = fr29_mul_c29(k.blk8_unscale29.data(), u);
         xd[0] = sbox_lazy29_recoded(x0.l, &k.rc_full29[((size_t)half * t) * 9]);
-        for (int r = half; r < k.rf; ++r) { const int rc = product(k.mds_frag, r == k.rf - 1 ? -1 : r + 1); if (rc) return rc; }
+        for (int r = half; r < k.rf; ++r) { const int rc = product(k.mds_frag, r == k.rf - 1 ? -1 : r + 1, false); if (rc) return rc; }
         for (int j = 0; j < t; ++j) st4(states + 4 * (s * t + j), st[j]);
     }
     return 0;
@@ -343,6 +346,17 @@
         for (int i = 0; i < 32; ++i) if (S[i] > lim || S[i] < -lim) return -1;
         int64_t* col = cols + 8 * s;
         if (wide) mfma_word_cols_of_sums<true>(S, col); else mfma_word_cols_of_sums<false>(S, col);
+        const fr_t d = mfma_finish_bytes(col, qh + s, carry + s); memcpy(digits + 32 * s, d.v, 32);
+    }
+    return 0;
+}
+int hc_mfma_finish_bytes_mad(const int32_t* sums, size_t n, int64_t* cols, int32_t* qh, int64_t* carry, int8_t* digits) {
+    const int32_t lim = 17 * 32 * 128 * 128;
+    for (size_t s = 0; s < n; ++s) {
+        const int32_t* S = sums + 32 * s;
+        for (int i = 0; i < 32; ++i) if (S[i] > lim || S[i] < -lim) return -1;
+        int64_t* col = cols + 8 * s;
+        mfma_word_cols_mad_of_sums(S, col);
         const fr_t d = mfma_finish_bytes(col, qh + s, carry + s); memcpy(digits + 32 * s, d.v, 32);
     }
     return 0;
@@ -427,13 +441,48 @@
     return 0;
 }
 }
-static void leaf_init(fr_t init[17]) {
-    const fr_t AB = host::h_tag("FSv1-ABSORB-BYTES"), CH = host::h_tag("FSv1-CHALLENGE");
-    for (int j = 0; j < 17; ++j) init[j] = host::h_zero();
-    init[0] = AB; init[1] = host::h_words("FRI/leaf/poseidon")[0]; init[2] = AB; init[3] = host::h_words("FRI/leaf")[0];
-    init[6] = CH; init[7] = AB; init[8] = host::h_words("leaf")[0]; init[16] = host::h_tag("FSv1-TRANSCRIPT-INIT");
-}
+static void leaf_init(fr_t init[17]) { host::leaf_template(init); }
 extern "C" {
+int hc_leaf_round0(void* tparams, const uint64_t* f, const uint64_t* f_next, size_t n, uint64_t* init_out, uint32_t* table_out, uint64_t* x45_out, uint32_t* limbs_out, uint64_t* sbox_out) {
+    HcParams* P = (HcParams*)tparams; const host::KernelConsts& k = P->kc;
+    if (k.t != 17 || k.mds_frag.empty() || k.rf < 2) return -1;
+    fr_t init[17], K[17]; uint32_t krc29[17 * 9];
+    leaf_init(init); host::leaf_round0_consts(P->ref, init, K, krc29);
+    if (init_out) for (int j = 0; j < 17; ++j) st4(init_out + 4 * j, init[j]);
+    if (table_out) memcpy(table_out, krc29, sizeof(krc29));
+    for (size_t s = 0; s < n; ++s) {
+        fr_t x[2], xd[2];
+        x[0] = fr_pow5_r29<PF>(fr_add<PF>(ld4(f + 4 * s), k.rc_full[4]));
+        x[1] = fr_pow5_r29<PF>(fr_add<PF>(f_next ? ld4(f_next + 4 * s) : host::h_zero(), k.rc_full[5]));
+        for (int e = 0; e < 2; ++e) { xd[e] = recode_signed(x[e]); if (x45_out) st4(x45_out + 4 * (2 * s + e), x[e]); }
+        for (int i = 0; i < 17; ++i) {
+            const int8_t* fr[2] = {&k.mds_frag[((size_t)i * 17 + 4) * 1024], &k.mds_frag[((size_t)i * 17 + 5) * 1024]};
+            int32_t S[32]; if (blk8_tile_sums(fr, xd, 2, S)) return -2;
+            for (int c = 0; c < 32; ++c) if (S[c] > 2 * 32 * 128 * 128 || S[c] < -2 * 32 * 128 * 128) return -2;
+            uint32_t l[9]; blk8_finish_sums_limbs(S, l);
+            if (limbs_out) memcpy(limbs_out + 9 * (17 * s + i), l, sizeof(l));
+            if (sbox_out) st4(sbox_out + 4 * (17 * s + i), sbox_lazy29(l, &krc29[9 * i]));
+        }
+    }
+    return 0;
+}
+size_t hc_row0_table(void* h, uint64_t* out, size_t cap) {
+    const std::vector<fr_t>& v = ((HcParams*)h)->kc.row0;
+    if (out) for (size_t i = 0; i < v.size() && i < cap; ++i) st4(out + 4 * i, v[i]);
+    return v.size();
+}
+int hc_squeeze_row(void* h, const uint64_t* states, size_t n, uint64_t* out) {
+    HcParams* P = (HcParams*)h; const host::KernelConsts& k = P->kc;
+    if (k.t != 17 || k.mds_frag.empty()) return -1;
+    const int8_t* fr[17]; for (int e = 0; e < 17; ++e) fr[e] = &k.mds_frag[(size_t)e * 1024];
+    for (size_t s = 0; s < n; ++s) {
+        fr_t xd[17]; for (int e = 0; e < 17; ++e) xd[e] = recode_signed(ld4(states + 4 * (17 * s + e)));
+        int32_t S[32]; if (blk8_tile_sums(fr, xd, 17, S)) return -2;
+        int64_t col[8]; mfma_word_cols_mad_of_sums(S, col);
+        st4(out + 4 * s, mfma_finish_words_canonical(col));
+    }
+    return 0;
+}
 int hc_leaf_pair(void* tparams, const uint64_t* f, const uint64_t* f_next, size_t n, size_t m, uint64_t* hout) {
     HcParams* P = (HcParams*)tparams;
     fr_t init[17]; leaf_init(init);
diff --git a/stark_mlwe_amd/csrc/poseidon_pair.hpp b/stark_mlwe_amd/csrc/poseidon_pair.hpp
--- a/stark_mlwe_amd/csrc/poseidon_pair.hpp
+++ b/stark_mlwe_amd/csrc/poseidon_pair.hpp
@@ -24,6 +24,7 @@
     __host__ __device__ static constexpr int dslot(int q) { return 1 + (q % NXD); }
     __host__ __device__ static constexpr size_t lds_bytes() { return (size_t)(T + EXTRA) * 2 * 64 * 16; }
 };
+constexpr int kLeafKrcOff = 51 + 40;
 static inline size_t pair_lds_bytes(int t) { return t == 17 ? PairCfg<17>::lds_bytes() : PairCfg<9>::lds_bytes(); }
 
 struct PairState {
@@ -122,11 +123,11 @@
     mfma_post_words(acc, col, c29);
     mfma_finish_words(col, l);
 }
-__device__ __forceinline__ void pair_sto_sbox29(const PairState& s, int j, const uint32_t* l, const uint32_t* rc29, bool recode) {
-    const fr29_t x5 = pow5_lazy29(lazy29_add_c29(l, rc29));
-    s.sto(j, recode ? recode_lazy29(x5) : fr29_pack_reduce<PF>(x5.l));
-}
-__device__ __forceinline__ void pair_mds_sbox_mfma(const PairState& s, const void* frag, const uint32_t* rc29, bool recode) {
+__device__ __forceinline__ void pair_sto_sbox29(const PairState& s, int j, const uint32_t* l, const uint32_t* rc29) {
+    s.sto(j, recode_lazy29(pow5_lazy29(lazy29_add_c29(l, rc29))));
+}
+constexpr int kEntrySlot = 17 + 2;
+__device__ __forceinline__ void pair_mds_sbox_mfma(const PairState& s, const void* frag, const uint32_t* rc29, bool entry = false) {
     constexpr int T = 17;
     const int lane = s.lane, h = lane >> 5;
     mfma_v4i b[T][2];
@@ -149,10 +150,43 @@
         }
         int64_t col[8];
         mfma_post_words(acc, col);
-        if (rc29) { uint32_t l[9]; mfma_finish_words(col, l); pair_sto_sbox29(s, i, l, c29(rc29, i), recode); }
+        if (rc29) { uint32_t l[9]; mfma_finish_words(col, l); pair_sto_sbox29(s, i, l, c29(rc29, i)); }
+        else if (entry) {
+            if (i == 0) { uint32_t l[9]; mfma_finish_words(col, l); s.sto(kEntrySlot, lazy29_to_slot(l)); }
+            else s.sto(i, mfma_finish_bytes(col));
+        }
         else s.sto(i, mfma_finish_words_canonical(col));
     }
     __syncthreads();
+}
+
+__device__ __forceinline__ mfma_v4i blk8_b_of_slot(const PairState& s, int j, int ct) {
+    const uint4 u = s.st[(2 * j + (s.lane >> 5)) * 64 + 32 * ct + (s.lane & 31)];
+    return mfma_v4i{(int)u.x, (int)u.y, (int)u.z, (int)u.w};
+}
+__device__ __forceinline__ fr_t pair_squeeze_row_mfma(const PairState& s, const void* frag) {
+    constexpr int T = 17;
+    const mfma_v4i* A = reinterpret_cast<const mfma_v4i*>(frag) + s.lane;
+    mfma_v16i acc[2];
+    mfma_zero_tile(acc);
+#pragma unroll 1
+    for (int e0 = 0; e0 < 16; e0 += 8) {
+        mfma_v4i a[8];
+#pragma unroll
+        for (int k = 0; k < 8; ++k) a[k] = A[(size_t)(e0 + k) * 64];
+#pragma unroll
+        for (int k = 0; k < 8; ++k)
+#pragma unroll
+            for (int ct = 0; ct < 2; ++ct) acc[ct] = __builtin_amdgcn_mfma_i32_32x32x32_i8(a[k], blk8_b_of_slot(s, e0 + k, ct), acc[ct], 0, 0, 0);
+    }
+    {
+        const mfma_v4i a = A[(size_t)16 * 64];
+#pragma unroll
+        for (int ct = 0; ct < 2; ++ct) acc[ct] = __builtin_amdgcn_mfma_i32_32x32x32_i8(a, blk8_b_of_slot(s, 16, ct), acc[ct], 0, 0, 0);
+    }
+    int64_t col[8];
+    mfma_post_words(acc, col);
+    return mfma_finish_words_canonical(col);
 }
 
 struct Blk8Tabs {
@@ -167,13 +201,35 @@
     __host__ __device__ static constexpr int ymail(int q) { return 17 + (q & 1); }
     __host__ __device__ static constexpr int hmail(int q) { return (q & 1) ? 19 : 0; }
 };
+static_assert(kEntrySlot == Blk8Cfg::hmail(1) && kEntrySlot != Blk8Cfg::hmail(0) && kEntrySlot != Blk8Cfg::ymail(0), "the entry row's slot is untouched until barrier_0");
 __device__ __forceinline__ void blk8_load_frags16(mfma_v4i (&a)[16], const mfma_v4i* A, int lane) {
 #pragma unroll
     for (int e = 0; e < 16; ++e) a[e] = (A + (size_t)e * 64)[lane];
 }
-__device__ __forceinline__ mfma_v4i blk8_b_of_slot(const PairState& s, int j, int ct) {
-    const uint4 u = s.st[(2 * j + (s.lane >> 5)) * 64 + 32 * ct + (s.lane & 31)];
-    return mfma_v4i{(int)u.x, (int)u.y, (int)u.z, (int)u.w};
+__device__ __forceinline__ void pair_leaf_round0_mfma(const PairState& s, const void* frag, const uint32_t* krc29) {
+    constexpr int T = 17;
+    mfma_v4i b[2][2];
+#pragma unroll
+    for (int e = 0; e < 2; ++e)
+#pragma unroll
+        for (int ct = 0; ct < 2; ++ct) b[e][ct] = blk8_b_of_slot(s, 4 + e, ct);
+    __syncthreads();
+    const mfma_v4i* A = reinterpret_cast<const mfma_v4i*>(frag) + s.lane;
+#pragma unroll 1
+    for (int i = s.isY ? 1 : 0; i < T; i += 2) {
+        mfma_v16i acc[2];
+        mfma_zero_tile(acc);
+        const mfma_v4i* Ai = A + ((size_t)i * T + 4) * 64;
+#pragma unroll
+        for (int e = 0; e < 2; ++e) {
+            const mfma_v4i a = Ai[(size_t)e * 64];
+#pragma unroll
+            for (int ct = 0; ct < 2; ++ct) acc[ct] = __builtin_amdgcn_mfma_i32_32x32x32_i8(a, b[e][ct], acc[ct], 0, 0, 0);
+        }
+        uint32_t l[9]; mfma_post_limbs(acc, l);
+        pair_sto_sbox29(s, i, l, c29(krc29, i));
+    }
+    __syncthreads();
 }
 template <int Q>
 __device__ __forceinline__ void blk8_round_x(const PairState& s, const Blk8Tabs& Tb, fr29_t& u, mfma_v4i (&b)[8][2]) {
@@ -210,7 +266,7 @@
     b[Q][0] = blk8_b_of_slot(s, Blk8Cfg::ymail(Q), 0); b[Q][1] = blk8_b_of_slot(s, Blk8Cfg::ymail(Q), 1);
 }
 template <int NLX, bool LAZY = false>
-__device__ __forceinline__ void blk8_lane_rows(const PairState& s, const Blk8Tabs& Tb, const mfma_v4i (&b)[8][2], bool last, const uint32_t* rc29_next = nullptr, bool recode_next = true) {
+__device__ __forceinline__ void blk8_lane_rows(const PairState& s, const Blk8Tabs& Tb, const mfma_v4i (&b)[8][2], bool last, const uint32_t* rc29_next = nullptr) {
     static_assert(NLX >= 1 && NLX <= 15, "shares");
     const int lane = s.lane;
     const int j0 = s.isY ? NLX + 1 : 1, j1 = s.isY ? 16 : NLX;
@@ -231,14 +287,14 @@
         const int jn = j < j1 ? j + 1 : j1;
 #pragma unroll
         for (int p = 0; p < 8; ++p) a[p] = (Tb.lfrag + ((size_t)(jn - 1) * 8 + p) * 64)[lane];
-        if (rc29_next) { uint32_t l[9]; mfma_post_limbs(acc, l); pair_sto_sbox29(s, j, l, c29(rc29_next, j), recode_next); }
+        if (rc29_next) { uint32_t l[9]; mfma_post_limbs(acc, l); pair_sto_sbox29(s, j, l, c29(rc29_next, j)); }
         else if (LAZY && !last) s.sto(j, mfma_post_bytes(acc));
         else { const fr_t z = mfma_post(acc); s.sto(j, last ? z : recode_signed(z)); }
     }
     __syncthreads();
 }
 template <int NLX, bool LAZY = false>
-__device__ __forceinline__ void pair_block8(const PairState& s, const Blk8Tabs& Tb, fr29_t& u, bool last, const uint32_t* rc29_next = nullptr, bool recode_next = true,
+__device__ __forceinline__ void pair_block8(const PairState& s, const Blk8Tabs& Tb, fr29_t& u, bool last, const uint32_t* rc29_next = nullptr,
                                             const uint32_t* unscale29 = nullptr) {
     mfma_v4i b[8][2];
     if (!s.isY) {
@@ -251,8 +307,8 @@
         blk8_round_y<4>(s, Tb, b, a, g); blk8_round_y<5>(s, Tb, b, a, g); blk8_round_y<6>(s, Tb, b, a, g); blk8_round_y<7>(s, Tb, b, a, g);
     }
     __builtin_amdgcn_sched_barrier(0);
-    if (rc29_next && !s.isY) { const fr29_t x = fr29_mul_c29(unscale29, u); pair_sto_sbox29(s, 0, x.l, c29(rc29_next, 0), recode_next); }
-    blk8_lane_rows<NLX, LAZY>(s, Tb, b, last, rc29_next, recode_next);
+    if (rc29_next && !s.isY) { const fr29_t x = fr29_mul_c29(unscale29, u); pair_sto_sbox29(s, 0, x.l, c29(rc29_next, 0)); }
+    blk8_lane_rows<NLX, LAZY>(s, Tb, b, last, rc29_next);
 }
 
 template <int T>
@@ -264,36 +320,44 @@
     return fr_add<PF>(base, fr_wide29_reduce_lazy<PF>(u));
 }
 
-template <int T, bool BLK8 = false, bool FUSE = BLK8>
+template <int T, bool BLK8 = false, bool FUSE = BLK8, bool SBOXED = false>
 __device__ __forceinline__ fr_t pair_permute(const PairState& s, const PoseidonDev& P, bool only0, int r_begin = 0) {
     static_assert(!BLK8 || T == 17, "8-round blocks exist for t = 17");
     static_assert(!FUSE || BLK8, "the fused hand-over belongs to the 8-round form");
+    static_assert(!SBOXED || FUSE, "entering behind an S-box belongs to the fused form");
     typedef PairCfg<T> Cfg;
     constexpr int NXD = Cfg::NXD, NXU = Cfg::NXU, W = 2 * T - 1;
     const int half = P.rf / 2;
     if constexpr (FUSE) {
-        if (r_begin < half) pair_sbox_full<T, true>(s, P.rc_full + r_begin * T);
+        if constexpr (!SBOXED) { if (r_begin < half) pair_sbox_full<T, true>(s, P.rc_full + r_begin * T); }
         for (int r = r_begin; r < half; ++r)
-            pair_mds_sbox_mfma(s, (r == half - 1) ? P.mds_pre_frag : P.mds_frag, (r == half - 1) ? nullptr : c29(P.rc_full29, (size_t)(r + 1) * T), true);
+            pair_mds_sbox_mfma(s, (r == half - 1) ? P.mds_pre_frag : P.mds_frag, (r == half - 1) ? nullptr : c29(P.rc_full29, (size_t)(r + 1) * T), r == half - 1);
     } else
     for (int r = r_begin; r < half; ++r) {
-        if constexpr (T == 17) { pair_sbox_full<T, true>(s, P.rc_full + r * T); pair_mds_sbox_mfma(s, (r == half - 1) ? P.mds_pre_frag : P.mds_frag, nullptr, true); }
+        if constexpr (T == 17) { pair_sbox_full<T, true>(s, P.rc_full + r * T); pair_mds_sbox_mfma(s, (r == half - 1) ? P.mds_pre_frag : P.mds_frag, nullptr); }
         else { pair_sbox_full<T>(s, P.rc_full + r * T); pair_apply_lu<T>(s, (r == half - 1) ? P.lu_pre29 : P.lu29); }
     }
     fr_t s0 = fr_zero<PF>();
-    if (!s.isY) s0 = s.ld(0);
+    if constexpr (!FUSE) { if (!s.isY) s0 = s.ld(0); }
     if constexpr (BLK8) {
-        fr29_t u = fr29_unpack(s0);
-        if (!s.isY) u = lazy29_add_c29(u.l, c29(P.rc_partial_scaled29, 0));
-        for (int j = s.isY ? 9 : 1; j <= (s.isY ? 16 : 8); ++j) s.sto(j, recode_signed(s.ld(j)));
-        __syncthreads();
+        fr29_t u;
+        if constexpr (FUSE) {
+#pragma unroll
+            for (int i = 0; i < 9; ++i) u.l[i] = 0;
+            if (!s.isY) { u = lazy29_add_slot(u, s.ld(kEntrySlot)); u = lazy29_add_c29(u.l, c29(P.rc_partial_scaled29, 0)); }
+        } else {
+            u = fr29_unpack(s0);
+            if (!s.isY) u = lazy29_add_c29(u.l, c29(P.rc_partial_scaled29, 0));
+            for (int j = s.isY ? 9 : 1; j <= (s.isY ? 16 : 8); ++j) s.sto(j, recode_signed(s.ld(j)));
+            __syncthreads();
+        }
         const int nb = P.rp / 8;
 #pragma unroll 1
         for (int b = 0; b < nb; ++b) {
             const Blk8Tabs Tb{reinterpret_cast<const mfma_v4i*>(P.blk8_efrag) + (size_t)b * 8 * 16 * 64, reinterpret_cast<const mfma_v4i*>(P.blk8_lfrag) + (size_t)b * 16 * 8 * 64,
                               reinterpret_cast<const mfma_v4i*>(P.blk8_unit_frag), reinterpret_cast<const mfma_v4i*>(P.blk8_gfrag) + (size_t)b * 28 * 64,
                               c29(P.rc_partial_scaled29, (size_t)8 * b + 1)};
-            if constexpr (FUSE) pair_block8<Blk8Cfg::NLX, true>(s, Tb, u, b == nb - 1, b == nb - 1 ? c29(P.rc_full29, (size_t)half * T) : nullptr, !(only0 && half == P.rf - 1), P.blk8_unscale29());
+            if constexpr (FUSE) pair_block8<Blk8Cfg::NLX, true>(s, Tb, u, b == nb - 1, b == nb - 1 ? c29(P.rc_full29, (size_t)half * T) : nullptr, P.blk8_unscale29());
             else pair_block8<Blk8Cfg::NLX>(s, Tb, u, b == nb - 1);
         }
         if constexpr (!FUSE) { if (!s.isY) s0 = fr29_pack_reduce<PF>(fr29_mul_c29(P.blk8_unscale29(), u).l); }
@@ -352,8 +416,16 @@
     for (int r = half; r < P.rf; ++r) {
         const bool squeeze = only0 && r == P.rf - 1;
         if constexpr (FUSE) {  }
-        else if constexpr (T == 17) { if (squeeze) pair_sbox_full<T>(s, P.rc_full + r * T); else pair_sbox_full<T, true>(s, P.rc_full + r * T); }
+        else if constexpr (T == 17) pair_sbox_full<T, true>(s, P.rc_full + r * T);
         else pair_sbox_full<T>(s, P.rc_full + r * T);
+        if constexpr (T == 17) {
+            if (squeeze) {
+                fr_t out = fr_zero<PF>();
+                if (!s.isY) out = pair_squeeze_row_mfma(s, P.mds_frag);
+                __syncthreads();
+                return out;
+            }
+        } else
         if (squeeze) {
             const int j0 = s.isY ? Cfg::NX : 0, j1 = s.isY ? T : Cfg::NX;
             DotAcc acc; acc.init();
@@ -365,8 +437,8 @@
             __syncthreads();
             return out;
         }
-        if constexpr (FUSE) pair_mds_sbox_mfma(s, P.mds_frag, r == P.rf - 1 ? nullptr : c29(P.rc_full29, (size_t)(r + 1) * T), !(only0 && r + 1 == P.rf - 1));
-        else if constexpr (T == 17) pair_mds_sbox_mfma(s, P.mds_frag, nullptr, true); else pair_apply_lu<T>(s, P.lu29);
+        if constexpr (FUSE) pair_mds_sbox_mfma(s, P.mds_frag, r == P.rf - 1 ? nullptr : c29(P.rc_full29, (size_t)(r + 1) * T));
+        else if constexpr (T == 17) pair_mds_sbox_mfma(s, P.mds_frag, nullptr); else pair_apply_lu<T>(s, P.lu29);
     }
     return s.ld(0);
 }
@@ -383,6 +455,14 @@
     extern __shared__ uint4 lds[];
     PairState s = pair_setup(lds);
     const size_t i = (size_t)blockIdx.x * 64 + s.lane; const bool live = i < n; const size_t ii = live ? i : n - 1;
+    if constexpr (BLK8) {
+        const fr_t in = s.isY ? (f_next ? ldg(f_next + ii / m) : fr_zero<PF>()) : ldg(f + ii);
+        s.sto(s.isY ? 5 : 4, recode_signed(fr_pow5_r29<PF>(fr_add<PF>(in, P.rc_full[s.isY ? 5 : 4]))));
+        __syncthreads();
+        pair_leaf_round0_mfma(s, P.mds_frag, reinterpret_cast<const uint32_t*>(leafc + kLeafKrcOff));
+        const fr_t out = pair_permute<17, true, true, true>(s, P, true, 1);
+        if (live && !s.isY) stg(h + i, out);
+    } else {
     const fr_t x4 = fr_pow5_r29<PF>(fr_add<PF>(ldg(f + ii), P.rc_full[4]));
     const fr_t x5 = fr_pow5_r29<PF>(fr_add<PF>(f_next ? ldg(f_next + ii / m) : fr_zero<PF>(), P.rc_full[5]));
     const int j0 = s.isY ? PairCfg<17>::NX : 0, j1 = s.isY ? 17 : PairCfg<17>::NX;
@@ -396,6 +476,7 @@
     __syncthreads();
     fr_t out = pair_permute<17, BLK8>(s, P, true, 1);
     if (live && !s.isY) stg(h + i, out);
+    }
 }
 
 template <int T, class DS, bool BLK8 = false>
```
